# BraveGroup/DCD

Hardware: AMD Instinct MI355X
Metric: images/sec DGDE train step (bs=8, 384x1280) (higher is better)
Workload: dtype f32; 1 GPU; DGDE train bs=8 fp32 on 1xMI355X, synthetic KITTI 384x1280 + random kpts_ann (DGDE.yaml, DLA-34+DCNv2, 6 objects/image); global_batch=8, per_gpu_batch=8, input=384x1280, parallelism=dp1, dcn_precision=f32, step_launch=eager, sync_bn=False

## Files before the change

dcd_amd/_ext.py:

```python
import torch

from . import _lib

import threading

PRECISION = {"f32": 0, "bf16x3": 1, "bf16": 2}
_default_precision = "f32"
_scoped = threading.local()


def set_precision(name):
    global _default_precision
    if name not in PRECISION:
        raise ValueError("precision must be one of %s" % sorted(PRECISION))
    _default_precision = name


def get_precision():
    return getattr(_scoped, "name", None) or _default_precision


class precision_scope:

    def __init__(self, name):
# ... 25 lines not shown
    _lib.require_cuda(input, weight, bias, offset, mask)
    for name, t in (("input", input), ("weight", weight), ("bias", bias), ("offset", offset), ("mask", mask)):
        if t.dtype != torch.float32:
            raise RuntimeError("%s must be float32 (the op is fp32-only, like the reference)" % name)
    if input.dim() != 4 or weight.dim() != 4:
        raise RuntimeError("input and weight must be 4-D")
    if weight.shape[2] != kernel_h or weight.shape[3] != kernel_w:
        raise RuntimeError("Input shape and kernel shape wont match: (%d x %d vs %d x %d)." % (
            kernel_h, kernel_w, weight.shape[2], weight.shape[3]))
    if input.shape[1] != weight.shape[1]:
        raise RuntimeError("Input shape and kernel channels wont match: (%d vs %d)." % (input.shape[1], weight.shape[1]))
    if bias.numel() != weight.shape[0]:
        raise RuntimeError("bias must have Cout elements")


def _dims(input, weight, kernel_h, kernel_w, stride_h, stride_w, pad_h, pad_w, dilation_h, dilation_w):
    B, C, H, W = input.shape
    Ho = (H + 2 * pad_h - (dilation_h * (kernel_h - 1) + 1)) // stride_h + 1
    Wo = (W + 2 * pad_w - (dilation_w * (kernel_w - 1) + 1)) // stride_w + 1
    return B, C, H, W, weight.shape[0], Ho, Wo


def _workspace(L, input, geom):
    nbytes = L.dcd_dcn_v2_workspace_bytes(*geom)
    if nbytes == 0:
        raise RuntimeError("dcn_v2: unsupported geometry %s" % (geom,))
    return torch.empty(nbytes, dtype=torch.uint8, device=input.device), nbytes


def dcn_v2_forward(input, weight, bias, offset, mask, kernel_h, kernel_w, stride_h, stride_w,
                   pad_h, pad_w, dilation_h, dilation_w, deformable_group, precision=None):
    _check(input, weight, bias, offset, mask, kernel_h, kernel_w)
    L = _lib.lib()
    B, C, H, W, Co, Ho, Wo = _dims(input, weight, kernel_h, kernel_w, stride_h, stride_w, pad_h, pad_w,
                                   dilation_h, dilation_w)
    if tuple(offset.shape) != (B, 2 * deformable_group * kernel_h * kernel_w, Ho, Wo):
        raise RuntimeError("offset shape %s does not match (B, 2*dg*kh*kw, Ho, Wo)" % (tuple(offset.shape),))
    if tuple(mask.shape) != (B, deformable_group * kernel_h * kernel_w, Ho, Wo):
        raise RuntimeError("mask shape %s does not match (B, dg*kh*kw, Ho, Wo)" % (tuple(mask.shape),))
    input, weight, bias, offset, mask = (t.contiguous() for t in (input, weight, bias, offset, mask))
    geom = (B, C, H, W, Co, kernel_h, kernel_w, stride_h, stride_w, pad_h, pad_w, dilation_h, dilation_w,
            deformable_group)
    ws, nbytes = _workspace(L, input, geom)
    output = torch.empty((B, Co, Ho, Wo), dtype=torch.float32, device=input.device)
    prec = PRECISION[precision or get_precision()]
    st = L.dcd_dcn_v2_forward(_lib.stream_of(input), input.data_ptr(), weight.data_ptr(), bias.data_ptr(),
                              offset.data_ptr(), mask.data_ptr(), output.data_ptr(), *geom, prec,
                              ws.data_ptr(), nbytes)
    _lib.check(st, "dcd_dcn_v2_forward")
    return output


def dcn_v2_backward(input, weight, bias, offset, mask, grad_output, kernel_h, kernel_w, stride_h, stride_w,
                    pad_h, pad_w, dilation_h, dilation_w, deformable_group, precision=None):
    _check(input, weight, bias, offset, mask, kernel_h, kernel_w)
    _lib.require_cuda(grad_output)
    if not input.is_contiguous():
        raise RuntimeError("input tensor has to be contiguous")
    if not weight.is_contiguous():
        raise RuntimeError("weight tensor has to be contiguous")
    L = _lib.lib()
    B, C, H, W, Co, Ho, Wo = _dims(input, weight, kernel_h, kernel_w, stride_h, stride_w, pad_h, pad_w,
                                   dilation_h, dilation_w)
    if tuple(grad_output.shape) != (B, Co, Ho, Wo):
        raise RuntimeError("grad_output shape %s does not match the output" % (tuple(grad_output.shape),))
    if grad_output.dtype != torch.float32:
        raise RuntimeError("grad_output must be float32")
    bias, offset, mask, grad_output = (t.contiguous() for t in (bias, offset, mask, grad_output))
    geom = (B, C, H, W, Co, kernel_h, kernel_w, stride_h, stride_w, pad_h, pad_w, dilation_h, dilation_w,
            deformable_group)
    ws, nbytes = _workspace(L, input, geom)
    grad_input = torch.empty_like(input)
    grad_offset = torch.empty_like(offset)
    grad_mask = torch.empty_like(mask)
    grad_weight = torch.empty_like(weight)
    grad_bias = torch.empty_like(bias)
    prec = PRECISION[precision or get_precision()]
    st = L.dcd_dcn_v2_backward(_lib.stream_of(input), input.data_ptr(), weight.data_ptr(), bias.data_ptr(),
                               offset.data_ptr(), mask.data_ptr(), grad_output.data_ptr(),
                               grad_input.data_ptr(), grad_offset.data_ptr(), grad_mask.data_ptr(),
                               grad_weight.data_ptr(), grad_bias.data_ptr(), *geom, prec, ws.data_ptr(), nbytes)
    _lib.check(st, "dcd_dcn_v2_backward")
    return [grad_input, grad_offset, grad_mask, grad_weight, grad_bias]
```

dcd_amd/_lib.py:

```python
import ctypes
import os

_HERE = os.path.dirname(os.path.abspath(__file__))
LIB_PATH = os.path.join(_HERE, "libdcd_hip.so")
_LIB = None

c_void_p, c_int, c_float, c_size_t, c_int64, c_double = (ctypes.c_void_p, ctypes.c_int, ctypes.c_float,
                                                         ctypes.c_size_t, ctypes.c_int64, ctypes.c_double)


class LossRowsArgs(ctypes.Structure):
    _INTS = ("B", "M", "C", "K", "NP", "num_classes", "ch_box2d", "ch_offset", "ch_corner", "ch_corner_unc", "ch_dims",
             "ch_ori_cls", "ch_ori_off", "ch_depth", "ch_depth_unc", "ch_kpts2d", "ch_kpts3d", "trunc_log")
    _FLOATS = ("depth_lo", "depth_hi", "unc_lo", "unc_hi", "depth_weight")
    _POINTERS = ("pois", "reg_mask", "trunc_mask", "find_pcl", "ori_mask", "cls_ids", "centers", "pad_size", "bboxes",
                 "locations", "rotys", "offset_3D", "dimensions", "orientations", "keypoints", "kp_depth_mask", "kpts2d",
                 "kpts3d", "calib_P", "calib", "dim_mean", "kps_pred", "kps_tgt", "kps3d_pred", "kps3d_tgt", "rot", "P_rows",
                 "kmask", "pair_depth", "pair_mask", "cols", "corners_pred", "corners_tgt", "iou3d", "sums", "grad_sums",
                 "grad_pois", "grad_pair", "grad_kps", "grad_kps3d")
    _fields_ = ([(n, c_int) for n in _INTS] + [(n, c_float) for n in _FLOATS] + [("dim_weight", c_float * 3)]
                + [("down_ratio", c_float), ("kd_eps", c_float)] + [(n, c_void_p) for n in _POINTERS])

HEADS_MAX = 16


class HeadRowsArgs(ctypes.Structure):
    _fields_ = ([(n, c_int) for n in ("n_heads", "T", "R", "K", "C")]
                + [(n, c_int * HEADS_MAX) for n in ("trunk", "ch0", "out")]
                + [("weight", c_void_p * HEADS_MAX), ("bias", c_void_p * HEADS_MAX), ("feat", c_void_p), ("y", c_void_p),
                   ("grad_y", c_void_p), ("grad_feat", c_void_p), ("grad_weight", c_void_p * HEADS_MAX),
                   ("grad_bias", c_void_p * HEADS_MAX)])


class EvalMatchArgs(ctypes.Structure):
    _INTS = ("mode", "n_img", "n_comb", "n_rows", "G", "D", "n_dc", "max_dt", "T", "n_slots")
    _POINTERS = ("gt_off", "dt_off", "dc_off", "pair_off", "overlaps", "ign_gt", "ign_dt", "dt_score", "gt_alpha", "dt_alpha",
                 "dt_box2d", "dc_box", "comb", "min_overlap", "thresholds", "n_thresh", "scores", "counts", "sim_part")
    _fields_ = [(n, c_int) for n in _INTS] + [("P", c_int64)] + [(n, c_void_p) for n in _POINTERS]


DECODE_MAX_CLASSES = 8


class DecodeArgs(ctypes.Structure):
    _INTS = ("B", "K", "C", "nk", "n_bins", "num_classes", "ch_box2d", "ch_offset", "ch_corner", "ch_corner_unc", "ch_dims",
             "ch_ori_cls", "ch_ori_off", "ch_depth", "ch_depth_unc", "ch_kpts2d", "ch_kpts3d", "orientation", "dim_mode",
             "dim_std_on", "depth_mode", "uncertainty_as_conf", "records")
    _FLOATS = ("down_ratio", "depth_lo", "depth_hi", "eps")
    _fields_ = ([(n, c_int) for n in _INTS] + [(n, c_float) for n in _FLOATS] + [("depth_ref", c_float * 2)]
                + [("dim_mean", c_float * 3 * DECODE_MAX_CLASSES), ("dim_std", c_float * 3 * DECODE_MAX_CLASSES)])


class RecordsArgs(ctypes.Structure):
    _INTS = ("B", "M", "C", "nk", "n_bins", "ch_offset", "ch_ori_cls", "ch_ori_off", "ch_kpts2d", "ch_kpts3d")
    _fields_ = [(n, c_int) for n in _INTS] + [("down_ratio", c_float)]


SIGNATURES = {
    "dcd_version": (ctypes.c_char_p, []),
    "dcd_dcn_v2_workspace_bytes": (c_size_t, [c_int] * 14),
    "dcd_dcn_v2_forward": (c_int, [c_void_p] * 7 + [c_int] * 15 + [c_void_p, c_size_t]),
    "dcd_dcn_v2_backward": (c_int, [c_void_p] * 12 + [c_int] * 15 + [c_void_p, c_size_t]),
    "dcd_dcn_v2_forget": (c_int, [c_void_p]),
    "dcd_dcn_v2_policy_state": (c_int, [c_void_p, c_void_p]),
    "dcd_dcn_v2_policy_free": (c_int, []),
    "dcd_dcn_v2_set_handover": (c_int, [c_int]),
    "dcd_edge_depth_forward": (c_int, [c_void_p] * 6 + [c_int, c_int, c_int, c_float, c_float, c_int, c_int]
                               + [c_void_p] * 3),
    "dcd_edge_depth_backward": (c_int, [c_void_p] * 7 + [c_int, c_int, c_int, c_float, c_float, c_int]
                                + [c_void_p] * 2),
    "dcd_focal_loss": (c_int, [c_void_p, c_void_p, c_void_p, c_int64, c_float, c_float, c_void_p, c_void_p]),
    "dcd_giou_loss": (c_int, [c_void_p, c_void_p, c_void_p, c_int, c_void_p, c_void_p, c_void_p]),
    "dcd_nms_hm": (c_int, [c_void_p, c_void_p, c_int, c_int, c_int, c_int, c_void_p]),
    "dcd_heatmap_topk": (c_int, [c_void_p, c_void_p] + [c_int] * 6 + [c_void_p] * 5 + [c_void_p, c_size_t]),
    "dcd_heatmap_topk_workspace_bytes": (c_size_t, [c_int] * 5),
    "dcd_poi_gather": (c_int, [c_void_p, c_void_p, c_void_p] + [c_int] * 5 + [c_void_p]),
    "dcd_poi_scatter_add": (c_int, [c_void_p, c_void_p, c_void_p] + [c_int] * 5 + [c_void_p]),
    "dcd_patch_scatter_add": (c_int, [c_void_p, c_void_p, c_void_p, c_int, c_int, c_int64, c_int, c_int, c_void_p]),
    "dcd_iou3d": (c_int, [c_void_p, c_void_p, c_void_p, c_int, c_void_p]),
    "dcd_conv3x3_workspace_bytes": (c_size_t, [c_int] * 5),
    "dcd_conv3x3": (c_int, [c_void_p] * 6 + [c_int] * 6 + [c_void_p, c_size_t]),
    "dcd_conv3x3_weights_bytes": (c_size_t, [c_int] * 3),
    "dcd_conv3x3_transform_weights": (c_int, [c_void_p, c_void_p, c_int, c_int, c_void_p, c_void_p]),
    "dcd_conv3x3_transform_weights_table": (c_int, [c_void_p, c_void_p, c_int]),
    "dcd_conv3x3_prepared": (c_int, [c_void_p] * 6 + [c_int] * 6 + [c_void_p, c_size_t]),
    "dcd_conv3x3_split_weights_bytes": (c_size_t, [c_int] * 3),
    "dcd_conv3x3_split_transform_weights": (c_int, [c_void_p, c_void_p, c_int, c_int, c_void_p, c_void_p]),
    "dcd_conv3x3_split_transform_weights_table": (c_int, [c_void_p, c_void_p, c_int]),
    "dcd_conv3x3_split_workspace_bytes": (c_size_t, [c_int] * 5),
    "dcd_conv3x3_split_prepared": (c_int, [c_void_p] * 6 + [c_int] * 7 + [c_void_p, c_size_t]),
    "dcd_conv1x1_bf16": (c_int, [c_void_p, c_void_p, c_int, c_int, c_int, c_void_p, c_void_p, c_void_p, c_int, c_int, c_int64]),
    "dcd_conv1x1_wrw_bf16_workspace_bytes": (c_size_t, [c_int, c_int, c_int, c_int64]),
    "dcd_conv1x1_wrw_bf16": (c_int, [c_void_p, c_void_p, c_void_p, c_void_p, c_int, c_int, c_int, c_int, c_int64, c_void_p, c_size_t]),
    "dcd_conv3x3_s2_f32": (c_int, [c_void_p, c_void_p, c_void_p, c_void_p, c_int, c_int, c_int, c_int, c_int]),
    "dcd_conv3x3_s2_f32_backward_data": (c_int, [c_void_p, c_void_p, c_void_p, c_void_p, c_int, c_int, c_int, c_int, c_int]),
    "dcd_conv3x3_s2_f32_wrw_workspace_bytes": (c_size_t, [c_int, c_int, c_int, c_int, c_int]),
    "dcd_conv3x3_s2_f32_wrw": (c_int, [c_void_p, c_void_p, c_void_p, c_void_p, c_int, c_int, c_int, c_int, c_int, c_void_p, c_size_t]),
    "dcd_clip_adamw_workspace_bytes": (c_size_t, [c_int, c_void_p]),
    "dcd_clip_grad_norm_scalars": (c_int, [c_void_p, c_int, c_void_p, c_void_p, c_float, c_void_p, c_size_t, c_void_p]),
    "dcd_adamw_apply": (c_int, [c_void_p, c_int] + [c_void_p] * 7 + [c_double] * 4 + [c_void_p]),
    "dcd_conv1x1_f32": (c_int, [c_void_p, c_void_p, c_int, c_int, c_int, c_void_p, c_void_p, c_void_p, c_int, c_int, c_int64]),
    "dcd_conv1x1_wrw_f32_workspace_bytes": (c_size_t, [c_int, c_int, c_int, c_int64]),
    "dcd_conv1x1_wrw_f32": (c_int, [c_void_p, c_void_p, c_void_p, c_void_p, c_int, c_int, c_int, c_int, c_int64, c_void_p, c_size_t]),
    "dcd_conv3x3_bf16_weights_bytes": (c_size_t, [c_int] * 3),
    "dcd_conv3x3_bf16_transform_weights": (c_int, [c_void_p, c_void_p, c_int, c_int, c_void_p, c_void_p]),
    "dcd_conv3x3_bf16_transform_weights_table": (c_int, [c_void_p, c_void_p, c_int]),
    "dcd_conv3x3_bf16_workspace_bytes": (c_size_t, [c_int] * 5),
    "dcd_conv3x3_bf16_prepared": (c_int, [c_void_p] * 6 + [c_int] * 6 + [c_void_p, c_size_t]),
    "dcd_conv_stem_workspace_bytes": (c_size_t, [c_int] * 3),
    "dcd_conv_stem": (c_int, [c_void_p] * 4 + [c_int] * 7 + [c_void_p, c_size_t]),
    "dcd_conv_stem_wrw_workspace_bytes": (c_size_t, [c_int] * 3),
    "dcd_conv_stem_wrw": (c_int, [c_void_p] * 4 + [c_int] * 6 + [c_void_p, c_size_t]),
    "dcd_context_norm_forward": (c_int, [c_void_p] * 4 + [c_int, c_int, c_float]),
    "dcd_context_norm_backward": (c_int, [c_void_p] * 5 + [c_int, c_int]),
    "dcd_context_norm_relu_add_forward": (c_int, [c_void_p] * 4 + [c_int, c_int, c_float]),
    "dcd_gmw_refine": (c_int, [c_void_p] * 5 + [c_int, c_void_p, c_void_p, c_int, c_int, c_int] + [c_void_p] * 3),
    "dcd_gmw_pack_records": (c_int, [c_void_p] * 4 + [c_int, c_int, c_void_p, c_int, c_int, c_int] + [c_void_p] * 9),
    "dcd_sum_tensors": (c_int, [c_void_p, c_void_p, c_int, c_void_p, c_int64]),
    "dcd_conv3x3_wrw_workspace_bytes": (c_size_t, [c_int] * 5),
    "dcd_conv3x3_wrw": (c_int, [c_void_p] * 4 + [c_int] * 6 + [c_void_p, c_size_t]),
    "dcd_upsample_dw_forward": (c_int, [c_void_p] * 4 + [c_int] * 5),
    "dcd_upsample_dw_forward_add": (c_int, [c_void_p] * 5 + [c_int] * 5),
    "dcd_maxpool2x2_forward": (c_int, [c_void_p, c_void_p, c_void_p, c_int64, c_int, c_int]),
    "dcd_maxpool2x2_backward": (c_int, [c_void_p, c_void_p, c_void_p, c_void_p, c_int64, c_int, c_int]),
    "dcd_upsample_dw_backward": (c_int, [c_void_p] * 6 + [c_int] * 5),
    "dcd_bn_workspace_bytes": (c_size_t, [c_int]),
    "dcd_bn_stats": (c_int, [c_void_p, c_void_p, c_int, c_int, c_int64, c_void_p, c_void_p, c_size_t]),
    "dcd_channel_sums": (c_int, [c_void_p, c_void_p, c_int, c_int, c_int64, c_void_p, c_void_p, c_size_t]),
    "dcd_bn_train_apply": (c_int, [c_void_p] * 6 + [c_double] + [c_void_p] * 3 + [c_float, c_float, c_int] + [c_void_p] * 3
                           + [c_int, c_int, c_int64]),
    "dcd_bn_eval_apply": (c_int, [c_void_p] * 7 + [c_float, c_int, c_void_p, c_int, c_int, c_int64]),
    "dcd_bn_backward_stats": (c_int, [c_void_p] * 5 + [c_int, c_int, c_int64, c_void_p, c_void_p, c_size_t]),
    "dcd_trunk_row_sums": (c_int, [c_void_p, c_void_p, c_void_p, c_int, c_int, c_void_p]),
    "dcd_trunk_finalize_forward": (c_int, [c_void_p, c_void_p, c_void_p, c_void_p, c_double, c_double, c_int, c_void_p, c_void_p, c_void_p]),
    "dcd_trunk_finalize_backward": (c_int, [c_void_p, c_void_p, c_void_p, c_void_p, c_void_p, c_double, c_int, c_void_p, c_void_p, c_void_p]),
    "dcd_trunk_grad_wg": (c_int, [c_void_p, c_void_p, c_void_p, c_int, c_int, c_void_p]),
    "dcd_bn_backward_relu_from_x": (c_int, [c_void_p] * 10 + [c_int, c_int, c_int64, c_void_p, c_size_t]),
    "dcd_bn_backward_stats_params_relu_from_x": (c_int, [c_void_p] * 7 + [c_int, c_int, c_int64, c_void_p, c_void_p, c_void_p, c_void_p, c_size_t]),
# ... 80 lines not shown
```

dcd_amd/csrc/conv.hip:

```cpp
#include <hip/hip_runtime.h>
#include <stdint.h>
#include <stdlib.h>

#include "../../include/dcd_hip.h"
#include "tuning_env.h"
#include "lds_limit.h"
#include "bf16_split.h"

typedef float f32x16 __attribute__((ext_vector_type(16)));
typedef float f32x4 __attribute__((ext_vector_type(4)));
typedef float f32x2 __attribute__((ext_vector_type(2)));

namespace {

constexpr int WN_CH = 8;
constexpr int WN_NT = 512;

template <int TR, int TC, int NB>
struct WinoGeom {
    static constexpr int KS = 32 * NB;
    static constexpr int U = 16 * KS * WN_CH;
    static constexpr int NTILE = TR * TC;
    static constexpr int ROWS = 4 * TR + 2;
    static constexpr int Q = (2 * TC + 8) / 4;
// ... 59 lines not shown
        for (int b = 0; b < 3; ++b) {
            t[0][b] = g[0][b];
            t[1][b] = 0.5f * (g[0][b] + g[1][b] + g[2][b]);
            t[2][b] = 0.5f * (g[0][b] - g[1][b] + g[2][b]);
            t[3][b] = g[2][b];
        }
#pragma unroll
        for (int xi = 0; xi < 4; ++xi) {
            const float u[4] = {t[xi][0], 0.5f * (t[xi][0] + t[xi][1] + t[xi][2]), 0.5f * (t[xi][0] - t[xi][1] + t[xi][2]), t[xi][2]};
#pragma unroll
            for (int nu = 0; nu < 4; ++nu)
                ul[((((size_t)(z * nchunk + ck) * 16 + xi * 4 + nu) * 2 + h) * WN_KS + kk) * 4 + s] = u[nu];
        }
    }
}

__global__ void wino_prep_weights(const float *__restrict__ w, float *__restrict__ ul, int Cc, int Kk, int mode, int nchunk, int nz,
                                  int WN_KS)
{
    wino_prep_body(w, ul, Cc, Kk, mode, nchunk, nz, WN_KS, blockIdx.x * blockDim.x + threadIdx.x, gridDim.x * blockDim.x);
}

struct PrepBoth {
    float *ul[2];
    int Cc[2], Kk[2], nchunk[2], nz[2], ks[2];
};

__global__ void wino_prep_weights_both(const float *__restrict__ w, PrepBoth p)
{
    const int mode = blockIdx.y;
    if (!p.ul[mode]) return;
    wino_prep_body(w, p.ul[mode], p.Cc[mode], p.Kk[mode], mode, p.nchunk[mode], p.nz[mode], p.ks[mode],
                   blockIdx.x * blockDim.x + threadIdx.x, gridDim.x * blockDim.x);
}

__global__ void wino_prep_weights_table(const long long *__restrict__ table)
{
    const long long *e = table + 5 * (size_t)blockIdx.z;
    const float *w = reinterpret_cast<const float *>(e[0]);
    const int mode = blockIdx.y;
    float *ul = reinterpret_cast<float *>(e[1 + mode]);
    if (!w || !ul) return;
    const int Cin = (int)e[3], Cout = (int)e[4];
    const int Cc = mode ? Cout : Cin, Kk = mode ? Cin : Cout;
    const int WN_KS = Kk <= 32 ? 32 : 64;
    wino_prep_body(w, ul, Cc, Kk, mode, (Cc + WN_CH - 1) / WN_CH, (Kk + WN_KS - 1) / WN_KS, WN_KS,
                   blockIdx.x * blockDim.x + threadIdx.x, gridDim.x * blockDim.x);
}

template <int TR, int TC, int NB>
__global__ __launch_bounds__(WN_NT) void wino_conv3x3_f32(const float *__restrict__ x, const float *__restrict__ ul, float *y,
                                                          float *__restrict__ part, const float *__restrict__ bias,
                                                          const float *residual, int Cc, int H, int W, int Kk, int tiles_x,
                                                          int nchunk, int nz)
{
    using G = WinoGeom<TR, TC, NB>;
    constexpr int WN_ROWS = G::ROWS, WN_RS = G::RS, WN_PLANE = G::PLANE, WN_IN = G::IN, WN_BUF = G::BUF, WN_Q = G::Q;
    constexpr int WN_KS = G::KS, WN_U = G::U;
    extern __shared__ __attribute__((aligned(16))) float lds[];
    const int tid = threadIdx.x;
    const int lane = tid & 63, wave = tid >> 6;
    const int p = lane & 31, h = lane >> 5;
    const int xi = wave & 3, tg = wave >> 2;
    int bx = blockIdx.x, b = blockIdx.y;
    xcd_remap(bx, b);
    const int ty = bx / tiles_x, tx = bx - ty * tiles_x;
    const int r0 = ty * (4 * TR), c0 = tx * (2 * TC);
    const int z = blockIdx.z % nz, ks = blockIdx.z / nz, ksplit = gridDim.z / nz;
    const int ck0 = (int)((int64_t)ks * nchunk / ksplit), ck1 = (int)((int64_t)(ks + 1) * nchunk / ksplit);
    const int HW = H * W;
    const bool live = p < G::NTILE;
    const int pe = live ? p : 0;
    const int trow = pe / TC, tcol = pe - trow * TC;

    const int ra = xi == 0 ? 0 : 1, rb = xi == 3 ? 3 : 2;
    const float sa = xi == 2 ? -1.f : 1.f, sb = (xi == 0 || xi == 3) ? -1.f : 1.f;
    const int lanebase = (2 * TR * tg + 2 * trow) * WN_RS + 2 + 2 * tcol + h * WN_PLANE;
    const int base1 = lanebase + ra * WN_RS, base2 = lanebase + rb * WN_RS;

    const float *x_b = x + (size_t)b * Cc * HW;
    const float *ul_z = ul + (size_t)z * nchunk * WN_U;

    constexpr int KIN = (WN_CH * WN_ROWS * WN_Q + WN_NT - 1) / WN_NT;
    constexpr int KW = WN_U / 4 / WN_NT;
    int sg[KIN], sl[KIN];
    bool sv_[KIN];
#pragma unroll
    for (int k = 0; k < KIN; ++k) {
        const int e = tid + WN_NT * k;
        const int ch = e / (WN_ROWS * WN_Q), rem = e - ch * (WN_ROWS * WN_Q);
        const int row = rem / WN_Q, q = rem - row * WN_Q;
        const int yy = r0 - 1 + row, xx = c0 - 4 + 4 * q;
        sv_[k] = e < WN_CH * WN_ROWS * WN_Q;
        sg[k] = (sv_[k] && yy >= 0 && yy < H && xx >= 0 && xx < W) ? ch * HW + yy * W + xx : -1;
        sl[k] = ch * WN_PLANE + row * WN_RS + 4 * q;
    }
    f32x4 rin[KIN];
    auto issue_w = [&](int ck, float *buf) {
        const float *src = ul_z + (size_t)ck * WN_U + 4 * tid;
        float *dst = buf + WN_IN + 4 * 64 * __builtin_amdgcn_readfirstlane(wave);
#pragma unroll
        for (int k = 0; k < KW; ++k)
            __builtin_amdgcn_global_load_lds(src + 4 * WN_NT * k, (__attribute__((address_space(3))) void *)(dst + 4 * WN_NT * k), 16, 0, 0);
    };
    auto issue = [&](int ck) {
        const float *src = x_b + (size_t)ck * WN_CH * HW;
        const int cleft = Cc - ck * WN_CH;
// ... 55 lines not shown
            if (s + 1 < 4) {
                win_read4(cp1 + 2 * (s + 1) * WN_PLANE, qa);
                win_read4(cp2 + 2 * (s + 1) * WN_PLANE, qb);
            }
#endif
            const float v[4] = {t0 - t2, t1 + t2, t2 - t1, t1 - t3};
            __builtin_amdgcn_sched_barrier(0);
#pragma unroll
            for (int nu = 0; nu < 4; ++nu) {
                acc[nu][0] = __builtin_amdgcn_mfma_f32_32x32x2f32(a0[nu][s], v[nu], acc[nu][0], 0, 0, 0);
                if (NB == 2) acc[nu][NB - 1] = __builtin_amdgcn_mfma_f32_32x32x2f32(a1[nu][s], v[nu], acc[nu][NB - 1], 0, 0, 0);
            }
        }
#ifndef WN_ABL_NOSTAGE
        if (ck + 1 < ck1) commit(lds + ((ck + 1 - ck0) & 1) * WN_BUF);
#endif
        asm volatile("s_waitcnt vmcnt(0)" ::: "memory");
        __syncthreads();
    }
#ifdef WN_ABL_NOEPI
    if (acc[0][0][0] != 123.456f) return;
#endif

    float *ex = lds;
    float *y_b = (ks == 0 ? y : part + (size_t)(ks - 1) * gridDim.y * Kk * HW) + (size_t)b * Kk * HW;
    const float *r_b = (residual && ks == 0) ? residual + (size_t)b * Kk * HW : nullptr;
    const int orow0 = r0 + 2 * TR * tg + 2 * trow, ocol = c0 + 2 * tcol;
#pragma unroll
    for (int mb = 0; mb < NB; ++mb) {
        float *mine = ex + (size_t)wave * 32 * 64 + lane;
#pragma unroll
        for (int r = 0; r < 16; ++r) {
            mine[r * 64] = acc[0][mb][r] + acc[1][mb][r] + acc[2][mb][r];
            mine[(16 + r) * 64] = acc[1][mb][r] - acc[2][mb][r] - acc[3][mb][r];
        }
        __syncthreads();
        const float *t0 = ex + (size_t)(tg * 4 + 0) * 32 * 64 + lane, *t1 = t0 + 32 * 64, *t2 = t1 + 32 * 64, *t3 = t2 + 32 * 64;
        if (live && ocol < W) {
#pragma unroll
            for (int rr = 0; rr < 4; ++rr) {
                const int r = 4 * xi + rr;
                const int k = z * WN_KS + mb * 32 + (r & 3) + 8 * (r >> 2) + 4 * h;
                const float a0 = t0[r * 64], a1 = t1[r * 64], a2 = t2[r * 64], a3 = t3[r * 64];
                const float b0 = t0[(16 + r) * 64], b1 = t1[(16 + r) * 64], b2 = t2[(16 + r) * 64], b3 = t3[(16 + r) * 64];
                if (k < Kk) {
                    const float bk = (bias && ks == 0) ? bias[k] : 0.f;
                    const size_t o = (size_t)k * HW + (size_t)orow0 * W + ocol;
                    float *dst = y_b + o;
                    f32x2 r0 = {bk, bk}, r1 = {bk, bk};
                    if (r_b) {
                        if (orow0 < H) r0 += *reinterpret_cast<const f32x2 *>(r_b + o);
                        if (orow0 + 1 < H) r1 += *reinterpret_cast<const f32x2 *>(r_b + o + W);
                    }
                    if (orow0 < H) *reinterpret_cast<f32x2 *>(dst) = f32x2{a0 + a1 + a2 + r0.x, b0 + b1 + b2 + r0.y};
                    if (orow0 + 1 < H) *reinterpret_cast<f32x2 *>(dst + W) = f32x2{a1 - a2 - a3 + r1.x, b1 - b2 - b3 + r1.y};
                }
            }
        }
        __syncthreads();
    }
}

constexpr int WS_CH = 16;

template <int NB>
__device__ __forceinline__ void wino_prep_split_body(const float *__restrict__ w, unsigned *__restrict__ us, int Cc, int Kk, int mode,
                                                     int nchunk, int nz, int first, int step)
{
    constexpr int KS = 32 * NB;
    const int n = nz * nchunk * KS * 2 * 4;
    for (int idx = first; idx < n; idx += step) {
        int r = idx;
        const int d = r & 3; r >>= 2;
        const int h = r & 1; r >>= 1;
        const int kk = r % KS; r /= KS;
        const int ck = r % nchunk, z = r / nchunk;
        const int k = z * KS + kk;
        float u[2][16];
#pragma unroll
        for (int e = 0; e < 2; ++e) {
            const int c = ck * WS_CH + 2 * (2 * d + e) + h;
            float g[3][3];
#pragma unroll
            for (int a = 0; a < 3; ++a)
#pragma unroll
                for (int b = 0; b < 3; ++b) {
                    float v = 0.f;
                    if (k < Kk && c < Cc)
                        v = mode == 0 ? w[(((size_t)k * Cc + c) * 3 + a) * 3 + b] : w[(((size_t)c * Kk + k) * 3 + (2 - a)) * 3 + (2 - b)];
                    g[a][b] = v;
                }
            float t[4][3];
#pragma unroll
            for (int b = 0; b < 3; ++b) {
                t[0][b] = g[0][b];
                t[1][b] = 0.5f * (g[0][b] + g[1][b] + g[2][b]);
                t[2][b] = 0.5f * (g[0][b] - g[1][b] + g[2][b]);
                t[3][b] = g[2][b];
            }
#pragma unroll
            for (int xi = 0; xi < 4; ++xi) {
                u[e][xi * 4 + 0] = t[xi][0];
                u[e][xi * 4 + 1] = 0.5f * (t[xi][0] + t[xi][1] + t[xi][2]);
                u[e][xi * 4 + 2] = 0.5f * (t[xi][0] - t[xi][1] + t[xi][2]);
                u[e][xi * 4 + 3] = t[xi][2];
            }
        }
        const int ob = kk >> 5, lane = h * 32 + (kk & 31);
// ... 521 lines not shown
    }
}

}

struct ConvPlan {
    int geom;
    int nb;
    int tiles_x, tiles_y, nchunk, nz, ksplit;
};

static int device_cus()
{
    static int cus = 0;
    if (!cus) {
        int dev = 0, n = 0;
        if (hipGetDevice(&dev) != hipSuccess || hipDeviceGetAttribute(&n, hipDeviceAttributeMultiprocessorCount, dev) != hipSuccess || n <= 0)
            n = 256;
        cus = n;
    }
    return cus;
}

static ConvPlan conv_plan(int B, int Cc, int H, int W, int Kk)
{
    ConvPlan best{};
    const int cus = device_cus();
    int64_t best_cost = -1;
    for (int g = 0; g < 2; ++g) {
        ConvPlan p;
        p.geom = g;
        p.tiles_x = g == 0 ? (W + 31) / 32 : (W + 19) / 20;
        p.tiles_y = g == 0 ? (H + 7) / 8 : (H + 11) / 12;
        p.nchunk = (Cc + WN_CH - 1) / WN_CH;
        p.nb = Kk <= 32 ? 1 : 2;
        p.nz = (Kk + 32 * p.nb - 1) / (32 * p.nb);
        const int64_t wgs = (int64_t)p.tiles_x * p.tiles_y * B * p.nz;
        static const int min_chunks = dcd_env("DCD_CONV_MINCHUNK") ? atoi(dcd_env("DCD_CONV_MINCHUNK")) : 4;
        int ks = 1;
        while (ks < 8 && wgs * (ks * 2) <= cus && p.nchunk / (ks * 2) >= min_chunks) ks *= 2;
        p.ksplit = ks;
        const int64_t rounds = (wgs * ks + cus - 1) / cus;
        const int64_t cost = rounds * ((p.nchunk + ks - 1) / ks + 2) * (g == 0 ? 16 : 17);
        if (best_cost < 0 || cost < best_cost) {
            best_cost = cost;
            best = p;
        }
    }
    return best;
}

template <int TR, int TC, int NB>
static int conv_launch(hipStream_t stream, const ConvPlan &pl, const float *input, const float *ul, float *output, float *part,
                       const float *bias, const float *residual, int B, int Cc, int H, int W, int Kk)
{
    static LdsLimit lds_limit;
    size_t ldsb = (size_t)2 * WinoGeom<TR, TC, NB>::BUF * sizeof(float);
    if (ldsb < (size_t)8 * 32 * 64 * sizeof(float)) ldsb = (size_t)8 * 32 * 64 * sizeof(float);
    if (!lds_limit.raise((int)ldsb, wino_conv3x3_f32<TR, TC, NB>)) return DCD_ERR_LAUNCH;
    hipLaunchKernelGGL((wino_conv3x3_f32<TR, TC, NB>), dim3(pl.tiles_x * pl.tiles_y, B, pl.nz * pl.ksplit), dim3(WN_NT), ldsb, stream,
                       input, ul, output, part, bias, residual, Cc, H, W, Kk, pl.tiles_x, pl.nchunk, pl.nz);
    return DCD_OK;
}

template <int NB, int NP>
static int conv_launch_split(hipStream_t stream, const ConvPlan &pl, const float *input, const unsigned *us, float *output, float *part,
                             const float *bias, const float *residual, int B, int Cc, int H, int W, int Kk)
{
    static LdsLimit lds_limit;
    using G = WinoGeom<2, 16, NB>;
    const size_t ldsb = ((size_t)((WS_CH * G::PLANE + 3) & ~3) + (size_t)2 * 16 * NB * 2 * 256) * sizeof(float);
    if (!lds_limit.raise((int)ldsb, wino_conv3x3_split<NB, NP>)) return DCD_ERR_LAUNCH;
    hipLaunchKernelGGL((wino_conv3x3_split<NB, NP>), dim3(pl.tiles_x * pl.tiles_y, B, pl.nz * pl.ksplit), dim3(WN_NT), ldsb, stream, input,
                       us, output, part, bias, residual, Cc, H, W, Kk, pl.tiles_x, pl.nchunk, pl.nz);
    return DCD_OK;
}

static ConvPlan conv_plan_split(int B, int Cc, int H, int W, int Kk)
{
    ConvPlan p;
    p.geom = 0;
    p.tiles_x = (W + 31) / 32;
    p.tiles_y = (H + 7) / 8;
    p.nchunk = (Cc + WS_CH - 1) / WS_CH;
    p.nb = Kk <= 32 ? 1 : 2;
    p.nz = (Kk + 32 * p.nb - 1) / (32 * p.nb);
    const int64_t wgs = (int64_t)p.tiles_x * p.tiles_y * B * p.nz;
    const int cus = device_cus();
    int ks = 1;
    while (ks < 8 && wgs * (ks * 2) <= cus && p.nchunk / (ks * 2) >= 2) ks *= 2;
    p.ksplit = ks;
    return p;
}

static bool conv_direct_ok(int Cc, int H, int W)
{
    return (int64_t)(Cc + DC_CH) * H * W < (1ll << 29);
}

static ConvPlan conv_plan_direct(int B, int Cc, int H, int W, int Kk)
{
    static const int pin = dcd_env("DCD_CONV_DIRECT_P") ? atoi(dcd_env("DCD_CONV_DIRECT_P")) : 0;
    const int cus = device_cus();
    ConvPlan best{};
    int64_t best_cost = -1;
    for (int P = 2; P <= 4; P += 2) {
        if (P != (pin == 4 ? 4 : 2)) continue;
        ConvPlan p;
        static const int wxpin = dcd_env("DCD_CONV_DIRECT_WX") ? atoi(dcd_env("DCD_CONV_DIRECT_WX")) : 0;
        const int wx = P == 2 && wxpin == 2 ? 2 : 1;
        p.geom = P | (wx << 4);
        p.tiles_x = (W + 32 * wx - 1) / (32 * wx);
        p.tiles_y = (H + 4 * P - 1) / (4 * P);
        p.nchunk = (Cc + DC_CH - 1) / DC_CH;
// ... 4 lines not shown
        int ks = 1;
        while (ks < 8) {
            const int64_t next = wgs * ks * 2;
            const int left = p.nchunk / (ks * 2);
            const bool fill = next <= 3 * cus && left >= min_chunks;
            const bool small = 2 * next <= 3 * cus && left >= 2;
            if (!fill && !small) break;
            ks *= 2;
        }
        p.ksplit = ks;
        best = p;
    }
    (void)best_cost;
    return best;
}

template <int NB, int P, int MODE, int WX>
static int conv_launch_direct(hipStream_t stream, const ConvPlan &pl, const float *input, const unsigned *wd, float *output, float *part,
                              const float *bias, const float *residual, int B, int Cc, int H, int W, int Kk)
{
    static LdsLimit lds_limit;
    const size_t ldsb = ((size_t)2 * (4 * P + 2) * (32 * WX + 8) + (size_t)2 * 9 * NB * 64) * 16;
    if constexpr (MODE == 2) {
        if (!lds_limit.raise((int)ldsb, conv3x3_direct_bf16_w4<NB, P, WX>)) return DCD_ERR_LAUNCH;
        hipLaunchKernelGGL((conv3x3_direct_bf16_w4<NB, P, WX>), dim3(pl.tiles_x * pl.tiles_y, B, pl.nz * pl.ksplit), dim3(DC_NT * WX), ldsb,
                           stream, input, wd, output, part, bias, residual, Cc, H, W, Kk, pl.tiles_x, pl.nchunk, pl.nz);
    } else {
        if (!lds_limit.raise((int)ldsb, conv3x3_direct_bf16<NB, P, MODE, WX>)) return DCD_ERR_LAUNCH;
        hipLaunchKernelGGL((conv3x3_direct_bf16<NB, P, MODE, WX>), dim3(pl.tiles_x * pl.tiles_y, B, pl.nz * pl.ksplit), dim3(DC_NT * WX), ldsb,
                           stream, input, wd, output, part, bias, residual, Cc, H, W, Kk, pl.tiles_x, pl.nchunk, pl.nz);
    }
    return DCD_OK;
}

static size_t tw_dwords_split(int Cin, int Cout, int backward_data)
{
    const int Cc = backward_data ? Cout : Cin, Kk = backward_data ? Cin : Cout;
    const int nb = Kk <= 32 ? 1 : 2;
    return (size_t)((Cc + WS_CH - 1) / WS_CH) * ((Kk + 32 * nb - 1) / (32 * nb)) * 16 * nb * 2 * 256;
}

extern "C" {

size_t dcd_conv3x3_workspace_bytes(int B, int Cin, int H, int W, int Cout)
{
    if (B <= 0 || Cin <= 0 || Cout <= 0 || H <= 0 || W <= 0) return 0;
    const int cmax = Cin > Cout ? Cin : Cout;
    const size_t nchunk = (size_t)(cmax + WN_CH - 1) / WN_CH, nz = (size_t)(cmax + 63) / 64;
    const ConvPlan f = conv_plan(B, Cin, H, W, Cout), d = conv_plan(B, Cout, H, W, Cin);
    const size_t pf = (size_t)(f.ksplit - 1) * B * Cout * H * W, pd = (size_t)(d.ksplit - 1) * B * Cin * H * W;
    return (nchunk * nz * 16 * 64 * WN_CH + (pf > pd ? pf : pd)) * sizeof(float);
}

static int conv3x3_run(hipStream_t stream, const float *input, const float *weights, int prepared, const float *bias,
                       const float *residual, float *output, int B, int Cin, int H, int W, int Cout, int backward_data, void *workspace,
                       size_t workspace_bytes)
{
    (void)hipGetLastError();
    if (!input || !weights || !output || B <= 0 || Cin <= 0 || Cout <= 0 || H <= 0 || W <= 0) return DCD_ERR_BAD_ARG;
    if ((W & 3) || (H & 1) || (int64_t)(Cin > Cout ? Cin : Cout) * H * W >= (1ll << 31) || (bias && backward_data)) return DCD_ERR_BAD_ARG;
    const int Cc = backward_data ? Cout : Cin, Kk = backward_data ? Cin : Cout;
    ConvPlan pl = conv_plan(B, Cc, H, W, Kk);
    if (const char *e = dcd_env("DCD_CONV_GEOM")) {
        const int g = atoi(e);
        if (g == 0 || g == 1) {
            ConvPlan q = pl;
            q.geom = g;
            q.tiles_x = g == 0 ? (W + 31) / 32 : (W + 19) / 20;
            q.tiles_y = g == 0 ? (H + 7) / 8 : (H + 11) / 12;
            q.ksplit = 1;
            pl = q;
        }
    }
    const int ksz = 32 * pl.nb;
    const size_t ul_floats = prepared ? 0 : (size_t)pl.nchunk * pl.nz * 16 * ksz * WN_CH;
    const size_t img = (size_t)B * Kk * H * W;
    const size_t need = (ul_floats + (size_t)(pl.ksplit - 1) * img) * sizeof(float);
    if (need && (!workspace || workspace_bytes < need)) return DCD_ERR_WORKSPACE;
    float *part = (float *)workspace + ul_floats;
    const float *ul = weights;
    if (!prepared) {
        const int nprep = pl.nz * pl.nchunk * ksz * WN_CH;
        hipLaunchKernelGGL(wino_prep_weights, dim3((nprep + 255) / 256 < 4096 ? (nprep + 255) / 256 : 4096), dim3(256), 0, stream, weights,
                           (float *)workspace, Cc, Kk, backward_data ? 1 : 0, pl.nchunk, pl.nz, ksz);
        ul = (const float *)workspace;
    }
    const int st = pl.geom == 0 ? (pl.nb == 2 ? conv_launch<2, 16, 2>(stream, pl, input, ul, output, part, bias, residual, B, Cc, H, W, Kk)
                                              : conv_launch<2, 16, 1>(stream, pl, input, ul, output, part, bias, residual, B, Cc, H, W, Kk))
                                : (pl.nb == 2 ? conv_launch<3, 10, 2>(stream, pl, input, ul, output, part, bias, residual, B, Cc, H, W, Kk)
                                              : conv_launch<3, 10, 1>(stream, pl, input, ul, output, part, bias, residual, B, Cc, H, W, Kk));
    if (st != DCD_OK) return st;
    if (pl.ksplit > 1) {
        const size_t n4 = img / 4;
        const int nb = (int)((n4 + 255) / 256 < 2048 ? (n4 + 255) / 256 : 2048);
        hipLaunchKernelGGL(wino_sum_partials, dim3(nb), dim3(256), 0, stream, output, (const float *)part, n4, pl.ksplit - 1);
    }
    return hipGetLastError() == hipSuccess ? DCD_OK : DCD_ERR_LAUNCH;
}

int dcd_conv3x3(void *stream_, const float *input, const float *weight, const float *bias, const float *residual, float *output,
                int B, int Cin, int H, int W, int Cout, int backward_data, void *workspace, size_t workspace_bytes)
{
    if (!workspace) return DCD_ERR_BAD_ARG;
    return conv3x3_run((hipStream_t)stream_, input, weight, 0, bias, residual, output, B, Cin, H, W, Cout, backward_data, workspace,
                       workspace_bytes);
}

static size_t tw_floats(int Cin, int Cout, int backward_data)
{
    const int Cc = backward_data ? Cout : Cin, Kk = backward_data ? Cin : Cout;
    const int nb = Kk <= 32 ? 1 : 2, ks = 32 * nb;
    return (size_t)((Cc + WN_CH - 1) / WN_CH) * ((Kk + ks - 1) / ks) * 16 * ks * WN_CH;
}

size_t dcd_conv3x3_weights_bytes(int Cin, int Cout, int backward_data)
{
    return Cin > 0 && Cout > 0 ? tw_floats(Cin, Cout, backward_data) * sizeof(float) : 0;
}

int dcd_conv3x3_transform_weights(void *stream_, const float *weight, int Cin, int Cout, float *forward_out, float *backward_out)
{
    (void)hipGetLastError();
    if (!weight || Cin <= 0 || Cout <= 0 || (!forward_out && !backward_out)) return DCD_ERR_BAD_ARG;
    PrepBoth p;
    int nmax = 0;
    for (int mode = 0; mode < 2; ++mode) {
        const int Cc = mode ? Cout : Cin, Kk = mode ? Cin : Cout;
        p.ul[mode] = mode ? backward_out : forward_out;
        p.Cc[mode] = Cc;
        p.Kk[mode] = Kk;
        p.ks[mode] = Kk <= 32 ? 32 : 64;
        p.nchunk[mode] = (Cc + WN_CH - 1) / WN_CH;
        p.nz[mode] = (Kk + p.ks[mode] - 1) / p.ks[mode];
        const int n = p.nz[mode] * p.nchunk[mode] * p.ks[mode] * WN_CH;
        if (p.ul[mode] && n > nmax) nmax = n;
    }
    const int nb = (nmax + 255) / 256 < 4096 ? (nmax + 255) / 256 : 4096;
    hipLaunchKernelGGL(wino_prep_weights_both, dim3(nb, 2), dim3(256), 0, (hipStream_t)stream_, weight, p);
    return hipGetLastError() == hipSuccess ? DCD_OK : DCD_ERR_LAUNCH;
}

int dcd_conv3x3_transform_weights_table(void *stream_, const long long *table, int entries)
{
// ... 109 lines not shown
int dcd_conv3x3_bf16_transform_weights_table(void *stream_, const long long *table, int entries)
{
    (void)hipGetLastError();
    if (!table || entries <= 0 || entries > 65535) return DCD_ERR_BAD_ARG;
    hipLaunchKernelGGL(direct_prep_weights_table, dim3(32, 2, entries), dim3(256), 0, (hipStream_t)stream_, table);
    return hipGetLastError() == hipSuccess ? DCD_OK : DCD_ERR_LAUNCH;
}

size_t dcd_conv3x3_bf16_workspace_bytes(int B, int Cin, int H, int W, int Cout)
{
    if (B <= 0 || Cin <= 0 || Cout <= 0 || H <= 0 || W <= 0) return 0;
    const size_t pf = (size_t)(conv_plan_direct(B, Cin, H, W, Cout).ksplit - 1) * B * Cout * H * W;
    const size_t pd = (size_t)(conv_plan_direct(B, Cout, H, W, Cin).ksplit - 1) * B * Cin * H * W;
    return (pf > pd ? pf : pd) * sizeof(float) + 16;
}

int dcd_conv3x3_bf16_prepared(void *stream_, const float *input, const void *transformed, const float *bias, const float *residual,
                              float *output, int B, int Cin, int H, int W, int Cout, int backward_data, void *workspace,
                              size_t workspace_bytes)
{
    hipStream_t stream = (hipStream_t)stream_;
    (void)hipGetLastError();
    if (!input || !transformed || !output || B <= 0 || Cin <= 0 || Cout <= 0 || H <= 0 || W <= 0) return DCD_ERR_BAD_ARG;
    if (bias && backward_data) return DCD_ERR_BAD_ARG;
    const int Cc = backward_data ? Cout : Cin, Kk = backward_data ? Cin : Cout;
    if (!conv_direct_ok(Cc, H, W) || (int64_t)Kk * H * W >= (1ll << 31) || (W & 3)) return DCD_ERR_BAD_ARG;
    const ConvPlan pl = conv_plan_direct(B, Cc, H, W, Kk);
    const size_t img = (size_t)B * Kk * H * W;
    const size_t need = (size_t)(pl.ksplit - 1) * img * sizeof(float);
    if (need && (!workspace || workspace_bytes < need)) return DCD_ERR_WORKSPACE;
    if (pl.ksplit > 1 && (img & 3)) return DCD_ERR_BAD_ARG;
    float *part = (float *)workspace;
    const unsigned *wd = (const unsigned *)transformed;
    static const int mpin = dcd_env("DCD_CONV_DIRECT_MODE") ? atoi(dcd_env("DCD_CONV_DIRECT_MODE")) : -1;
    const int P = pl.geom & 15, wx = pl.geom >> 4;
    const int mode = P == 4 ? 0 : (mpin >= 0 ? mpin : 1);
#define DCD_DIRECT(NB_, P_, M_, WX_) conv_launch_direct<NB_, P_, M_, WX_>(stream, pl, input, wd, output, part, bias, residual, B, Cc, H, W, Kk)
#define DCD_DIRECT_NB(NB_)                                                                                                              \
    (P == 4 ? DCD_DIRECT(NB_, 4, 0, 1)                                                                                                  \
            : wx == 2 ? (mode == 2 ? DCD_DIRECT(NB_, 2, 2, 2) : DCD_DIRECT(NB_, 2, 1, 2))                                               \
                      : (mode == 2 ? DCD_DIRECT(NB_, 2, 2, 1) : mode == 1 ? DCD_DIRECT(NB_, 2, 1, 1) : DCD_DIRECT(NB_, 2, 0, 1)))
    const int st = pl.nb == 2 ? DCD_DIRECT_NB(2) : DCD_DIRECT_NB(1);
#undef DCD_DIRECT_NB
#undef DCD_DIRECT
    if (st != DCD_OK) return st;
    if (pl.ksplit > 1) {
        const size_t n4 = img / 4;
        const int nb = (int)((n4 + 255) / 256 < 2048 ? (n4 + 255) / 256 : 2048);
        hipLaunchKernelGGL(wino_sum_partials, dim3(nb), dim3(256), 0, stream, output, (const float *)part, n4, pl.ksplit - 1);
    }
    return hipGetLastError() == hipSuccess ? DCD_OK : DCD_ERR_LAUNCH;
}

int dcd_conv1x1_bf16(void *stream_, const float *weight, int ldw, int transposed, int n_inputs, const float *const *inputs,
                     const int *channels, float *output, int B, int M, long long HW)
{
    (void)hipGetLastError();
    if (!weight || !inputs || !channels || !output || n_inputs < 1 || n_inputs > 4 || B <= 0 || M <= 0 || HW <= 0 || (HW & 3) || ldw <= 0)
        return DCD_ERR_BAD_ARG;
    PwArgs a;
    a.n_in = n_inputs;
    a.K = 0;
    for (int i = 0; i < 4; ++i) {
        a.in[i] = i < n_inputs ? inputs[i] : nullptr;
        a.ch[i] = i < n_inputs ? channels[i] : 0;
        if (i < n_inputs && (!inputs[i] || channels[i] <= 0 || (channels[i] & 15) || (int64_t)channels[i] * HW >= (1ll << 29)))
            return DCD_ERR_BAD_ARG;
        a.K += a.ch[i];
    }
    if ((int64_t)M * HW >= (1ll << 31)) return DCD_ERR_BAD_ARG;
    a.w = weight; a.ldw = ldw; a.wt = transposed ? 1 : 0; a.out = output; a.M = M; a.HW = HW;
    const int nb = M <= 32 ? 1 : 2;
    dim3 grid((unsigned)((HW + 511) / 512), B, (M + 32 * nb - 1) / (32 * nb));
    if (nb == 2) hipLaunchKernelGGL(pw_conv_bf16<2>, grid, dim3(PW_NT), 0, (hipStream_t)stream_, a);
    else hipLaunchKernelGGL(pw_conv_bf16<1>, grid, dim3(PW_NT), 0, (hipStream_t)stream_, a);
    return hipGetLastError() == hipSuccess ? DCD_OK : DCD_ERR_LAUNCH;
}

static void pw_wrw_partition(int B, int O, int C, long long HW, int &nog, int &ncg, int &S)
{
    nog = (O + 63) / 64;
    ncg = (C + 127) / 128;
    const int64_t T = (int64_t)B * ((HW + 63) / 64);
    int64_t s = 2 * (int64_t)device_cus() / (nog * ncg);
    if (s > T / 4) s = T / 4;
    if (s < 1) s = 1;
    S = (int)s;
}

size_t dcd_conv1x1_wrw_bf16_workspace_bytes(int B, int O, int C, long long HW)
{
    if (B <= 0 || O <= 0 || C <= 0 || HW <= 0) return 0;
    int nog, ncg, S;
    pw_wrw_partition(B, O, C, HW, nog, ncg, S);
    return (size_t)nog * ncg * S * 64 * 128 * sizeof(float);
}

int dcd_conv1x1_wrw_bf16(void *stream_, const float *grad_output, const float *input, float *grad_weight, int ldw, int B, int O, int C,
                         long long HW, void *workspace, size_t workspace_bytes)
{
    hipStream_t stream = (hipStream_t)stream_;
    (void)hipGetLastError();
    if (!grad_output || !input || !grad_weight || !workspace || B <= 0 || O <= 0 || C <= 0 || HW <= 0 || (HW & 3) || ldw < C)
        return DCD_ERR_BAD_ARG;
    if ((int64_t)B * (O > C ? O : C) * HW >= (1ll << 29)) return DCD_ERR_BAD_ARG;
    int nog, ncg, S;
// ... 215 lines not shown
```

dcd_amd/csrc/dcn_bwd_sweep.inc:

```

#ifndef SW_ABL_TAPS
#define SW_ABL_TAPS 9
#endif
#ifdef SW_ABL_NOMFMA
__device__ __forceinline__ f32x4 sw_fake_mfma(float a, float b, f32x4 c) { c.x = fmaf(a, b, c.x); c.y += a; c.z += b; c.w = fmaf(a, b, c.w); return c; }
#define SW_MFMA(a, b, c) sw_fake_mfma(a, b, c)
#else
#define SW_MFMA(a, b, c) __builtin_amdgcn_mfma_f32_16x16x4f32(a, b, c, 0, 0, 0)
#endif
constexpr int SW_PX = 16;
constexpr int SW_WW = 24;
constexpr int SW_RING = 9;
constexpr int SW_CH = 16;
constexpr int SW_CELLS = SW_RING * SW_WW;
constexpr int SW_PLANE = SW_CELLS + 3;
constexpr int SW_ZERO = SW_CELLS;
constexpr int SW_W_FLOATS = 9 * 16 * 64;
constexpr int SW_DW_FLOATS = 9 * 64 * SW_CH;
constexpr int SW_PART_FLOATS = SW_DW_FLOATS + 64;

__device__ __forceinline__ void sweep_prep_weights_body(const float *__restrict__ w, float *__restrict__ wp, const Geom &g, int nck, int nob,
                                                        int bid, int nb)
{
    const int n = nck * SW_W_FLOATS * nob;
// ... 761 lines not shown
            const int e = lane + 64 * k;
            const int ch = e / SW_WW, col = e - ch * SW_WW;
            const float gv = ring[(ch * SW_PLANE + sl * SW_WW + col) * 2 + 1];
            const int xx = x0 - 4 + col;
            if (gv != 0.f && ch < cleft && yy >= 0 && yy < H && xx >= 0 && xx < W) atomicAdd(gin_c + (size_t)ch * HW + yy * W + xx, gv);
        }
    }

    if (DWK && !SPLIT) {
#pragma unroll
        for (int ob = 0; ob < 4; ++ob)
            accw[8][ob] = __builtin_amdgcn_mfma_f32_16x16x4f32(dyo_p3[ob], pend_col, accw[8][ob], 0, 0, 0);
    }
    }

    if (DWK) {
        float *dst = a.dwpart + ((size_t)ck * (a.nslot / a.nck) + (id0 / (8 * a.nck)) * 8 + (id0 & 7)) * SW_PART_FLOATS;
#pragma unroll
        for (int t = 0; t < 9; ++t)
#pragma unroll
            for (int ob = 0; ob < 4; ++ob)
#pragma unroll
                for (int i = 0; i < 4; ++i) dst[(t * 64 + 16 * ob + 4 * q + i) * SW_CH + j] = accw[t][ob][i];
#pragma unroll
        for (int ob = 0; ob < 4; ++ob) {
            float v_ = bsum[ob];
            v_ += __shfl_xor(v_, 16);
            v_ += __shfl_xor(v_, 32);
            if (q == 0) dst[SW_DW_FLOATS + 16 * ob + j] = v_;
        }
    }
}

__device__ __forceinline__ void sweep_reduce_coord_body(const float *__restrict__ cpart, float *__restrict__ goff,
                                                        float *__restrict__ gmsk, int B, int HW, int nck,
                                                        const unsigned *__restrict__ far_scal, int total_tiles, int bid, int nb)
{
    const bool zero = far_dominated(far_scal, total_tiles);
    const int64_t n4 = (int64_t)B * 27 * HW / 4, per_b4 = (int64_t)27 * HW / 4, off4 = (int64_t)18 * HW / 4;
    const size_t stride4 = (size_t)B * 27 * HW / 4;
    for (int64_t i = (int64_t)bid * blockDim.x + threadIdx.x; i < n4; i += (int64_t)nb * blockDim.x) {
        f32x4 s = {0.f, 0.f, 0.f, 0.f};
        if (!zero) s = reinterpret_cast<const f32x4 *>(cpart)[i];
        for (int ck = 1; ck < nck && !zero; ++ck) {
            const f32x4 v = reinterpret_cast<const f32x4 *>(cpart)[i + ck * stride4];
            s.x += v.x; s.y += v.y; s.z += v.z; s.w += v.w;
        }
        const int64_t b = i / per_b4, r = i - b * per_b4;
        if (r < off4) reinterpret_cast<f32x4 *>(goff)[b * off4 + r] = s;
        else reinterpret_cast<f32x4 *>(gmsk)[b * (per_b4 - off4) + (r - off4)] = s;
    }
}

__device__ __forceinline__ void sweep_reduce_dw_body(const float *__restrict__ part, float *__restrict__ gw, float *__restrict__ gbias,
                                                     const Geom &g, int nck, int nvp, const unsigned *__restrict__ far_scal,
                                                     int total_tiles, int bx, int nbx, int by, int nby)
{
    if (far_dominated(far_scal, total_tiles)) return;
    const int n = nck * SW_DW_FLOATS + 64;
    const int v0 = (int)((int64_t)by * nvp / nby), v1 = (int)((int64_t)(by + 1) * nvp / nby);
    for (int idx = bx * blockDim.x + threadIdx.x; idx < n; idx += nbx * blockDim.x) {
        const bool is_bias = idx >= nck * SW_DW_FLOATS;
        const int ck = is_bias ? 0 : idx / SW_DW_FLOATS, e = is_bias ? SW_DW_FLOATS + (idx - nck * SW_DW_FLOATS) : idx - ck * SW_DW_FLOATS;
        const int c = e & 15, o = is_bias ? e - SW_DW_FLOATS : (e >> 4) & 63, t = e >> 10;
        const int cc = ck * SW_CH + c;
        if (o >= g.Co || (!is_bias && cc >= g.C)) continue;
        const float *src = part + (size_t)ck * nvp * SW_PART_FLOATS + e;
        float s = 0.f;
#pragma unroll 8
        for (int vv = v0; vv < v1; ++vv) s += src[(size_t)vv * SW_PART_FLOATS];
        if (is_bias) atomicAdd(gbias + o, s);
        else atomicAdd(gw + ((size_t)o * g.C + cc) * 9 + t, s);
    }
}

__device__ __forceinline__ void sweep_reduce_gemm_body(const float *__restrict__ part, float *__restrict__ gw, int n, int S,
                                                       const unsigned *__restrict__ far_scal, int total_tiles, int bid, int nb)
{
    if (far_dominated(far_scal, total_tiles)) return;
    for (int i = (bid * blockDim.x + threadIdx.x) * 4; i < n; i += nb * blockDim.x * 4) {
        if (i + 3 < n) {
            f32x4 acc = {0.f, 0.f, 0.f, 0.f};
            for (int s = 0; s < S; ++s) acc += *reinterpret_cast<const f32x4 *>(part + (size_t)s * n + i);
            *reinterpret_cast<f32x4 *>(gw + i) = acc;
        } else {
            for (int j = 0; i + j < n; ++j) {
                float a = 0.f;
                for (int s = 0; s < S; ++s) a += part[(size_t)s * n + i + j];
                gw[i + j] = a;
            }
        }
    }
}

struct SweepEpilogueArgs {
    const float *cpart, *gy, *dwpart;
    float *goff, *gmsk, *gw, *gbias;
    const unsigned *far_scal, *bias_only_if_far;
    Geom g;
    int nck, nvp, total_tiles, nb_coord, bias_splits, dw_bx, dw_by, gemm_n, gemm_S;
    unsigned *far_report = nullptr;
    unsigned far_base = 0;
};
__global__ __launch_bounds__(256) void dcn_sweep_epilogue(SweepEpilogueArgs a)
{
    int bid = blockIdx.x;
    if (a.far_report && bid == 0 && threadIdx.x == 0) {
        const unsigned c = a.far_scal[3] & ~FAR_BY_COUNT;
        *a.far_report = c >= a.far_base ? c - a.far_base : 0u;
    }
    if (bid < a.nb_coord) {
        sweep_reduce_coord_body(a.cpart, a.goff, a.gmsk, a.g.B, a.g.HoWo, a.nck, a.far_scal, a.total_tiles, bid, a.nb_coord);
        return;
    }
    bid -= a.nb_coord;
    const int nb_bias = a.g.Co * a.bias_splits;
    if (bid < nb_bias) {
        bias_grad_body(a.gy, a.gbias, a.g.B, a.g.Co, a.g.HoWo, a.bias_only_if_far, bid % a.g.Co, bid / a.g.Co, a.bias_splits);
        return;
    }
    bid -= nb_bias;
    if (a.dw_by > 0)
        sweep_reduce_dw_body(a.dwpart, a.gw, a.gbias, a.g, a.nck, a.nvp, a.far_scal, a.total_tiles, bid % a.dw_bx, a.dw_bx, bid / a.dw_bx, a.dw_by);
    else
        sweep_reduce_gemm_body(a.dwpart, a.gw, a.gemm_n, a.gemm_S, a.far_scal, a.total_tiles, bid, (int)gridDim.x - a.nb_coord - nb_bias);
}

struct SweepPlan {
    int nck, nstrip, nseg, seg_rows, nv;
    int nslot;
    int nob;
    int dw_split, dw_kchunk;
    size_t wp_floats, cpart_floats, dw_floats, col_floats;
};
constexpr int SW_GEMM_T = 128, SW_GEMM_K = 16;

__host__ inline SweepPlan sweep_plan(const Geom &g)
{
    SweepPlan p;
    p.nck = (g.C + SW_CH - 1) / SW_CH;
    p.nstrip = (g.W + SW_PX - 1) / SW_PX;
    const int64_t base = (int64_t)g.B * p.nstrip * p.nck;
    static const int min_rows = dcd_env("DCD_SWEEP_MIN_ROWS") && atoi(dcd_env("DCD_SWEEP_MIN_ROWS")) > 0 ? atoi(dcd_env("DCD_SWEEP_MIN_ROWS")) : 3;
    int best = 1;
    int64_t best_cost = -1;
    for (int ns = 1; ns <= g.H; ++ns) {
        const int rows = (g.H + ns - 1) / ns;
        if (rows < min_rows && ns > 1) break;
        const int real_ns = (g.H + rows - 1) / rows;
        const int64_t total = base * real_ns;
        const int64_t cost = ((total + 1023) / 1024) * (rows + 5);
        if (best_cost < 0 || cost < best_cost) { best_cost = cost; best = real_ns; }
    }
    p.seg_rows = (g.H + best - 1) / best;
    p.nseg = (g.H + p.seg_rows - 1) / p.seg_rows;
    p.nv = g.B * p.nstrip * p.nseg;
    const int64_t units = (int64_t)((p.nv + 7) / 8) * 8 * p.nck;
    const int grp = 8 * p.nck;
    int64_t slots = units < 1024 ? units : (1024 / grp) * (int64_t)grp;
    if (slots < grp) slots = grp;
    if (const char *e = dcd_env("DCD_SWEEP_SLOTS")) {
        const int64_t v_ = atoll(e);
        slots = v_ <= 0 ? units : (v_ / grp > 0 ? v_ / grp : 1) * grp;
    }
// ... 45 lines not shown
```

dcd_amd/csrc/dcn_v2.hip:

```cpp

#include <hip/hip_runtime.h>
#include <stdint.h>
#include <stdlib.h>
#include <string.h>
#include <atomic>
#include <map>
#include <vector>
#include <mutex>
#include <utility>

#include "../../include/dcd_hip.h"
#include "tuning_env.h"
#include "lds_limit.h"

typedef float f32x16 __attribute__((ext_vector_type(16)));
typedef float f32x32 __attribute__((ext_vector_type(32)));

namespace {

template <int N> struct IntC {
    static constexpr int value = N;
};

struct Geom {
    int B, C, H, W, Co, kh, kw, sh, sw, ph, pw, dh, dw, dg;
    int Ho, Wo, HoWo, KK, cpg, cpgp, Kp, Cop;
};

__host__ inline int round_up(int x, int m) { return (x + m - 1) / m * m; }

__host__ inline bool make_geom(Geom &g, int B, int C, int H, int W, int Co, int kh, int kw, int sh, int sw, int ph,
                               int pw, int dh, int dw, int dg)
{
    if (B <= 0 || C <= 0 || H <= 0 || W <= 0 || Co <= 0 || kh <= 0 || kw <= 0 || sh <= 0 || sw <= 0 || ph < 0 ||
        pw < 0 || dh <= 0 || dw <= 0 || dg <= 0 || C % dg)
        return false;
    g.B = B; g.C = C; g.H = H; g.W = W; g.Co = Co; g.kh = kh; g.kw = kw; g.sh = sh; g.sw = sw;
    g.ph = ph; g.pw = pw; g.dh = dh; g.dw = dw; g.dg = dg;
    g.Ho = (H + 2 * ph - (dh * (kh - 1) + 1)) / sh + 1;
    g.Wo = (W + 2 * pw - (dw * (kw - 1) + 1)) / sw + 1;
    if (g.Ho <= 0 || g.Wo <= 0) return false;
    g.HoWo = g.Ho * g.Wo;
    g.KK = kh * kw;
    g.cpg = C / dg;
    g.cpgp = round_up(g.cpg, 32);
    g.Kp = dg * g.KK * g.cpgp;
    g.Cop = round_up(Co, 32);
    if ((int64_t)C * H * W >= (1ll << 31) || (int64_t)Co * g.HoWo >= (1ll << 31) ||
        (int64_t)g.Kp * g.Cop >= (1ll << 31) || (int64_t)dg * 2 * g.KK * g.HoWo >= (1ll << 31))
        return false;
    return true;
}

__device__ __forceinline__ void prep_weights_body(const float *__restrict__ w, float *__restrict__ wf, float *__restrict__ wb, const Geom &g,
                                                  int bid, int nb)
{
    const int n = g.Kp * g.Cop;
    for (int idx = bid * blockDim.x + threadIdx.x; idx < n; idx += nb * blockDim.x) {
        const int o = idx / g.Kp, kp = idx - o * g.Kp;
        const int seg = kp / g.cpgp, cc = kp - seg * g.cpgp;
        const int grp = seg / g.KK, t = seg - grp * g.KK;
        float v = 0.f;
        if (o < g.Co && cc < g.cpg) v = w[((size_t)o * g.C + grp * g.cpg + cc) * g.KK + t];
        wb[idx] = v;
        wf[(size_t)kp * g.Cop + o] = v;
    }
// ... 1927 lines not shown
__device__ __forceinline__ void zero_ranges_body(const ZeroRanges &z, unsigned bid, unsigned nb)
{
    if (z.mark_p && bid == 0 && threadIdx.x == 0) *z.mark_p = z.mark_v;
#pragma unroll
    for (int r = 0; r < 8; ++r) {
        unsigned *p = z.p[r];
        const unsigned n = z.n[r];
        for (unsigned i = bid * blockDim.x + threadIdx.x; i < n; i += nb * blockDim.x) p[i] = 0u;
    }
}
__global__ void dcn_zero_ranges(ZeroRanges z) { zero_ranges_body(z, blockIdx.x, gridDim.x); }

inline int pick_mb(int nb, int tiles_total)
{
    for (int mb = 8; mb > 1; mb >>= 1) {
        if (mb > nb) continue;
        if ((int64_t)tiles_total * ((nb + mb - 1) / mb) >= 1024) return mb;
    }
    return 1;
}

#include "dcn_v2_bf16x3.inc"
#include "dcn_bwd_sweep.inc"

}

namespace {

template <int V>
__global__ void dcn_offset_mask_split(const float *__restrict__ out, float *__restrict__ offset, float *__restrict__ mask, int B, int T,
                                      int64_t HW)
{
    const int64_t per_img = (int64_t)3 * T * HW / V, n = (int64_t)B * per_img;
    for (int64_t i = (int64_t)blockIdx.x * blockDim.x + threadIdx.x; i < n; i += (int64_t)gridDim.x * blockDim.x) {
        const int64_t b = i / per_img, r = (i - b * per_img) * V;
        const bool is_off = r < (int64_t)2 * T * HW;
        float *dst = is_off ? offset + b * 2 * T * HW + r : mask + b * T * HW + (r - (int64_t)2 * T * HW);
        if (V == 4) {
            f32x4 v = *reinterpret_cast<const f32x4 *>(out + b * 3 * T * HW + r);
            if (!is_off) {
#pragma unroll
                for (int j = 0; j < 4; ++j) v[j] = 1.f / (1.f + __expf(-v[j]));
            }
            *reinterpret_cast<f32x4 *>(dst) = v;
        } else {
            const float v = out[b * 3 * T * HW + r];
            *dst = is_off ? v : 1.f / (1.f + __expf(-v));
        }
    }
}

template <int V>
__global__ void dcn_offset_mask_merge(const float *__restrict__ goff, const float *__restrict__ gmask, const float *__restrict__ mask,
                                      float *__restrict__ gout, int B, int T, int64_t HW)
{
    const int64_t per_img = (int64_t)3 * T * HW / V, n = (int64_t)B * per_img;
    for (int64_t i = (int64_t)blockIdx.x * blockDim.x + threadIdx.x; i < n; i += (int64_t)gridDim.x * blockDim.x) {
        const int64_t b = i / per_img, r = (i - b * per_img) * V;
        const bool is_off = r < (int64_t)2 * T * HW;
        const int64_t rm = r - (int64_t)2 * T * HW;
        if (V == 4) {
            f32x4 v;
            if (is_off) v = *reinterpret_cast<const f32x4 *>(goff + b * 2 * T * HW + r);
            else {
                const f32x4 g = *reinterpret_cast<const f32x4 *>(gmask + b * T * HW + rm);
                const f32x4 m = *reinterpret_cast<const f32x4 *>(mask + b * T * HW + rm);
#pragma unroll
                for (int j = 0; j < 4; ++j) v[j] = g[j] * m[j] * (1.f - m[j]);
            }
            *reinterpret_cast<f32x4 *>(gout + b * 3 * T * HW + r) = v;
        } else {
            float v;
            if (is_off) v = goff[b * 2 * T * HW + r];
            else {
                const float m = mask[b * T * HW + rm];
                v = gmask[b * T * HW + rm] * m * (1.f - m);
            }
            gout[b * 3 * T * HW + r] = v;
        }
    }
}

}

#include "dcn_dense.inc"

extern "C" {

static size_t dw_partial_floats(int Cin, int Cout)
{
    const size_t nb = (size_t)((Cin + DW_CB - 1) / DW_CB) * ((Cout + TL_OB - 1) / TL_OB);
    return (nb > 512 ? nb : 512) * (size_t)(2 * 32 * DW_CB * 9);
}

static size_t tileflag_bytes(const Geom &g) { return ((size_t)g.B * ((g.H + 3) / 4) * ((g.W + 31) / 32) + 255) / 256 * 256; }

static size_t blockmax_bytes(const Geom &g)
{
    return ((size_t)g.B * g.dg * g.KK * ((g.Ho + 7) / 8) * ((g.Wo + 7) / 8) + 255) / 256 * 256 + tileflag_bytes(g);
}

static size_t base_workspace_bytes(const Geom &g)
{
    const size_t cells = (size_t)g.B * g.dg * g.KK * g.H * g.W;
    const size_t ntile = (size_t)g.B * ((g.HoWo + 31) / 32);
    const size_t n = (size_t)g.Kp * g.Cop * sizeof(float) * 2 + 256 + ((cells + 255) / 256 * 256) + cells * INV_CAP * 8 + 256 +
                     ((ntile + 255) / 256 * 256) + (ntile + 63) / 64 * 64 * sizeof(int) + dw_partial_floats(g.C, g.Co) * sizeof(float);
    return (n + 255) / 256 * 256 + blockmax_bytes(g);
}

size_t dcd_dcn_v2_workspace_bytes(int B, int Cin, int H, int W, int Cout, int kh, int kw, int sh, int sw, int ph,
                                  int pw, int dh, int dw, int dg)
{
    Geom g;
    if (!make_geom(g, B, Cin, H, W, Cout, kh, kw, sh, sw, ph, pw, dh, dw, dg)) return 0;
    return base_workspace_bytes(g) + dense_workspace_bytes(g) + sweep_workspace_bytes(g);
}

int dcd_dcn_v2_forward(void *stream_, const float *input, const float *weight, const float *bias,
                       const float *offset, const float *mask, float *output, int B, int Cin, int H, int W,
                       int Cout, int kh, int kw, int sh, int sw, int ph, int pw, int dh, int dw, int dg,
                       int precision, void *workspace, size_t workspace_bytes)
{
    hipStream_t stream = (hipStream_t)stream_;
    (void)hipGetLastError();
    Geom g;
    if (!input || !weight || !bias || !offset || !mask || !output || !workspace) return DCD_ERR_BAD_ARG;
    if (!make_geom(g, B, Cin, H, W, Cout, kh, kw, sh, sw, ph, pw, dh, dw, dg)) return DCD_ERR_BAD_ARG;
    if (precision != DCD_PREC_F32 && precision != DCD_PREC_BF16X3 && precision != DCD_PREC_BF16) return DCD_ERR_BAD_ARG;
    const bool split = precision != DCD_PREC_F32;
    const bool one = precision == DCD_PREC_BF16;
    const size_t nw = (size_t)g.Kp * g.Cop;
    if (workspace_bytes < nw * sizeof(float) * 2) return DCD_ERR_WORKSPACE;
    if (dense_ok(g, false)) {
        if (workspace_bytes < base_workspace_bytes(g) + dense_workspace_bytes(g)) return DCD_ERR_WORKSPACE;
        dense_forward(stream, input, weight, bias, offset, mask, output, g, (float *)((char *)workspace + base_workspace_bytes(g)),
                      precision);
        return hipGetLastError() == hipSuccess ? DCD_OK : DCD_ERR_LAUNCH;
    }
    float *wf = (float *)workspace, *wb = wf + nw;

    const int tiles = (g.HoWo + 31) / 32;
    const int nb = g.Cop / 32;
    const int mb = pick_mb(nb, tiles * B);
    dim3 grid((tiles + 3) / 4, B, (nb + mb - 1) / mb), block(256);
#ifndef DCN_NO_FWD_TILE
    if (kh == 3 && kw == 3 && sh == 1 && sw == 1 && ph == 1 && pw == 1 && dh == 1 && dw == 1 && dg == 1 && (W & 3) == 0 &&
        H >= 8 && W >= 32 && dcd_env("DCD_NO_TILE") == nullptr) {
        const int nz = (Cout + TL_OB - 1) / TL_OB;
        const int nchunk = split ? (Cin + TB_CH - 1) / TB_CH : (Cin + TL_CH - 1) / TL_CH;
        const size_t nwl = (size_t)nz * nchunk * (split ? TB_W_FLOATS : TL_W_FLOATS);
        if (nwl <= 2 * nw) {
            static LdsLimit lds_limit8, lds_limit4, lds_limit8b, lds_limit4b;
            static int tile_rows = 0;
            if (tile_rows == 0) {
                const char *e = dcd_env("DCD_TILE_ROWS");
                tile_rows = (e && atoi(e) == 4) ? 4 : 8;
            }
            if (!lds_limit8.raise((int)(2 * TileCfg<8>::BUF * sizeof(float)), dcn_fwd_tile_f32<8>) ||
                !lds_limit4.raise((int)(2 * TileCfg<4>::BUF * sizeof(float)), dcn_fwd_tile_f32<4>))
                return DCD_ERR_LAUNCH;
            if (split && (!lds_limit8b.raise((int)(TileCfgB<8>::NBUF * TileCfgB<8>::BUF * sizeof(float)), dcn_fwd_tile_bf16x3<8, 3>,
                                             dcn_fwd_tile_bf16x3<8, 1>) ||
                          !lds_limit4b.raise((int)(TileCfgB<4>::NBUF * TileCfgB<4>::BUF * sizeof(float)), dcn_fwd_tile_bf16x3<4, 3>,
                                             dcn_fwd_tile_bf16x3<4, 1>)))
                return DCD_ERR_LAUNCH;
            static int rescue_taps = 0;
            if (rescue_taps == 0) {
                const char *e = dcd_env("DCD_FWD_RESCUE_TAPS");
// ... 35 lines not shown
                }
#undef DCD_FWD_TILE_B
                else if (rows8)
                    hipLaunchKernelGGL(dcn_fwd_tile_f32<8>, dim3(regions, B, nz), dim3(512), 2 * TileCfg<8>::BUF * sizeof(float), stream,
                                       input, offset, mask, wf, bias, output, g, tiles_x, nchunk, flags, (const float *)wf9, rescue_taps_call,
                                       (const unsigned *)far_count, far_limit);
                else
                    hipLaunchKernelGGL(dcn_fwd_tile_f32<4>, dim3(regions, B, nz), dim3(256), 2 * TileCfg<4>::BUF * sizeof(float), stream,
                                       input, offset, mask, wf, bias, output, g, tiles_x, nchunk, flags, (const float *)wf9, rescue_taps_call,
                                       (const unsigned *)far_count, far_limit);
                if (keeps) return hipGetLastError() == hipSuccess ? DCD_OK : DCD_ERR_LAUNCH;
                const int nb9 = g.Cop / 32, mb9 = nb9 >= 4 ? 4 : nb9 >= 2 ? 2 : 1;
                dim3 gridr((tiles_x * g.Ho + 3) / 4, B, (nb9 + mb9 - 1) / mb9);
                if (mb9 == 4)
                    hipLaunchKernelGGL((dcn_fwd9_f32<4, true>), gridr, dim3(256), 0, stream, input, offset, mask, wf9, bias, output, g,
                                       (const unsigned char *)flags, tiles_x, TRr, nchunk);
                else if (mb9 == 2)
                    hipLaunchKernelGGL((dcn_fwd9_f32<2, true>), gridr, dim3(256), 0, stream, input, offset, mask, wf9, bias, output, g,
                                       (const unsigned char *)flags, tiles_x, TRr, nchunk);
                else
                    hipLaunchKernelGGL((dcn_fwd9_f32<1, true>), gridr, dim3(256), 0, stream, input, offset, mask, wf9, bias, output, g,
                                       (const unsigned char *)flags, tiles_x, TRr, nchunk);
                return hipGetLastError() == hipSuccess ? DCD_OK : DCD_ERR_LAUNCH;
            }
        }
    }
#endif
#ifndef DCN_NO_FWD9
    if (g.KK == 9 && W >= 2 && (size_t)Cin * 9 * g.Cop <= nw) {
        const size_t n9 = (size_t)Cin * 9 * g.Cop;
        hipLaunchKernelGGL(dcn_prep_weights9, dim3((unsigned)((n9 + 255) / 256 < 2048 ? (n9 + 255) / 256 : 2048)), dim3(256), 0,
                           stream, weight, wf, g);
        const int mb9 = mb > 4 ? 4 : mb;
        dim3 grid9((tiles + 3) / 4, B, (nb + mb9 - 1) / mb9);
        switch (mb9) {
            case 4: hipLaunchKernelGGL(dcn_fwd9_f32<4>, grid9, block, 0, stream, input, offset, mask, wf, bias, output, g); break;
            case 2: hipLaunchKernelGGL(dcn_fwd9_f32<2>, grid9, block, 0, stream, input, offset, mask, wf, bias, output, g); break;
            default: hipLaunchKernelGGL(dcn_fwd9_f32<1>, grid9, block, 0, stream, input, offset, mask, wf, bias, output, g); break;
        }
        return hipGetLastError() == hipSuccess ? DCD_OK : DCD_ERR_LAUNCH;
    }
#endif
    hipLaunchKernelGGL(dcn_prep_weights, dim3((unsigned)((nw + 255) / 256 < 2048 ? (nw + 255) / 256 : 2048)), dim3(256),
                       0, stream, weight, wf, wb, g);
    switch (mb) {
        case 8: hipLaunchKernelGGL(dcn_fwd_f32<8>, grid, block, 0, stream, input, offset, mask, wf, bias, output, g); break;
        case 4: hipLaunchKernelGGL(dcn_fwd_f32<4>, grid, block, 0, stream, input, offset, mask, wf, bias, output, g); break;
        case 2: hipLaunchKernelGGL(dcn_fwd_f32<2>, grid, block, 0, stream, input, offset, mask, wf, bias, output, g); break;
        default: hipLaunchKernelGGL(dcn_fwd_f32<1>, grid, block, 0, stream, input, offset, mask, wf, bias, output, g); break;
    }
    return hipGetLastError() == hipSuccess ? DCD_OK : DCD_ERR_LAUNCH;
}

int dcd_dcn_v2_backward(void *stream_, const float *input, const float *weight, const float *bias,
                        const float *offset, const float *mask, const float *grad_output, float *grad_input,
                        float *grad_offset, float *grad_mask, float *grad_weight, float *grad_bias, int B,
                        int Cin, int H, int W, int Cout, int kh, int kw, int sh, int sw, int ph, int pw, int dh,
                        int dw, int dg, int precision, void *workspace, size_t workspace_bytes)
{
    (void)bias;
    hipStream_t stream = (hipStream_t)stream_;
    (void)hipGetLastError();
    Geom g;
    if (!input || !weight || !offset || !mask || !grad_output || !grad_input || !grad_offset || !grad_mask ||
        !grad_weight || !grad_bias || !workspace)
        return DCD_ERR_BAD_ARG;
    if (!make_geom(g, B, Cin, H, W, Cout, kh, kw, sh, sw, ph, pw, dh, dw, dg)) return DCD_ERR_BAD_ARG;
    if (precision != DCD_PREC_F32 && precision != DCD_PREC_BF16X3 && precision != DCD_PREC_BF16) return DCD_ERR_BAD_ARG;
    const bool split = precision != DCD_PREC_F32;
    const bool one = precision == DCD_PREC_BF16;
    const size_t nw = (size_t)g.Kp * g.Cop;
    if (workspace_bytes + 256 < dcd_dcn_v2_workspace_bytes(B, Cin, H, W, Cout, kh, kw, sh, sw, ph, pw, dh, dw, dg))
        return DCD_ERR_WORKSPACE;
    float *wf = (float *)workspace, *wb = wf + nw;
    const size_t cells = (size_t)B * dg * g.KK * H * W;
    InvLists inv;
    unsigned *absmax = (unsigned *)(wb + nw);
    inv.absmax_bits = absmax;
    inv.cnt = (unsigned char *)absmax + 256;
    inv.idx = (int *)(inv.cnt + (cells + 255) / 256 * 256);
    inv.w = (float *)(inv.idx + cells * INV_CAP);
    inv.packed = 0;
    const size_t ntile = (size_t)B * ((g.HoWo + 31) / 32);
    unsigned char *far_flag = (unsigned char *)(((uintptr_t)(inv.w + cells * INV_CAP) + 255) / 256 * 256);
    int *far_list = (int *)(far_flag + (ntile + 255) / 256 * 256);
    float *dw_part = (float *)(far_list + (ntile + 63) / 64 * 64);
    unsigned char *blockmax = (unsigned char *)workspace + (base_workspace_bytes(g) - blockmax_bytes(g));
    inv.blockmax = blockmax;
    unsigned char *tileflag = (unsigned char *)workspace + (base_workspace_bytes(g) - tileflag_bytes(g));
    inv.tileflag = nullptr;
    inv.flag_tx = (W + 31) / 32;
    inv.flag_ty = (H + 3) / 4;
    const dim3 bm_grid(((g.Ho + 7) / 8) * ((g.Wo + 7) / 8), dg * g.KK, B);

    const char *sw_e = dcd_env("DCD_SWEEP_WIDE");
    const bool sweep_wide = !(sw_e && atoi(sw_e) == 0);
    const bool use_sweep = sweep_ok(g) && (g.Cop <= 64 || (sweep_wide && (g.Cop <= 128 || !dense_ok(g, true)))) && dense_mode() != 1 &&
                           (sweep_mode() == 1 || !dense_ok(g, true));
    unsigned *dense_report = nullptr;
    const bool far_to_dense = use_sweep && dense_ok(g, true) &&
                              handover_far_dominated(weight, far_count_limit(g, g.Co > 64), &dense_report);
    if ((!use_sweep || far_to_dense) && dense_ok(g, true)) {
        ZeroRanges z;
        for (int r = 0; r < 8; ++r) { z.p[r] = nullptr; z.n[r] = 0; }
        z.p[0] = absmax; z.n[0] = 4;
        z.p[1] = (unsigned *)far_flag; z.n[1] = (unsigned)((ntile + 3) / 4);
        z.p[3] = (unsigned *)grad_bias; z.n[3] = (unsigned)Cout;
        hipLaunchKernelGGL(dcn_zero_ranges, dim3(8), dim3(256), 0, stream, z);
        hipLaunchKernelGGL(dcn_prep_weights, dim3((unsigned)((nw + 255) / 256 < 2048 ? (nw + 255) / 256 : 2048)), dim3(256),
                           0, stream, weight, wf, wb, g);
        const int64_t noff = (int64_t)B * dg * 2 * g.KK * g.HoWo;
        int gsz = (int)((noff + 4095) / 4096);
        if (gsz > 512) gsz = 512;
        hipLaunchKernelGGL(dcn_offset_absmax, dim3(gsz), dim3(256), 0, stream, offset, noff, absmax, g.HoWo, dg * 2 * g.KK,
                           (g.HoWo + 31) / 32, far_flag, far_list);
        if (dense_report) hipLaunchKernelGGL(dcn_far_report, dim3(1), dim3(64), 0, stream, (const unsigned *)absmax, dense_report);
        hipLaunchKernelGGL(dcn_offset_blockmax, bm_grid, dim3(64), 0, stream, offset, g, blockmax);
        hipLaunchKernelGGL(dcn_build_inverse, dim3((H * W + 255) / 256, dg * g.KK, B), dim3(256), 0, stream, offset, mask, inv, g);
        int splits = (int)(((int64_t)g.HoWo + 4095) / 4096);
        if (splits > 32) splits = 32;
        hipLaunchKernelGGL(dcn_bias_grad, dim3(Cout, splits), dim3(256), 0, stream, grad_output, grad_bias, B, Cout, g.HoWo);
        dense_backward(stream, input, wb, offset, mask, grad_output, grad_input, grad_offset, grad_mask, grad_weight, g, inv,
                       (float *)((char *)workspace + base_workspace_bytes(g)), precision);
        return hipGetLastError() == hipSuccess ? DCD_OK : DCD_ERR_LAUNCH;
    }
    const int tiles = (g.HoWo + 31) / 32;
    const int nblk = g.cpgp / 32;
    if (!use_sweep)
        hipLaunchKernelGGL(dcn_prep_weights, dim3((unsigned)((nw + 255) / 256 < 2048 ? (nw + 255) / 256 : 2048)), dim3(256),
                           0, stream, weight, wf, wb, g);
    if (use_sweep) {
        const SweepPlan sp = sweep_plan(g);
        float *swp = (float *)((char *)workspace + base_workspace_bytes(g) + dense_workspace_bytes(g));
        float *cpart = swp + sp.wp_floats, *dwpart = cpart + sp.cpart_floats;
        const unsigned *fs = (const unsigned *)absmax;
        int nsplit = 1;
        while (nsplit * 2 <= nblk) nsplit *= 2;
        unsigned *far_report = nullptr;
        const unsigned real_limit = far_count_limit(g, sp.nob > 1);
        const int handover = handover_decide(stream, weight, real_limit, &far_report);
        const unsigned far_limit = handover ? real_limit : FAR_COUNT_PIVOT - 1;
        {
            const int nb_gen = handover ? (int)((nw + 255) / 256 < 1024 ? (nw + 255) / 256 : 1024) : 0;
            const int nb_sw = (int)((sp.wp_floats + 255) / 256 < 2048 ? (sp.wp_floats + 255) / 256 : 2048);
            hipLaunchKernelGGL(dcn_sweep_prologue_a, dim3(nb_gen + nb_sw), dim3(256), 0, stream, weight, wf, wb, swp, absmax, g, sp.nck, sp.nob,
                               split ? 1 : 0, nb_gen, far_limit);
        }
        {
            ZeroRanges z;
            for (int r = 0; r < 8; ++r) { z.p[r] = nullptr; z.n[r] = 0; }
            z.p[2] = (unsigned *)grad_weight; z.n[2] = (unsigned)((size_t)Cout * Cin * g.KK);
            z.p[3] = (unsigned *)grad_bias; z.n[3] = (unsigned)Cout;
            z.p[4] = (unsigned *)grad_input; z.n[4] = (unsigned)((size_t)B * Cin * H * W);
            const int nb_zero = (int)(z.n[4] / 1024 + 1 < 4096 ? z.n[4] / 1024 + 1 : 4096);
            const int64_t noff = (int64_t)B * 18 * g.HoWo;
            int nb_scan = (int)((noff + 4095) / 4096);
            if (nb_scan > 512) nb_scan = 512;
            hipLaunchKernelGGL(dcn_sweep_prologue_b, dim3(nb_zero + nb_scan), dim3(256), 0, stream, z, nb_zero, offset, noff, absmax, g.HoWo,
                               (g.HoWo + 31) / 32);
        }
        {
            SweepArgs a;
            a.in = input; a.off = offset; a.msk = mask; a.wp = swp; a.gy = grad_output; a.gin = grad_input; a.cpart = cpart;
            a.dwpart = dwpart; a.far_scal = fs; a.g = g; a.nstrip = sp.nstrip; a.nseg = sp.nseg; a.seg_rows = sp.seg_rows;
            a.nck = sp.nck; a.nv = sp.nv; a.nslot = sp.nslot;
            a.col = dwpart + sp.dw_floats;
            static LdsLimit sw_lds_limit;
            const int ldsb = SW_WAVES * SW_LDS_FLOATS * (int)sizeof(float);
            if (!sw_lds_limit.raise(ldsb, dcn_bwd_sweep<DCD_PREC_F32, 1, true>, dcn_bwd_sweep<DCD_PREC_BF16X3, 1, true>,
                                    dcn_bwd_sweep<DCD_PREC_F32, 2, false>, dcn_bwd_sweep<DCD_PREC_BF16X3, 2, false>,
                                    dcn_bwd_sweep<DCD_PREC_F32, 4, false>, dcn_bwd_sweep<DCD_PREC_BF16X3, 4, false>,
                                    dcn_bwd_sweep<DCD_PREC_BF16, 1, true>, dcn_bwd_sweep<DCD_PREC_BF16, 2, false>,
                                    dcn_bwd_sweep<DCD_PREC_BF16, 4, false>))
                return DCD_ERR_LAUNCH;
            const dim3 sgrid(sp.nslot / SW_WAVES), sblock(64 * SW_WAVES);
#define DCD_LAUNCH_SWEEP(NOBV, DWKV)                                                                                     \
    do {                                                                                                                \
        if (one) hipLaunchKernelGGL((dcn_bwd_sweep<DCD_PREC_BF16, NOBV, DWKV>), sgrid, sblock, ldsb, stream, a);        \
        else if (split) hipLaunchKernelGGL((dcn_bwd_sweep<DCD_PREC_BF16X3, NOBV, DWKV>), sgrid, sblock, ldsb, stream, a); \
        else hipLaunchKernelGGL((dcn_bwd_sweep<DCD_PREC_F32, NOBV, DWKV>), sgrid, sblock, ldsb, stream, a);             \
    } while (0)
            if (sp.nob == 1) DCD_LAUNCH_SWEEP(1, true);
            else if (sp.nob == 2) DCD_LAUNCH_SWEEP(2, false);
            else DCD_LAUNCH_SWEEP(4, false);
#undef DCD_LAUNCH_SWEEP
        }
        {
            SweepEpilogueArgs e;
            e.cpart = cpart; e.gy = grad_output; e.dwpart = dwpart; e.goff = grad_offset; e.gmsk = grad_mask; e.gw = grad_weight;
            e.gbias = grad_bias; e.far_scal = fs; e.g = g; e.nck = sp.nck; e.total_tiles = B * tiles;
            e.far_report = far_report; e.far_base = FAR_COUNT_PIVOT - far_limit;
            e.bias_only_if_far = sp.nob == 1 ? fs : (const unsigned *)nullptr;
            const int64_t n4 = (int64_t)B * 27 * g.HoWo / 4;
            e.nb_coord = (int)((n4 + 255) / 256 < 4096 ? (n4 + 255) / 256 : 4096);
            int splits = (int)(((int64_t)g.HoWo + 4095) / 4096);
            if (splits > 32) splits = 32;
            if (splits < 1) splits = 1;
            e.bias_splits = splits;
            int nb_dw;
            if (sp.nob == 1) {
                const int nred = sp.nck * SW_DW_FLOATS + 64;
                e.nvp = sp.nslot / sp.nck;
                e.dw_bx = (nred + 255) / 256;
                e.dw_by = e.nvp >= 64 ? 16 : (e.nvp >= 8 ? 4 : 1);
                e.gemm_n = 0; e.gemm_S = 0;
                nb_dw = e.dw_bx * e.dw_by;
            } else {
                static_assert(SW_GEMM_T == SG_T && SW_GEMM_K == SG_K, "sweep_plan sizes the product's partials with these");
                const int K9 = Cin * 9, n = Cout * K9;
                SgemmArgs ga;
                ga.A = grad_output; ga.B = dwpart + sp.dw_floats; ga.C = dwpart; ga.bias = nullptr; ga.M = Cout; ga.N = K9; ga.K = g.HoWo;
                ga.lda = g.HoWo; ga.ldb = g.HoWo; ga.ldc = K9;
                ga.strideA = (long long)Cout * g.HoWo; ga.strideB = (long long)K9 * g.HoWo;
                ga.strideC = (long long)sp.dw_split * n; ga.strideCs = n;
                ga.nsplit = sp.dw_split; ga.kchunk = sp.dw_kchunk; ga.ct = 0; ga.b_off = nullptr;
                ga.skip_count = fs + 3; ga.skip_above = FAR_COUNT_PIVOT;
                if (split) sgemm_bf16x3(stream, true, true, ga, B, one);
                else sgemm_f32(stream, true, true, ga, B);
                e.nvp = 0; e.dw_bx = 0; e.dw_by = 0;
                e.gemm_n = n; e.gemm_S = B * sp.dw_split;
                nb_dw = (n / 4 + 255) / 256 < 512 ? (n / 4 + 255) / 256 : 512;
            }
            hipLaunchKernelGGL(dcn_sweep_epilogue, dim3(e.nb_coord + Cout * splits + nb_dw), dim3(256), 0, stream, e);
        }
        if (!handover) return hipGetLastError() == hipSuccess ? DCD_OK : DCD_ERR_LAUNCH;
        inv.packed = 0;
        inv.tileflag = nullptr;
        hipLaunchKernelGGL(dcn_offset_blockmax, bm_grid, dim3(64), 0, stream, offset, g, blockmax, fs);
        hipLaunchKernelGGL(dcn_build_inverse, dim3((H * W + 255) / 256, 9, B), dim3(256), 0, stream, offset, mask, inv, g, fs);
        {
            const int in_tiles = (H * W + 31) / 32;
            int mbi = nblk >= 8 ? 8 : nblk >= 4 ? 4 : nblk >= 2 ? 2 : 1;
            while (mbi > 1 && (int64_t)in_tiles * B * ((nblk + mbi - 1) / mbi) < 1024) mbi >>= 1;
            dim3 grid((in_tiles + 3) / 4, B, (nblk + mbi - 1) / mbi), block(256);
            if (mbi == 8) hipLaunchKernelGGL(dcn_bwd_input_f32<8>, grid, block, 0, stream, grad_output, wb, inv, grad_input, g, 0, fs);
            else if (mbi == 4) hipLaunchKernelGGL(dcn_bwd_input_f32<4>, grid, block, 0, stream, grad_output, wb, inv, grad_input, g, 0, fs);
            else if (mbi == 2) hipLaunchKernelGGL(dcn_bwd_input_f32<2>, grid, block, 0, stream, grad_output, wb, inv, grad_input, g, 0, fs);
            else hipLaunchKernelGGL(dcn_bwd_input_f32<1>, grid, block, 0, stream, grad_output, wb, inv, grad_input, g, 0, fs);
        }
        {
            dim3 grid((tiles + 3) / 4, B, nsplit), block(256);
#define DCD_LAUNCH_BD_FAR(NS)                                                                                            \
    hipLaunchKernelGGL(dcn_bwd_data_f32<NS>, grid, block, 0, stream, input, offset, mask, wb, grad_output, grad_input,  \
                       grad_offset, grad_mask, grad_bias, g, nsplit, inv, fs, (const int *)far_list, 1)
            if (g.Cop == 32) DCD_LAUNCH_BD_FAR(16);
            else if (g.Cop == 64) DCD_LAUNCH_BD_FAR(32);
            else if (g.Cop == 128) DCD_LAUNCH_BD_FAR(64);
            else if (g.Cop == 256) DCD_LAUNCH_BD_FAR(128);
            else DCD_LAUNCH_BD_FAR(0);
#undef DCD_LAUNCH_BD_FAR
        }
        {
            const int RB = 9 * nblk;
            const int nb = g.Cop / 32;
            const int mb = nb >= 8 ? 8 : nb >= 4 ? 4 : nb >= 2 ? 2 : 1;
            const int gx = (RB + 3) / 4, gz = (nb + mb - 1) / mb;
            const int total = B * tiles;
            int S = 512 / (gx * gz);
            if (S < 1) S = 1;
            if (S > total) S = total;
            dim3 grid(gx, S, gz), block(256);
            const size_t lds = (size_t)(4 * 32 * 33 + mb * 32 * 33) * sizeof(float);
#define DCD_LAUNCH_BW_FAR(MBV)                                                                                           \
    hipLaunchKernelGGL(dcn_bwd_weight_f32<MBV>, grid, block, lds, stream, input, offset, mask, grad_output, grad_weight, g, \
                       tiles, S, fs, (const int *)far_list)
            if (mb == 8) DCD_LAUNCH_BW_FAR(8);
            else if (mb == 4) DCD_LAUNCH_BW_FAR(4);
            else if (mb == 2) DCD_LAUNCH_BW_FAR(2);
            else DCD_LAUNCH_BW_FAR(1);
#undef DCD_LAUNCH_BW_FAR
        }
        return hipGetLastError() == hipSuccess ? DCD_OK : DCD_ERR_LAUNCH;
    }
    int nsplit = 1;
    while ((int64_t)tiles * B * nsplit < 1536 && nsplit * 2 <= nblk) nsplit *= 2;

    const bool tile_shape = kh == 3 && kw == 3 && sh == 1 && sw == 1 && ph == 1 && pw == 1 && dh == 1 && dw == 1 && dg == 1 &&
                            (W & 3) == 0 && H >= 8 && W >= 32 && dcd_env("DCD_NO_TILE") == nullptr;
    static int bd128 = -1;
    if (bd128 < 0) {
        const char *e = dcd_env("DCD_BD_TILE128");
        bd128 = (e && atoi(e) == 1) ? 1 : 0;
    }
    const bool bd_tile_ok = tile_shape && (g.Cop == 64 || (g.Cop == 128 && bd128));
    {
        ZeroRanges z;
        for (int r = 0; r < 8; ++r) { z.p[r] = nullptr; z.n[r] = 0; }
        z.p[0] = absmax; z.n[0] = 4;
        z.p[1] = (unsigned *)far_flag; z.n[1] = (unsigned)((ntile + 3) / 4);
        z.p[2] = (unsigned *)grad_weight; z.n[2] = (unsigned)((size_t)Cout * Cin * g.KK);
        z.p[3] = (unsigned *)grad_bias; z.n[3] = (unsigned)Cout;
        if (nsplit > 1 || (bd_tile_ok && nblk > 1)) {
            z.p[4] = (unsigned *)grad_offset; z.n[4] = (unsigned)((size_t)B * dg * 2 * g.KK * g.HoWo);
            z.p[5] = (unsigned *)grad_mask; z.n[5] = (unsigned)((size_t)B * dg * g.KK * g.HoWo);
        }
        z.p[6] = (unsigned *)tileflag; z.n[6] = (unsigned)(tileflag_bytes(g) / 4);
        const size_t most = (size_t)z.n[2] > (size_t)z.n[4] ? z.n[2] : z.n[4];
        hipLaunchKernelGGL(dcn_zero_ranges, dim3((unsigned)(most / 1024 + 1 < 2048 ? most / 1024 + 1 : 2048)), dim3(256), 0, stream, z);
    }

    {
        const int64_t noff = (int64_t)B * dg * 2 * g.KK * g.HoWo;
        int gsz = (int)((noff + 4095) / 4096);
        if (gsz > 512) gsz = 512;
        hipLaunchKernelGGL(dcn_offset_absmax, dim3(gsz), dim3(256), 0, stream, offset, noff, absmax, g.HoWo, dg * 2 * g.KK,
                           (g.HoWo + 31) / 32, far_flag, far_list);
        const int HWin = H * W;
#ifndef DCN_NO_BWD_TILE
        static int bi_nblk = 0;
        if (bi_nblk == 0) {
            const char *e = dcd_env("DCD_BI_TILE_NBLK");
            bi_nblk = e ? atoi(e) : 2;
            if (bi_nblk < 1) bi_nblk = 2;
        }
        const bool bi_tile_ok = tile_shape && nblk <= bi_nblk && (nblk <= 2 || g.Cop <= 64) && H < 65536 && W < 65536 &&
                                dcd_env("DCD_NO_BI_TILE") == nullptr;
#else
        const bool bi_tile_ok = false;
#endif
        inv.packed = bi_tile_ok ? 1 : 0;
        static int bi_hybrid = -1;
        if (bi_hybrid < 0) {
            const char *e = dcd_env("DCD_BI_HYBRID");
            bi_hybrid = (e && atoi(e) == 0) ? 0 : 1;
        }
// ... 79 lines not shown
        if (dw_gen == 0) {
            const char *e = dcd_env("DCD_DW_GEN");
            dw_gen = (e && atoi(e) == 1) ? 1 : 2;
        }
        static int dw_colmajor = -1;
        if (dw_colmajor < 0) {
            const char *e = dcd_env("DCD_DW_ORDER");
            dw_colmajor = (e && atoi(e) == 0) ? 0 : 1;
        }
        const int tiles_x = (g.Wo + 31) / 32, tiles_y = (g.Ho + DW_TR - 1) / DW_TR;
        const int ncb = (Cin + DW_CB - 1) / DW_CB, nzo = (Cout + TL_OB - 1) / TL_OB;
        const int total = B * tiles_x * tiles_y;
        int S = 512 / (ncb * nzo);
        if (S < 1) S = 1;
        if (S > total) S = total;
        if (split)
            hipLaunchKernelGGL(dcn_bwd_weight_tile_v2<DCD_PREC_BF16X3>, dim3(ncb, S, nzo), dim3(DW_NT),
                               Dw2Cfg<DCD_PREC_BF16X3>::FLOATS * sizeof(float), stream, input, offset, mask, grad_output, dw_part, g,
                               tiles_x, tiles_y, S, (const unsigned *)absmax, dw_colmajor);
        else if (dw_gen == 2)
            hipLaunchKernelGGL(dcn_bwd_weight_tile_v2<DCD_PREC_F32>, dim3(ncb, S, nzo), dim3(DW_NT),
                               Dw2Cfg<DCD_PREC_F32>::FLOATS * sizeof(float), stream, input, offset, mask, grad_output, dw_part, g,
                               tiles_x, tiles_y, S, (const unsigned *)absmax, dw_colmajor);
        else
            hipLaunchKernelGGL(dcn_bwd_weight_tile_f32, dim3(ncb, S, nzo), dim3(DW_NT), ldsb, stream, input, offset, mask, grad_output,
                               dw_part, g, tiles_x, tiles_y, S, (const unsigned *)absmax);
        const int nred = ncb * nzo * 2 * 32 * DW_CB * 9;
        const int rgroups = S >= 16 ? 16 : S;
        hipLaunchKernelGGL(dcn_dw_reduce, dim3((nred + 255) / 256, rgroups), dim3(256), 0, stream, dw_part, grad_weight, g, ncb, nzo, S,
                           (const unsigned *)absmax);
        dw_tiled = true;
    }
#endif
    {
        const int RB = dg * g.KK * nblk;
        const int nb = g.Cop / 32;
        const int mb = nb >= 8 ? 8 : nb >= 4 ? 4 : nb >= 2 ? 2 : 1;
        const int gx = (RB + 3) / 4, gz = (nb + mb - 1) / mb;
        const int total = B * tiles;
        int S = 512 / (gx * gz);
        if (S < 1) S = 1;
        if (S > total) S = total;
        dim3 grid(gx, S, gz), block(256);
        const size_t lds = (size_t)(4 * 32 * 33 + mb * 32 * 33) * sizeof(float);
#define DCD_LAUNCH_BW(MBV)                                                                                        \
    hipLaunchKernelGGL(dcn_bwd_weight_f32<MBV>, grid, block, lds, stream, input, offset, mask, grad_output, grad_weight, g, \
                       tiles, S, dw_tiled ? (const unsigned *)absmax : (const unsigned *)nullptr, (const int *)far_list)
        if (mb == 8) DCD_LAUNCH_BW(8);
        else if (mb == 4) DCD_LAUNCH_BW(4);
        else if (mb == 2) DCD_LAUNCH_BW(2);
        else DCD_LAUNCH_BW(1);
#undef DCD_LAUNCH_BW
    }
    return hipGetLastError() == hipSuccess ? DCD_OK : DCD_ERR_LAUNCH;
}

#ifdef SW_PROFILE
int dcd_debug_sweep_profile(unsigned long long *host_out)
{
    return hipMemcpyFromSymbol(host_out, HIP_SYMBOL(sw_prof_buf), sizeof(unsigned long long) * 2048) == hipSuccess ? 0 : 1;
}
#endif

int dcd_dcn_v2_forget(const float *weight)
{
    int dev = 0;
    if (hipGetDevice(&dev) != hipSuccess) return DCD_ERR_LAUNCH;
    std::lock_guard<std::mutex> lock(g_handover_mu);
    int n = 0;
    for (auto it = g_handover.begin(); it != g_handover.end();) {
        if (it->first.first == dev && (!weight || it->first.second == (const void *)weight)) {
            if (it->second.host) {
                *(volatile unsigned *)it->second.host = HANDOVER_UNKNOWN;
                g_handover_free[dev].push_back(it->second);
            }
            it = g_handover.erase(it);
            ++n;
        } else {
            ++it;
        }
    }
    (void)n;
    return DCD_OK;
}

int dcd_dcn_v2_policy_state(const float *weight, unsigned *far_count)
{
    int dev = 0;
    if (!weight || hipGetDevice(&dev) != hipSuccess) return -1;
    std::lock_guard<std::mutex> lock(g_handover_mu);
    auto it = g_handover.find(std::make_pair(dev, (const void *)weight));
    if (it == g_handover.end() || !it->second.host) return 0;
    const unsigned far = *(volatile unsigned *)it->second.host;
    if (far == HANDOVER_UNKNOWN) return 1;
    if (far_count) *far_count = far;
    return 2;
}

int dcd_dcn_v2_set_handover(int mode)
{
    if (mode < -1 || mode > 2) return DCD_ERR_BAD_ARG;
    g_handover_pin.store(mode, std::memory_order_relaxed);
    return DCD_OK;
}

int dcd_dcn_v2_policy_free(void)
{
    std::lock_guard<std::mutex> lock(g_handover_mu);
    for (auto &kv : g_handover)
        if (kv.second.host) (void)hipHostFree(kv.second.host);
    g_handover.clear();
    for (auto &kv : g_handover_free)
        for (HandoverState &h : kv.second)
            if (h.host) (void)hipHostFree(h.host);
    g_handover_free.clear();
    (void)hipGetLastError();
    return DCD_OK;
}

int dcd_dcn_offset_mask_split(void *stream_, const float *out, float *offset, float *mask, int B, int taps, int64_t HW)
{
    (void)hipGetLastError();
    if (!out || !offset || !mask || B <= 0 || taps <= 0 || HW <= 0) return DCD_ERR_BAD_ARG;
    const bool v4 = (HW & 3) == 0 && (((uintptr_t)out | (uintptr_t)offset | (uintptr_t)mask) & 15) == 0;
    const int64_t n = (int64_t)B * 3 * taps * HW / (v4 ? 4 : 1);
    const unsigned grid = (unsigned)((n + 255) / 256 < 8192 ? (n + 255) / 256 : 8192);
    if (v4) hipLaunchKernelGGL(dcn_offset_mask_split<4>, dim3(grid), dim3(256), 0, (hipStream_t)stream_, out, offset, mask, B, taps, HW);
    else hipLaunchKernelGGL(dcn_offset_mask_split<1>, dim3(grid), dim3(256), 0, (hipStream_t)stream_, out, offset, mask, B, taps, HW);
    return hipGetLastError() == hipSuccess ? DCD_OK : DCD_ERR_LAUNCH;
}

int dcd_dcn_offset_mask_merge(void *stream_, const float *grad_offset, const float *grad_mask, const float *mask, float *grad_out, int B,
                              int taps, int64_t HW)
{
    (void)hipGetLastError();
    if (!grad_offset || !grad_mask || !mask || !grad_out || B <= 0 || taps <= 0 || HW <= 0) return DCD_ERR_BAD_ARG;
    const bool v4 = (HW & 3) == 0 &&
                    (((uintptr_t)grad_offset | (uintptr_t)grad_mask | (uintptr_t)mask | (uintptr_t)grad_out) & 15) == 0;
    const int64_t n = (int64_t)B * 3 * taps * HW / (v4 ? 4 : 1);
    const unsigned grid = (unsigned)((n + 255) / 256 < 8192 ? (n + 255) / 256 : 8192);
    if (v4)
        hipLaunchKernelGGL(dcn_offset_mask_merge<4>, dim3(grid), dim3(256), 0, (hipStream_t)stream_, grad_offset, grad_mask, mask, grad_out,
                           B, taps, HW);
    else
        hipLaunchKernelGGL(dcn_offset_mask_merge<1>, dim3(grid), dim3(256), 0, (hipStream_t)stream_, grad_offset, grad_mask, mask, grad_out,
                           B, taps, HW);
    return hipGetLastError() == hipSuccess ? DCD_OK : DCD_ERR_LAUNCH;
}

int dcd_sgemm_shifted(void *stream_, const float *A, int lda, long long strideA, const float *Bbase, const long long *b_off,
                      long long strideB, int b_kcontig, const float *bias, float *C, int ldc, long long strideC,
                      long long strideCs, int M, int N, int K, int Z, int nsplit)
{
    (void)hipGetLastError();
    if (!A || !Bbase || !b_off || !C || M <= 0 || N <= 0 || K <= 0 || Z <= 0 || nsplit <= 0 || (lda & 3) || ((uintptr_t)A & 15) ||
        (strideA & 3) || (bias && nsplit != 1))
        return DCD_ERR_BAD_ARG;
    SgemmArgs a;
    a.A = A; a.B = Bbase; a.C = C; a.bias = bias; a.M = M; a.N = N; a.K = K; a.lda = lda; a.ldb = 0; a.ldc = ldc;
    a.strideA = strideA; a.strideB = strideB; a.strideC = strideC; a.strideCs = strideCs;
    a.nsplit = nsplit; a.kchunk = ((K + nsplit - 1) / nsplit + SG_K - 1) / SG_K * SG_K; a.ct = 0; a.b_off = b_off;
    if ((long long)a.kchunk * (nsplit - 1) >= K) return DCD_ERR_BAD_ARG;
    sgemm_f32_rows64((hipStream_t)stream_, b_kcontig != 0, a, Z);
    return hipGetLastError() == hipSuccess ? DCD_OK : DCD_ERR_LAUNCH;
}

}
```

dcd_amd/csrc/norm.hip:

```cpp
#include <hip/hip_runtime.h>
#include <stdint.h>
#include <stdlib.h>

#include "../../include/dcd_hip.h"
#include "tuning_env.h"

namespace {

constexpr int BT = 256;
constexpr int CH = 4096;
constexpr int SMAX = 256;

__device__ inline double wave_sum(double v)
{
#pragma unroll
    for (int o = 32; o; o >>= 1) v += __shfl_down(v, o);
    return v;
}

__device__ inline float bn_shift(float bias, float mean, float scale) { return fmaf(-mean, scale, bias); }

__device__ inline void block_sum2(double &a, double &b)
{
    __shared__ double sh[2][BT / 64];
    a = wave_sum(a);
    b = wave_sum(b);
    const int w = threadIdx.x >> 6;
    if ((threadIdx.x & 63) == 0) { sh[0][w] = a; sh[1][w] = b; }
    __syncthreads();
    if (threadIdx.x == 0) {
        a = sh[0][0]; b = sh[1][0];
#pragma unroll
        for (int i = 1; i < BT / 64; ++i) { a += sh[0][i]; b += sh[1][i]; }
    }
}

__device__ inline void channel_sums(const double *__restrict__ combined, const double *__restrict__ partial, int S, int c,
                                    double &s0, double &s1)
{
    if (!partial) { s0 = combined[2 * c]; s1 = combined[2 * c + 1]; return; }
    __shared__ double bc[2];
    if (threadIdx.x < 64) {
        double a = 0.0, b = 0.0;
        for (int s = threadIdx.x; s < S; s += 64) {
            a += partial[((long)c * S + s) * 2 + 0];
            b += partial[((long)c * S + s) * 2 + 1];
        }
        a = wave_sum(a);
        b = wave_sum(b);
        if (threadIdx.x == 0) { bc[0] = a; bc[1] = b; }
    }
    __syncthreads();
    s0 = bc[0];
    s1 = bc[1];
}

struct Plane {
// ... 506 lines not shown
}

__global__ __launch_bounds__(256) void trunk_finalize_fwd(const double *__restrict__ sums, const float *__restrict__ gamma,
                                                          const float *__restrict__ beta, double n, double eps, int R,
                                                          float *__restrict__ scale, float *__restrict__ shift, double *__restrict__ stats)
{
    const int r = blockIdx.x * blockDim.x + threadIdx.x;
    if (r >= R) return;
    const double mean = sums[2 * r] / n;
    const double raw = sums[2 * r + 1] / n - mean * mean;
    const double var = raw > 0.0 ? raw : 0.0;
    const double invstd = 1.0 / sqrt(var + eps);
    const double sc = (double)gamma[r] * invstd;
    scale[r] = (float)sc;
    shift[r] = (float)((double)beta[r] - mean * sc);
    stats[3 * r] = mean;
    stats[3 * r + 1] = var;
    stats[3 * r + 2] = invstd;
}

__global__ __launch_bounds__(256) void trunk_finalize_bwd(const float *__restrict__ dscale, const float *__restrict__ dshift,
                                                          const float *__restrict__ gamma, const double *__restrict__ stats, double n, int R,
                                                          double *__restrict__ dsums, float *__restrict__ dgamma, float *__restrict__ dbeta)
{
    const int r = blockIdx.x * blockDim.x + threadIdx.x;
    if (r >= R) return;
    const double mean = stats[3 * r], var = stats[3 * r + 1], invstd = stats[3 * r + 2];
    const double ds = dscale[r], dh = dshift[r], g = gamma[r];
    dgamma[r] = (float)((ds - dh * mean) * invstd);
    dbeta[r] = (float)dh;
    const double dinv = (ds - dh * mean) * g;
    double dmean = -dh * g * invstd;
    const double dvar = var > 0.0 ? dinv * -0.5 * invstd * invstd * invstd : 0.0;
    dmean += dvar * -2.0 * mean;
    dsums[2 * r] = dmean / n;
    dsums[2 * r + 1] = dvar / n;
}

__global__ __launch_bounds__(256) void trunk_dwg(const double *__restrict__ dsums, const double *__restrict__ Wd, int R, int K,
                                                 double *__restrict__ dWG)
{
    const long n = (long)R * (K + 1);
    for (long i = (long)blockIdx.x * blockDim.x + threadIdx.x; i < n; i += (long)gridDim.x * blockDim.x) {
        const long r = i / (K + 1);
        const int k = (int)(i - r * (K + 1));
        dWG[i] = k < K ? dsums[2 * r + 1] * Wd[r * K + k] : dsums[2 * r];
    }
}

inline bool bad_shape(int B, int C, long HW) { return B <= 0 || C <= 0 || HW <= 0 || C > 65535 || (double)B * ((HW + CH - 1) / CH) > 2.0e9; }

}

extern "C" {

size_t dcd_bn_workspace_bytes(int C) { return C > 0 ? (size_t)C * SMAX * 2 * sizeof(double) : 0; }

int dcd_bn_stats(void *stream_, const float *x, int B, int C, int64_t HW, double *stats, void *ws, size_t ws_bytes)
{
    hipStream_t stream = (hipStream_t)stream_;
    (void)hipGetLastError();
    if (!x || !stats || bad_shape(B, C, HW)) return DCD_ERR_BAD_ARG;
    if (!ws || ws_bytes < dcd_bn_workspace_bytes(C)) return DCD_ERR_WORKSPACE;
    const Plane g = make_plane(B, C, HW);
    const int S = sync_slices(g);
    if (S == 1) {
        hipLaunchKernelGGL(bn_partial, dim3(1, C), dim3(BT), 0, stream, x, g, 1, stats);
    } else {
        hipLaunchKernelGGL(bn_partial, dim3(S, C), dim3(BT), 0, stream, x, g, S, (double *)ws);
        hipLaunchKernelGGL(bn_combine, dim3(C), dim3(64), 0, stream, (const double *)ws, S, stats, (const float *)nullptr, (float *)nullptr,
                           (float *)nullptr);
    }
    return hipGetLastError() == hipSuccess ? DCD_OK : DCD_ERR_LAUNCH;
}

int dcd_channel_sums(void *stream_, const float *x, int B, int C, int64_t HW, float *sums, void *ws, size_t ws_bytes)
{
    hipStream_t stream = (hipStream_t)stream_;
    (void)hipGetLastError();
    if (!x || !sums || bad_shape(B, C, HW)) return DCD_ERR_BAD_ARG;
    if (!ws || ws_bytes < dcd_bn_workspace_bytes(C)) return DCD_ERR_WORKSPACE;
    const Plane g = make_plane(B, C, HW);
    const int S = slices(g);
    unsigned *arrivals = reinterpret_cast<unsigned *>(reinterpret_cast<double *>(ws) + (size_t)C * SMAX);
    static const int pin = dcd_env("DCD_CHANNEL_SUM_ONE_LAUNCH") ? atoi(dcd_env("DCD_CHANNEL_SUM_ONE_LAUNCH")) : -1;
    const bool one = pin >= 0 ? pin != 0 : (long)S * C <= 256;
    if (one) {
        hipLaunchKernelGGL(channel_sum_kernel, dim3(S, C), dim3(BT), 0, stream, x, g, S, (double *)ws, arrivals, sums);
    } else {
        hipLaunchKernelGGL(channel_sum_kernel, dim3(S, C), dim3(BT), 0, stream, x, g, S, (double *)ws, (unsigned *)nullptr, sums);
        hipLaunchKernelGGL(channel_sum_combine, dim3(C), dim3(64), 0, stream, (const double *)ws, S, sums);
    }
    return hipGetLastError() == hipSuccess ? DCD_OK : DCD_ERR_LAUNCH;
}

int dcd_bn_train_apply(void *stream_, const float *x, const float *residual, const float *weight, const float *bias,
                       const double *stats, double count, float *running_mean, float *running_var,
                       int64_t *num_batches_tracked, float momentum, float eps, int relu, float *y, float *save_mean,
                       float *save_invstd, int B, int C, int64_t HW)
{
    hipStream_t stream = (hipStream_t)stream_;
    (void)hipGetLastError();
    if (!x || !y || !stats || !save_mean || !save_invstd || bad_shape(B, C, HW) || !(count >= 1.0)) return DCD_ERR_BAD_ARG;
    if ((running_mean == nullptr) != (running_var == nullptr)) return DCD_ERR_BAD_ARG;
    const Plane g = make_plane(B, C, HW);
    hipLaunchKernelGGL(bn_apply, dim3(B * g.cpp, C), dim3(BT), 0, stream, x, residual, weight, bias, stats, (const double *)nullptr, 0,
// ... 236 lines not shown
```

dcd_amd/model/backbone/DCNv2/dcn_v2.py:

```python
import math
import os

import torch
from torch import nn
from torch.autograd import Function
from torch.autograd.function import once_differentiable
from torch.nn.modules.utils import _pair

from dcd_amd import _ext as _backend
from dcd_amd.model.layers.conv import Conv2d


def _precision_scope():
    from dcd_amd import _ext
    return _ext.get_precision()


class _DCNv2(Function):

    @staticmethod
    def forward(ctx, input, offset, mask, weight, bias, stride, padding, dilation, deformable_groups, precision=None):
        kernel = tuple(weight.shape[2:4])
        ctx.geometry = (*kernel, *_pair(stride), *_pair(padding), *_pair(dilation), int(deformable_groups))
        p = _precision_scope() if precision is None else precision
# ... 2 lines not shown
        return _backend.dcn_v2_forward(input, weight, bias, offset, mask, *ctx.geometry, **ctx.precision)

    @staticmethod
    @once_differentiable
    def backward(ctx, grad_output):
        input, offset, mask, weight, bias = ctx.saved_tensors
        grads = _backend.dcn_v2_backward(input.contiguous(), weight.contiguous(), bias, offset, mask, grad_output.contiguous(),
                                         *ctx.geometry, **ctx.precision)
        grad_input, grad_offset, grad_mask, grad_weight, grad_bias = grads
        return (grad_input, grad_offset, grad_mask, grad_weight, grad_bias) + (None,) * 5


_FUSED_GLUE = os.environ.get("DCD_OFFSET_MASK_FUSED", "1") != "0"


def _offset_mask_split(out):
    from dcd_amd import _lib
    B, C3, H, W = out.shape
    T = C3 // 3
    offset = torch.empty((B, 2 * T, H, W), dtype=out.dtype, device=out.device)
    mask = torch.empty((B, T, H, W), dtype=out.dtype, device=out.device)
    st = _lib.lib().dcd_dcn_offset_mask_split(_lib.stream_of(out), out.data_ptr(), offset.data_ptr(), mask.data_ptr(), B, T, H * W)
    _lib.check(st, "dcd_dcn_offset_mask_split")
    return offset, mask


def _offset_mask_merge(goff, gmask, mask):
    from dcd_amd import _lib
    B, T, H, W = mask.shape
    goff, gmask = goff.contiguous(), gmask.contiguous()
    gout = torch.empty((B, 3 * T, H, W), dtype=mask.dtype, device=mask.device)
    st = _lib.lib().dcd_dcn_offset_mask_merge(_lib.stream_of(mask), goff.data_ptr(), gmask.data_ptr(), mask.data_ptr(),
                                              gout.data_ptr(), B, T, H * W)
    _lib.check(st, "dcd_dcn_offset_mask_merge")
    return gout


class _OffsetMask(torch.autograd.Function):

    @staticmethod
    def forward(ctx, out):
        offset, mask = _offset_mask_split(out)
        ctx.save_for_backward(mask)
        return offset, mask

    @staticmethod
    @torch.autograd.function.once_differentiable
    def backward(ctx, goff, gmask):
        (mask,) = ctx.saved_tensors
        return _offset_mask_merge(goff, gmask, mask)


_ONE_NODE = os.environ.get("DCD_DCN_NODE", "1") != "0"


class _DCNWithOffsets(Function):

    @staticmethod
    def forward(ctx, input, w_off, b_off, weight, bias, geometry):
        from dcd_amd import ops
        input, w_off, weight = input.contiguous(), w_off.contiguous(), weight.contiguous()
        ctx.cprec = ops._conv_prec(input)
        p = _precision_scope()
        ctx.precision = {} if p == "f32" else {"precision": p}
        tw, ctx.tw_back = (ops.conv3x3_step_weights(w_off, input) if ops._PREP_BOTH and ctx.needs_input_grad[0] else (None, None))
        out = ops._conv3x3_call(input, w_off, w_off.shape[0], False, b_off.contiguous(), transformed=tw, prec=ctx.cprec)
        offset, mask = _offset_mask_split(out)
        ctx.geometry = geometry
        ctx.save_for_backward(input, offset, mask, weight, bias, w_off)
        return _backend.dcn_v2_forward(input, weight, bias, offset, mask, *geometry, **ctx.precision)

    @staticmethod
    @once_differentiable
    def backward(ctx, grad_output):
        from dcd_amd import ops
        input, offset, mask, weight, bias, w_off = ctx.saved_tensors
        grad_input, grad_offset, grad_mask, grad_weight, grad_bias = _backend.dcn_v2_backward(
            input, weight, bias, offset, mask, grad_output.contiguous(), *ctx.geometry, **ctx.precision)
        gout = _offset_mask_merge(grad_offset, grad_mask, mask)
        if ctx.needs_input_grad[0]:
            grad_input = ops._conv3x3_call(gout, w_off, w_off.shape[1], True, residual=grad_input.contiguous(), transformed=ctx.tw_back,
                                           prec=ctx.cprec)
        gw_off = ops._conv3x3_wrw_call(input, gout, w_off.shape, ctx.cprec) if ctx.needs_input_grad[1] else None
        gb_off = ops.channel_sums(gout) if ctx.needs_input_grad[2] else None
        return grad_input, gw_off, gb_off, grad_weight, grad_bias, None


def dcn_v2_conv(input, offset, mask, weight, bias, stride, padding, dilation, deformable_groups):
    dev = input.device.type
    if torch.is_autocast_enabled(dev):
        with torch.autocast(device_type=dev, enabled=False):
            args = (input.float(), offset.float(), mask.float(), weight.float(), bias.float(), stride, padding, dilation,
                    deformable_groups)
            return _DCNv2.apply(*args, "bf16") if input.is_cuda else _DCNv2.apply(*args)
    return _DCNv2.apply(input, offset, mask, weight, bias, stride, padding, dilation, deformable_groups)


class DCNv2(nn.Module):
    def __init__(self, in_channels, out_channels, kernel_size, stride, padding, dilation=1, deformable_groups=1):
        super().__init__()
        self.in_channels = in_channels
        self.out_channels = out_channels
        self.kernel_size = _pair(kernel_size)
        self.stride = _pair(stride)
        self.padding = _pair(padding)
        self.dilation = _pair(dilation)
        self.deformable_groups = deformable_groups
        self.weight = nn.Parameter(torch.empty(out_channels, in_channels, *self.kernel_size))
        self.bias = nn.Parameter(torch.empty(out_channels))
        self.reset_parameters()

    def reset_parameters(self):
        fan_in = self.in_channels * self.kernel_size[0] * self.kernel_size[1]
        bound = 1.0 / math.sqrt(fan_in)
        self.weight.data.uniform_(-bound, bound)
        self.bias.data.zero_()

    def _forget_policy(self):
        w = self._parameters.get("weight") if hasattr(self, "_parameters") else None
        if w is None or not w.is_cuda:
            return
        try:
            from dcd_amd import _lib
            with torch.cuda.device(w.device):
                _lib.lib().dcd_dcn_v2_forget(w.data_ptr())
        except Exception:
            pass

    def _apply(self, fn, *args, **kwargs):
        self._forget_policy()
        return super()._apply(fn, *args, **kwargs)

    def __del__(self):
        self._forget_policy()

    def forward(self, input, offset, mask):
        taps = self.deformable_groups * self.kernel_size[0] * self.kernel_size[1]
# ... 37 lines not shown
```

dcd_amd/ops.py:

```python
import os

import torch

from . import _lib


def _f32c(t):
    if t.dtype != torch.float32:
        t = t.float()
    return t.contiguous()


class _PairsDepth(torch.autograd.Function):
    @staticmethod
    def forward(ctx, kps, kps3d, rot_y, P, kmask, topk, zmin, zmax, normalized, sub_b3):
        _lib.require_cuda(kps, kps3d, rot_y, P)
        L = _lib.lib()
        kps, kps3d, P = _f32c(kps), _f32c(kps3d), _f32c(P)
        rot = _f32c(rot_y).reshape(-1)
        N, K = kps.shape[0], kps.shape[1]
        npairs = K * (K - 1) // 2
        M = topk if topk else npairs
        dev = kps.device
        depth = torch.empty((N, M), dtype=torch.float32, device=dev)
# ... 786 lines not shown
    return _conv_prec(like) != PREC_F32


def _wrw_prec(prec):
    return PREC_BF16 if prec == PREC_BF16 else PREC_F32


class SplitWeights:

    def __init__(self, tensor, prec):
        self.tensor = tensor
        self.prec = prec


class Bf16Weights(SplitWeights):

    def __init__(self, tensor):
        super().__init__(tensor, PREC_BF16)


_BF16_DIRECT = os.environ.get("DCD_CONV_BF16_DIRECT", "1") != "0"


def _layout(prec):
    if prec == PREC_F32:
        return "f32"
    return "bf16" if prec == PREC_BF16 and _BF16_DIRECT else "split"


def conv3x3_transform_weights(weight, forward=True, backward=True, like=None, prec=None):
    L = _lib.lib()
    Co, Ci = weight.shape[0], weight.shape[1]
    prec = _conv_prec(like) if prec is None else prec
    if _layout(prec) == "bf16":
        tf = torch.empty(L.dcd_conv3x3_bf16_weights_bytes(Ci, Co, 0) // 4, dtype=torch.int32, device=weight.device) if forward else None
        tb = torch.empty(L.dcd_conv3x3_bf16_weights_bytes(Ci, Co, 1) // 4, dtype=torch.int32, device=weight.device) if backward else None
        _lib.check(L.dcd_conv3x3_bf16_transform_weights(_lib.stream_of(weight), weight.data_ptr(), Ci, Co, _lib.ptr(tf), _lib.ptr(tb)),
                   "dcd_conv3x3_bf16_transform_weights")
        return (Bf16Weights(tf) if forward else None), (Bf16Weights(tb) if backward else None)
    if prec != PREC_F32:
        tf = torch.empty(L.dcd_conv3x3_split_weights_bytes(Ci, Co, 0) // 4, dtype=torch.int32, device=weight.device) if forward else None
        tb = torch.empty(L.dcd_conv3x3_split_weights_bytes(Ci, Co, 1) // 4, dtype=torch.int32, device=weight.device) if backward else None
        _lib.check(L.dcd_conv3x3_split_transform_weights(_lib.stream_of(weight), weight.data_ptr(), Ci, Co, _lib.ptr(tf), _lib.ptr(tb)),
                   "dcd_conv3x3_split_transform_weights")
        return (SplitWeights(tf, prec) if forward else None), (SplitWeights(tb, prec) if backward else None)
    tf = torch.empty(L.dcd_conv3x3_weights_bytes(Ci, Co, 0) // 4, dtype=torch.float32, device=weight.device) if forward else None
    tb = torch.empty(L.dcd_conv3x3_weights_bytes(Ci, Co, 1) // 4, dtype=torch.float32, device=weight.device) if backward else None
    _lib.check(L.dcd_conv3x3_transform_weights(_lib.stream_of(weight), weight.data_ptr(), Ci, Co, _lib.ptr(tf), _lib.ptr(tb)),
               "dcd_conv3x3_transform_weights")
    return tf, tb


def _conv3x3_call(inp, weight, out_channels, backward_data, bias=None, residual=None, transformed=None, residual_inplace=True,
                  prec=None):
    L = _lib.lib()
    B, _, H, W = inp.shape
    Co, Ci = weight.shape[0], weight.shape[1]
    if residual is not None:
        if tuple(residual.shape) != (B, out_channels, H, W) or residual.dtype != torch.float32 or not residual.is_contiguous():
            raise RuntimeError("conv3x3: residual must be a contiguous fp32 tensor of the output's shape")
        out = residual if residual_inplace else torch.empty_like(residual)
    else:
        out = torch.empty((B, out_channels, H, W), dtype=torch.float32, device=inp.device)
    if transformed is None:
        prec = _conv_prec(inp) if prec is None else prec
        if prec != PREC_F32:
            transformed = conv3x3_transform_weights(weight, not backward_data, backward_data, prec=prec)[1 if backward_data else 0]
    if isinstance(transformed, Bf16Weights):
        n = L.dcd_conv3x3_bf16_workspace_bytes(B, Ci, H, W, Co)
        ws = torch.empty(max(n, 16), dtype=torch.uint8, device=inp.device)
        st = L.dcd_conv3x3_bf16_prepared(_lib.stream_of(inp), inp.data_ptr(), transformed.tensor.data_ptr(), _lib.ptr(bias),
                                         _lib.ptr(residual), out.data_ptr(), B, Ci, H, W, Co, 1 if backward_data else 0, ws.data_ptr(), n)
        _lib.check(st, "dcd_conv3x3_bf16_prepared")
        return out
    if isinstance(transformed, SplitWeights):
        n = L.dcd_conv3x3_split_workspace_bytes(B, Ci, H, W, Co)
        ws = torch.empty(max(n, 16), dtype=torch.uint8, device=inp.device)
        st = L.dcd_conv3x3_split_prepared(_lib.stream_of(inp), inp.data_ptr(), transformed.tensor.data_ptr(), _lib.ptr(bias),
                                          _lib.ptr(residual), out.data_ptr(), B, Ci, H, W, Co, 1 if backward_data else 0,
                                          transformed.prec, ws.data_ptr(), n)
        _lib.check(st, "dcd_conv3x3_split_prepared")
        return out
    n = L.dcd_conv3x3_workspace_bytes(B, Ci, H, W, Co)
    if transformed is not None:
        n = max(n - min(L.dcd_conv3x3_weights_bytes(Ci, Co, 0), L.dcd_conv3x3_weights_bytes(Ci, Co, 1)), 0)
        ws = torch.empty(max(n, 16), dtype=torch.uint8, device=inp.device)
        st = L.dcd_conv3x3_prepared(_lib.stream_of(inp), inp.data_ptr(), transformed.data_ptr(), _lib.ptr(bias), _lib.ptr(residual),
                                    out.data_ptr(), B, Ci, H, W, Co, 1 if backward_data else 0, ws.data_ptr(), n)
        _lib.check(st, "dcd_conv3x3_prepared")
        return out
    ws = torch.empty(n, dtype=torch.uint8, device=inp.device)
    st = L.dcd_conv3x3(_lib.stream_of(inp), inp.data_ptr(), weight.data_ptr(), _lib.ptr(bias), _lib.ptr(residual), out.data_ptr(),
                       B, Ci, H, W, Co,
                       1 if backward_data else 0, ws.data_ptr(), n)
    _lib.check(st, "dcd_conv3x3")
    return out


_PREP_BOTH = os.environ.get("DCD_CONV_PREP_BOTH", "1") != "0"
_PREP_TABLE = os.environ.get("DCD_CONV_PREP_TABLE", "1") != "0"


class _PreparedWeights:

    def __init__(self, split=False):
        self.split = split
        self.entries = {}
        self.table = None
        self.order = []
        self.dirty = False
        self.captured = False
        self._immortal = []

    def lookup(self, weight):
        e = self.entries.get(id(weight))
        if e is None or e[0]() is not weight or e[1] != weight.data_ptr() or e[4] != weight._version:
            return None
        if not self.captured and torch.cuda.is_current_stream_capturing():
            self.captured = True
        e[5] = 0
        return e

    def register(self, weight):
        import weakref
        if not _PREP_TABLE or torch.cuda.is_current_stream_capturing() or not isinstance(weight, torch.nn.Parameter):
            return
        e = self.entries.get(id(weight))
        if e is not None and e[0]() is weight and e[1] == weight.data_ptr():
            return
        L = _lib.lib()
        Co, Ci = weight.shape[0], weight.shape[1]
        if self.split == "bf16":
            tf = torch.empty(L.dcd_conv3x3_bf16_weights_bytes(Ci, Co, 0) // 4, dtype=torch.int32, device=weight.device)
            tb = torch.empty(L.dcd_conv3x3_bf16_weights_bytes(Ci, Co, 1) // 4, dtype=torch.int32, device=weight.device)
        elif self.split:
            tf = torch.empty(L.dcd_conv3x3_split_weights_bytes(Ci, Co, 0) // 4, dtype=torch.int32, device=weight.device)
            tb = torch.empty(L.dcd_conv3x3_split_weights_bytes(Ci, Co, 1) // 4, dtype=torch.int32, device=weight.device)
        else:
            tf = torch.empty(L.dcd_conv3x3_weights_bytes(Ci, Co, 0) // 4, dtype=torch.float32, device=weight.device)
            tb = torch.empty(L.dcd_conv3x3_weights_bytes(Ci, Co, 1) // 4, dtype=torch.float32, device=weight.device)
        self.entries[id(weight)] = [weakref.ref(weight), weight.data_ptr(), tf, tb, -1, 0]
        self.dirty = True

    def refresh(self):
        if not self.entries or not _PREP_TABLE:
            return
        dead = [k for k, e in self.entries.items() if e[0]() is None or e[0]().data_ptr() != e[1] or e[5] >= 3]
        if (dead or self.dirty) and torch.cuda.is_current_stream_capturing():
            return
        if torch.cuda.is_current_stream_capturing():
            self.captured = True
# ... 754 lines not shown
```

include/dcd_hip.h:

```cpp
#ifndef DCD_HIP_H
#define DCD_HIP_H

#include <stddef.h>
#include <stdint.h>

#ifdef __cplusplus
extern "C" {
#endif

#define DCD_OK 0
#define DCD_ERR_BAD_ARG 1
#define DCD_ERR_WORKSPACE 2
#define DCD_ERR_LAUNCH 3

const char *dcd_version(void);


#define DCD_PREC_F32 0
#define DCD_PREC_BF16X3 1
#define DCD_PREC_BF16 2

size_t dcd_dcn_v2_workspace_bytes(int B, int Cin, int H, int W, int Cout, int kh, int kw, int sh, int sw,
                                  int ph, int pw, int dh, int dw, int dg);

int dcd_dcn_v2_forward(void *stream, const float *input, const float *weight, const float *bias,
                       const float *offset, const float *mask, float *output, int B, int Cin, int H, int W,
                       int Cout, int kh, int kw, int sh, int sw, int ph, int pw, int dh, int dw, int dg,
                       int precision, void *workspace, size_t workspace_bytes);

int dcd_dcn_v2_backward(void *stream, const float *input, const float *weight, const float *bias,
                        const float *offset, const float *mask, const float *grad_output, float *grad_input,
                        float *grad_offset, float *grad_mask, float *grad_weight, float *grad_bias, int B,
                        int Cin, int H, int W, int Cout, int kh, int kw, int sh, int sw, int ph, int pw, int dh,
                        int dw, int dg, int precision, void *workspace, size_t workspace_bytes);

int dcd_dcn_v2_forget(const float *weight);
int dcd_dcn_v2_policy_state(const float *weight, unsigned *far_count);
int dcd_dcn_v2_policy_free(void);
int dcd_dcn_v2_set_handover(int mode);

int dcd_edge_depth_forward(void *stream, const float *kps, const float *kps3d, const float *rot_y,
                           const float *P, const uint8_t *kmask, int N, int K, int topk, float zmin,
                           float zmax, int normalized, int sub_b3, float *depth, int32_t *pair_idx,
                           float *pair_mask);

int dcd_edge_depth_backward(void *stream, const float *kps, const float *kps3d, const float *rot_y,
                            const float *P, const float *grad_depth, const int32_t *pair_idx, int N, int K,
                            int topk, float zmin, float zmax, int normalized, float *grad_kps,
                            float *grad_kps3d);

int dcd_focal_loss(void *stream, const float *pred, const float *target, int64_t n, float alpha, float beta,
                   float *out, float *grad_pred);

int dcd_giou_loss(void *stream, const float *pred, const float *target, int N, float *losses, float *ious,
                  float *grad_pred);

int dcd_nms_hm(void *stream, const float *heat, int B, int C, int H, int W, float *out);
int dcd_heatmap_topk(void *stream, const float *heat, int B, int C, int H, int W, int K, int fuse_nms,
                     float *scores, int64_t *inds, float *clses, float *ys, float *xs, void *workspace,
                     size_t workspace_bytes);
size_t dcd_heatmap_topk_workspace_bytes(int B, int C, int H, int W, int K);

int dcd_poi_gather(void *stream, const float *feat, const int64_t *index, int B, int C, int H, int W, int M,
                   float *out);
int dcd_poi_scatter_add(void *stream, const float *grad_out, const int64_t *index, int B, int C, int H, int W,
                        int M, float *grad_feat);
int dcd_patch_scatter_add(void *stream, const float *grad_patches, const int64_t *base, int B, int C, int64_t plane, int pitch, int M,
                          float *out);

int dcd_iou3d(void *stream, const float *pred_corners, const float *target_corners, int N, float *iou);

#define DCD_HEADS_MAX 16
typedef struct dcd_head_rows_args {
    int n_heads, T, R, K, C;
    int trunk[DCD_HEADS_MAX], ch0[DCD_HEADS_MAX], out[DCD_HEADS_MAX];
    const float *weight[DCD_HEADS_MAX];
    const float *bias[DCD_HEADS_MAX];
    const float *feat;
    float *y;
    const float *grad_y;
    float *grad_feat;
    float *grad_weight[DCD_HEADS_MAX];
    float *grad_bias[DCD_HEADS_MAX];
} dcd_head_rows_args;

int dcd_head_rows_forward(void *stream, const dcd_head_rows_args *args);
int dcd_head_rows_backward(void *stream, const dcd_head_rows_args *args);
// ... 77 lines not shown
int dcd_bn_backward_stats(void *stream, const float *grad_y, const float *y, const float *x, const float *save_mean,
                          int B, int C, int64_t HW, double *sums, void *workspace, size_t workspace_bytes);
int dcd_bn_backward_relu_from_x(void *stream, const float *grad_y, const float *x, const float *weight, const float *bias,
                                const float *save_mean, const float *save_invstd, float *grad_x, float *grad_weight, float *grad_bias,
                                int B, int C, int64_t HW, void *workspace, size_t workspace_bytes);
int dcd_bn_backward_stats_params_relu_from_x(void *stream, const float *grad_y, const float *x, const float *weight, const float *bias,
                                             const float *save_mean, const float *save_invstd, int B, int C, int64_t HW, double *sums,
                                             float *grad_weight, float *grad_bias, void *workspace, size_t workspace_bytes);
int dcd_bn_backward_apply_relu_from_x(void *stream, const float *grad_y, const float *x, const float *weight, const float *bias,
                                      const float *save_mean, const float *save_invstd, const double *sums, double count, float *grad_x,
                                      int B, int C, int64_t HW);
int dcd_bn_backward_stats_params(void *stream, const float *grad_y, const float *y, const float *x, const float *save_mean,
                                 const float *save_invstd, int B, int C, int64_t HW, double *sums, float *grad_weight,
                                 float *grad_bias, void *workspace, size_t workspace_bytes);
int dcd_bn_backward_apply(void *stream, const float *grad_y, const float *y, const float *x, const float *weight,
                          const float *save_mean, const float *save_invstd, const double *sums, double count,
                          float *grad_x, float *grad_residual, float *grad_weight, float *grad_bias, int B, int C,
                          int64_t HW);
int dcd_trunk_row_sums(void *stream, const double *WG, const double *Wd, int R, int K, double *sums);
int dcd_trunk_finalize_forward(void *stream, const double *sums, const float *gamma, const float *beta, double count, double eps, int R,
                               float *scale, float *shift, double *stats);
int dcd_trunk_finalize_backward(void *stream, const float *grad_scale, const float *grad_shift, const float *gamma, const double *stats,
                                double count, int R, double *grad_sums, float *grad_gamma, float *grad_beta);
int dcd_trunk_grad_wg(void *stream, const double *grad_sums, const double *Wd, int R, int K, double *grad_WG);

int dcd_bn_at_forward(void *stream, const float *x, const int64_t *pos, const float *weight, const float *bias,
                      const double *stats, double count, float *running_mean, float *running_var,
                      int64_t *num_batches_tracked, float momentum, float eps, int relu, float *x_at, float *y_at,
                      float *save_mean, float *save_invstd, int B, int C, int64_t HW, int N, void *workspace,
                      size_t workspace_bytes);
int dcd_bn_at_backward_sums(void *stream, const float *grad_at, const float *x_at, const float *y_at, const float *weight,
                            const float *save_mean, const float *save_invstd, int relu, int total, int C, double *sums,
                            float *dzk);
int dcd_bn_train_forward(void *stream, const float *x, const float *residual, const float *weight, const float *bias,
                         float *running_mean, float *running_var, int64_t *num_batches_tracked, float momentum, float eps,
                         int relu, float *y, float *save_mean, float *save_invstd, int B, int C, int64_t HW,
                         void *workspace, size_t workspace_bytes);
int dcd_bn_backward(void *stream, const float *grad_y, const float *y, const float *x, const float *weight,
                    const float *save_mean, const float *save_invstd, float *grad_x, float *grad_residual,
                    float *grad_weight, float *grad_bias, int B, int C, int64_t HW, void *workspace,
                    size_t workspace_bytes);

size_t dcd_conv3x3_workspace_bytes(int B, int Cin, int H, int W, int Cout);
int dcd_conv3x3(void *stream, const float *input, const float *weight, const float *bias, const float *residual, float *output,
                int B, int Cin, int H, int W, int Cout, int backward_data, void *workspace, size_t workspace_bytes);

size_t dcd_conv3x3_weights_bytes(int Cin, int Cout, int backward_data);
int dcd_conv3x3_transform_weights(void *stream, const float *weight, int Cin, int Cout, float *forward_out, float *backward_out);
int dcd_conv3x3_transform_weights_table(void *stream, const long long *table, int entries);
int dcd_conv3x3_prepared(void *stream, const float *input, const float *transformed, const float *bias, const float *residual,
                         float *output, int B, int Cin, int H, int W, int Cout, int backward_data, void *workspace,
                         size_t workspace_bytes);

size_t dcd_conv3x3_split_weights_bytes(int Cin, int Cout, int backward_data);
int dcd_conv3x3_split_transform_weights(void *stream, const float *weight, int Cin, int Cout, void *forward_out, void *backward_out);
int dcd_conv3x3_split_transform_weights_table(void *stream, const long long *table, int entries);
size_t dcd_conv3x3_split_workspace_bytes(int B, int Cin, int H, int W, int Cout);
int dcd_conv3x3_split_prepared(void *stream, const float *input, const void *transformed, const float *bias, const float *residual,
                               float *output, int B, int Cin, int H, int W, int Cout, int backward_data, int precision, void *workspace,
                               size_t workspace_bytes);

size_t dcd_conv3x3_bf16_weights_bytes(int Cin, int Cout, int backward_data);
int dcd_conv3x3_bf16_transform_weights(void *stream, const float *weight, int Cin, int Cout, void *forward_out, void *backward_out);
int dcd_conv3x3_bf16_transform_weights_table(void *stream, const long long *table, int entries);
size_t dcd_conv3x3_bf16_workspace_bytes(int B, int Cin, int H, int W, int Cout);
int dcd_conv3x3_bf16_prepared(void *stream, const float *input, const void *transformed, const float *bias, const float *residual,
                              float *output, int B, int Cin, int H, int W, int Cout, int backward_data, void *workspace,
                              size_t workspace_bytes);

int dcd_conv1x1_bf16(void *stream, const float *weight, int ldw, int transposed, int n_inputs, const float *const *inputs,
                     const int *channels, float *output, int B, int M, long long HW);
size_t dcd_conv1x1_wrw_bf16_workspace_bytes(int B, int O, int C, long long HW);
int dcd_conv1x1_wrw_bf16(void *stream, const float *grad_output, const float *input, float *grad_weight, int ldw, int B, int O, int C,
                         long long HW, void *workspace, size_t workspace_bytes);

int dcd_conv1x1_f32(void *stream, const float *weight, int ldw, int transposed, int n_inputs, const float *const *inputs,
                    const int *channels, float *output, int B, int M, long long HW);
size_t dcd_conv1x1_wrw_f32_workspace_bytes(int B, int O, int C, long long HW);
int dcd_conv1x1_wrw_f32(void *stream, const float *grad_output, const float *input, float *grad_weight, int ldw, int B, int O, int C,
                        long long HW, void *workspace, size_t workspace_bytes);

int dcd_conv3x3_s2_f32(void *stream, const float *input, const float *weight, float *output, int B, int Cin, int H, int W, int Cout);
int dcd_conv3x3_s2_f32_backward_data(void *stream, const float *grad_output, const float *weight, float *grad_input, int B, int Cin, int H,
                                     int W, int Cout);
size_t dcd_conv3x3_s2_f32_wrw_workspace_bytes(int B, int Cin, int H, int W, int Cout);
int dcd_conv3x3_s2_f32_wrw(void *stream, const float *input, const float *grad_output, float *grad_weight, int B, int Cin, int H, int W,
                           int Cout, void *workspace, size_t workspace_bytes);

size_t dcd_conv3x3_wrw_workspace_bytes(int B, int Cin, int H, int W, int Cout);
int dcd_conv3x3_wrw(void *stream, const float *input, const float *grad_output, float *grad_weight, int B, int Cin, int H, int W,
                    int Cout, int precision, void *workspace, size_t workspace_bytes);

size_t dcd_conv_stem_workspace_bytes(int Cin, int Cout, int ksize);
int dcd_conv_stem(void *stream, const float *input, const float *weight, float *output, int B, int Cin, int H, int W, int Cout,
                  int ksize, int backward_data, void *workspace, size_t workspace_bytes);
size_t dcd_conv_stem_wrw_workspace_bytes(int Cin, int Cout, int ksize);
int dcd_conv_stem_wrw(void *stream, const float *input, const float *grad_output, float *grad_weight, int B, int Cin, int H, int W,
                      int Cout, int ksize, void *workspace, size_t workspace_bytes);

int dcd_upsample_dw_forward(void *stream, const float *x, const float *weight, float *y, int B, int C, int H, int W, int f);
int dcd_upsample_dw_forward_add(void *stream, const float *x, const float *weight, const float *skip, float *y, int B, int C, int H,
                                int W, int f);

int dcd_maxpool2x2_forward(void *stream, const float *x, float *y, int64_t planes, int H, int W);
int dcd_maxpool2x2_backward(void *stream, const float *x, const float *grad_y, float *grad_x, int64_t planes, int H, int W);
int dcd_upsample_dw_backward(void *stream, const float *x, const float *weight, const float *grad_y, float *grad_x,
// ... 87 lines not shown
```

Baseline: 220.3 images/s.

## Fuse DCN offset/mask split and sigmoid into conv epilogue; merge backward gradient assembly

In the forward pass, the offset/mask 3x3 conv epilogue now writes offset channels and sigmoid-activated mask channels directly into separate tensors, replacing a separate split kernel. In the backward pass, a new merged path reduces the coordinate partials into the concatenated offset/mask gradient, applies the mask derivative, and accumulates the bias channel sums in the same kernel. This removes the separate merge and channel_sums launches and the intermediate tensors they write and read. The cost is more special-casing in the conv kernel epilogue, plus a fallback path for plans that do not meet the fusion conditions (nb==1, no k-split).

```diff
diff --git a/dcd_amd/_ext.py b/dcd_amd/_ext.py
--- a/dcd_amd/_ext.py
+++ b/dcd_amd/_ext.py
@@ -101,7 +101,7 @@
 
 
 def dcn_v2_backward(input, weight, bias, offset, mask, grad_output, kernel_h, kernel_w, stride_h, stride_w,
-                    pad_h, pad_w, dilation_h, dilation_w, deformable_group, precision=None):
+                    pad_h, pad_w, dilation_h, dilation_w, deformable_group, precision=None, merged=False):
     _check(input, weight, bias, offset, mask, kernel_h, kernel_w)
     _lib.require_cuda(grad_output)
     if not input.is_contiguous():
@@ -116,6 +116,9 @@
     if grad_output.dtype != torch.float32:
         raise RuntimeError("grad_output must be float32")
     bias, offset, mask, grad_output = (t.contiguous() for t in (bias, offset, mask, grad_output))
+    if merged:
+        return _dcn_v2_backward_merged(input, weight, bias, offset, mask, grad_output, kernel_h, kernel_w, stride_h, stride_w,
+                                       pad_h, pad_w, dilation_h, dilation_w, deformable_group, precision)
     geom = (B, C, H, W, Co, kernel_h, kernel_w, stride_h, stride_w, pad_h, pad_w, dilation_h, dilation_w,
             deformable_group)
     ws, nbytes = _workspace(L, input, geom)
@@ -131,3 +134,23 @@
                                grad_weight.data_ptr(), grad_bias.data_ptr(), *geom, prec, ws.data_ptr(), nbytes)
     _lib.check(st, "dcd_dcn_v2_backward")
     return [grad_input, grad_offset, grad_mask, grad_weight, grad_bias]
+
+
+def _dcn_v2_backward_merged(input, weight, bias, offset, mask, grad_output, kernel_h, kernel_w, stride_h, stride_w,
+                            pad_h, pad_w, dilation_h, dilation_w, deformable_group, precision=None):
+    L = _lib.lib()
+    B, C, H, W, Co, Ho, Wo = _dims(input, weight, kernel_h, kernel_w, stride_h, stride_w, pad_h, pad_w, dilation_h, dilation_w)
+    geom = (B, C, H, W, Co, kernel_h, kernel_w, stride_h, stride_w, pad_h, pad_w, dilation_h, dilation_w, deformable_group)
+    ws, nbytes = _workspace(L, input, geom)
+    taps = deformable_group * kernel_h * kernel_w
+    grad_input = torch.empty_like(input)
+    grad_out = torch.empty((B, 3 * taps, Ho, Wo), dtype=torch.float32, device=input.device)
+    grad_out_bias = torch.empty(3 * taps, dtype=torch.float32, device=input.device)
+    grad_weight = torch.empty_like(weight)
+    grad_bias = torch.empty_like(bias)
+    prec = PRECISION[precision or get_precision()]
+    st = L.dcd_dcn_v2_backward_merged(_lib.stream_of(input), input.data_ptr(), weight.data_ptr(), offset.data_ptr(), mask.data_ptr(),
+                                      grad_output.data_ptr(), grad_input.data_ptr(), grad_out.data_ptr(), grad_out_bias.data_ptr(),
+                                      grad_weight.data_ptr(), grad_bias.data_ptr(), *geom, prec, ws.data_ptr(), nbytes)
+    _lib.check(st, "dcd_dcn_v2_backward_merged")
+    return [grad_input, grad_out, grad_out_bias, grad_weight, grad_bias]
diff --git a/dcd_amd/_lib.py b/dcd_amd/_lib.py
--- a/dcd_amd/_lib.py
+++ b/dcd_amd/_lib.py
@@ -61,6 +61,7 @@
     "dcd_dcn_v2_workspace_bytes": (c_size_t, [c_int] * 14),
     "dcd_dcn_v2_forward": (c_int, [c_void_p] * 7 + [c_int] * 15 + [c_void_p, c_size_t]),
     "dcd_dcn_v2_backward": (c_int, [c_void_p] * 12 + [c_int] * 15 + [c_void_p, c_size_t]),
+    "dcd_dcn_v2_backward_merged": (c_int, [c_void_p] * 11 + [c_int] * 15 + [c_void_p, c_size_t]),
     "dcd_dcn_v2_forget": (c_int, [c_void_p]),
     "dcd_dcn_v2_policy_state": (c_int, [c_void_p, c_void_p]),
     "dcd_dcn_v2_policy_free": (c_int, []),
@@ -84,6 +85,8 @@
     "dcd_conv3x3_transform_weights": (c_int, [c_void_p, c_void_p, c_int, c_int, c_void_p, c_void_p]),
     "dcd_conv3x3_transform_weights_table": (c_int, [c_void_p, c_void_p, c_int]),
     "dcd_conv3x3_prepared": (c_int, [c_void_p] * 6 + [c_int] * 6 + [c_void_p, c_size_t]),
+    "dcd_conv3x3_offset_mask_workspace_bytes": (c_size_t, [c_int] * 6),
+    "dcd_conv3x3_offset_mask": (c_int, [c_void_p, c_void_p, c_void_p, c_int] + [c_void_p] * 3 + [c_int] * 6 + [c_void_p, c_size_t]),
     "dcd_conv3x3_split_weights_bytes": (c_size_t, [c_int] * 3),
     "dcd_conv3x3_split_transform_weights": (c_int, [c_void_p, c_void_p, c_int, c_int, c_void_p, c_void_p]),
     "dcd_conv3x3_split_transform_weights_table": (c_int, [c_void_p, c_void_p, c_int]),
diff --git a/dcd_amd/csrc/channel_sum.h b/dcd_amd/csrc/channel_sum.h
--- /dev/null
+++ b/dcd_amd/csrc/channel_sum.h
@@ -0,0 +1,13 @@
+#pragma once
+#include <hip/hip_runtime.h>
+
+#include <cstddef>
+#include <cstdint>
+
+namespace dcd_internal {
+
+void channel_sum_combine_launch(hipStream_t stream, const double *partial, int S, int C, float *out);
+
+int channel_sums_two_launch(hipStream_t stream, const float *x, int B, int C, int64_t HW, float *sums, void *ws, size_t ws_bytes);
+
+}
diff --git a/dcd_amd/csrc/conv.hip b/dcd_amd/csrc/conv.hip
--- a/dcd_amd/csrc/conv.hip
+++ b/dcd_amd/csrc/conv.hip
@@ -135,7 +135,7 @@
 __global__ __launch_bounds__(WN_NT) void wino_conv3x3_f32(const float *__restrict__ x, const float *__restrict__ ul, float *y,
                                                           float *__restrict__ part, const float *__restrict__ bias,
                                                           const float *residual, int Cc, int H, int W, int Kk, int tiles_x,
-                                                          int nchunk, int nz)
+                                                          int nchunk, int nz, float *__restrict__ mask_out, int split_at)
 {
     using G = WinoGeom<TR, TC, NB>;
     constexpr int WN_ROWS = G::ROWS, WN_RS = G::RS, WN_PLANE = G::PLANE, WN_IN = G::IN, WN_BUF = G::BUF, WN_Q = G::Q;
@@ -297,8 +297,21 @@
                         if (orow0 < H) r0 += *reinterpret_cast<const f32x2 *>(r_b + o);
                         if (orow0 + 1 < H) r1 += *reinterpret_cast<const f32x2 *>(r_b + o + W);
                     }
-                    if (orow0 < H) *reinterpret_cast<f32x2 *>(dst) = f32x2{a0 + a1 + a2 + r0.x, b0 + b1 + b2 + r0.y};
-                    if (orow0 + 1 < H) *reinterpret_cast<f32x2 *>(dst + W) = f32x2{a1 - a2 - a3 + r1.x, b1 - b2 - b3 + r1.y};
+                    f32x2 v0 = {a0 + a1 + a2 + r0.x, b0 + b1 + b2 + r0.y}, v1 = {a1 - a2 - a3 + r1.x, b1 - b2 - b3 + r1.y};
+                    if constexpr (NB == 1) {
+                        if (mask_out) {
+                            const size_t pix = (size_t)orow0 * W + ocol;
+                            if (k < split_at) {
+                                dst = y + ((size_t)b * split_at + k) * HW + pix;
+                            } else {
+                                dst = mask_out + ((size_t)b * (Kk - split_at) + (k - split_at)) * HW + pix;
+                                v0.x = 1.f / (1.f + __expf(-v0.x)); v0.y = 1.f / (1.f + __expf(-v0.y));
+                                v1.x = 1.f / (1.f + __expf(-v1.x)); v1.y = 1.f / (1.f + __expf(-v1.y));
+                            }
+                        }
+                    }
+                    if (orow0 < H) *reinterpret_cast<f32x2 *>(dst) = v0;
+                    if (orow0 + 1 < H) *reinterpret_cast<f32x2 *>(dst + W) = v1;
                 }
             }
         }
@@ -926,14 +939,15 @@
 
 template <int TR, int TC, int NB>
 static int conv_launch(hipStream_t stream, const ConvPlan &pl, const float *input, const float *ul, float *output, float *part,
-                       const float *bias, const float *residual, int B, int Cc, int H, int W, int Kk)
+                       const float *bias, const float *residual, int B, int Cc, int H, int W, int Kk, float *mask_out = nullptr,
+                       int split_at = 0)
 {
     static LdsLimit lds_limit;
     size_t ldsb = (size_t)2 * WinoGeom<TR, TC, NB>::BUF * sizeof(float);
     if (ldsb < (size_t)8 * 32 * 64 * sizeof(float)) ldsb = (size_t)8 * 32 * 64 * sizeof(float);
     if (!lds_limit.raise((int)ldsb, wino_conv3x3_f32<TR, TC, NB>)) return DCD_ERR_LAUNCH;
     hipLaunchKernelGGL((wino_conv3x3_f32<TR, TC, NB>), dim3(pl.tiles_x * pl.tiles_y, B, pl.nz * pl.ksplit), dim3(WN_NT), ldsb, stream,
-                       input, ul, output, part, bias, residual, Cc, H, W, Kk, pl.tiles_x, pl.nchunk, pl.nz);
+                       input, ul, output, part, bias, residual, Cc, H, W, Kk, pl.tiles_x, pl.nchunk, pl.nz, mask_out, split_at);
     return DCD_OK;
 }
 
@@ -1044,14 +1058,8 @@
     return (nchunk * nz * 16 * 64 * WN_CH + (pf > pd ? pf : pd)) * sizeof(float);
 }
 
-static int conv3x3_run(hipStream_t stream, const float *input, const float *weights, int prepared, const float *bias,
-                       const float *residual, float *output, int B, int Cin, int H, int W, int Cout, int backward_data, void *workspace,
-                       size_t workspace_bytes)
-{
-    (void)hipGetLastError();
-    if (!input || !weights || !output || B <= 0 || Cin <= 0 || Cout <= 0 || H <= 0 || W <= 0) return DCD_ERR_BAD_ARG;
-    if ((W & 3) || (H & 1) || (int64_t)(Cin > Cout ? Cin : Cout) * H * W >= (1ll << 31) || (bias && backward_data)) return DCD_ERR_BAD_ARG;
-    const int Cc = backward_data ? Cout : Cin, Kk = backward_data ? Cin : Cout;
+static ConvPlan conv_plan_of_call(int B, int Cc, int H, int W, int Kk)
+{
     ConvPlan pl = conv_plan(B, Cc, H, W, Kk);
     if (const char *e = dcd_env("DCD_CONV_GEOM")) {
         const int g = atoi(e);
@@ -1064,6 +1072,19 @@
             pl = q;
         }
     }
+    return pl;
+}
+
+static int conv3x3_run(hipStream_t stream, const float *input, const float *weights, int prepared, const float *bias,
+                       const float *residual, float *output, int B, int Cin, int H, int W, int Cout, int backward_data, void *workspace,
+                       size_t workspace_bytes, float *mask_out = nullptr, int split_at = 0)
+{
+    (void)hipGetLastError();
+    if (!input || !weights || !output || B <= 0 || Cin <= 0 || Cout <= 0 || H <= 0 || W <= 0) return DCD_ERR_BAD_ARG;
+    if ((W & 3) || (H & 1) || (int64_t)(Cin > Cout ? Cin : Cout) * H * W >= (1ll << 31) || (bias && backward_data)) return DCD_ERR_BAD_ARG;
+    const int Cc = backward_data ? Cout : Cin, Kk = backward_data ? Cin : Cout;
+    const ConvPlan pl = conv_plan_of_call(B, Cc, H, W, Kk);
+    if (mask_out && (pl.nb != 1 || pl.ksplit != 1 || backward_data || residual)) return DCD_ERR_BAD_ARG;
     const int ksz = 32 * pl.nb;
     const size_t ul_floats = prepared ? 0 : (size_t)pl.nchunk * pl.nz * 16 * ksz * WN_CH;
     const size_t img = (size_t)B * Kk * H * W;
@@ -1078,9 +1099,11 @@
         ul = (const float *)workspace;
     }
     const int st = pl.geom == 0 ? (pl.nb == 2 ? conv_launch<2, 16, 2>(stream, pl, input, ul, output, part, bias, residual, B, Cc, H, W, Kk)
-                                              : conv_launch<2, 16, 1>(stream, pl, input, ul, output, part, bias, residual, B, Cc, H, W, Kk))
+                                              : conv_launch<2, 16, 1>(stream, pl, input, ul, output, part, bias, residual, B, Cc, H, W, Kk,
+                                                                      mask_out, split_at))
                                 : (pl.nb == 2 ? conv_launch<3, 10, 2>(stream, pl, input, ul, output, part, bias, residual, B, Cc, H, W, Kk)
-                                              : conv_launch<3, 10, 1>(stream, pl, input, ul, output, part, bias, residual, B, Cc, H, W, Kk));
+                                              : conv_launch<3, 10, 1>(stream, pl, input, ul, output, part, bias, residual, B, Cc, H, W, Kk,
+                                                                      mask_out, split_at));
     if (st != DCD_OK) return st;
     if (pl.ksplit > 1) {
         const size_t n4 = img / 4;
@@ -1296,6 +1319,58 @@
     return hipGetLastError() == hipSuccess ? DCD_OK : DCD_ERR_LAUNCH;
 }
 
+static bool offset_conv_fuses(int B, int Cin, int H, int W, int taps, int weights_form)
+{
+    if (weights_form != DCD_CONV_WEIGHTS_RAW && weights_form != DCD_CONV_WEIGHTS_F32) return false;
+    const ConvPlan pl = conv_plan_of_call(B, Cin, H, W, 3 * taps);
+    return pl.nb == 1 && pl.ksplit == 1;
+}
+
+static size_t offset_conv_image_bytes(int B, int H, int W, int taps) { return ((size_t)B * 3 * taps * H * W * sizeof(float) + 255) / 256 * 256; }
+
+size_t dcd_conv3x3_offset_mask_workspace_bytes(int B, int Cin, int H, int W, int taps, int weights_form)
+{
+    if (B <= 0 || Cin <= 0 || taps <= 0 || H <= 0 || W <= 0) return 0;
+    const int Cout = 3 * taps;
+    size_t inner;
+    if (weights_form == DCD_CONV_WEIGHTS_SPLIT) inner = dcd_conv3x3_split_workspace_bytes(B, Cin, H, W, Cout);
+    else if (weights_form == DCD_CONV_WEIGHTS_BF16) inner = dcd_conv3x3_bf16_workspace_bytes(B, Cin, H, W, Cout);
+    else if (weights_form == DCD_CONV_WEIGHTS_RAW || weights_form == DCD_CONV_WEIGHTS_F32) inner = dcd_conv3x3_workspace_bytes(B, Cin, H, W, Cout);
+    else return 0;
+    return (offset_conv_fuses(B, Cin, H, W, taps, weights_form) ? 0 : offset_conv_image_bytes(B, H, W, taps)) + inner + 16;
+}
+
+int dcd_conv3x3_offset_mask(void *stream_, const float *input, const void *weights, int weights_form, const float *bias, float *offset,
+                            float *mask, int B, int Cin, int H, int W, int taps, int precision, void *workspace, size_t workspace_bytes)
+{
+    if (!input || !weights || !bias || !offset || !mask || !workspace || B <= 0 || Cin <= 0 || taps <= 0 || H <= 0 || W <= 0)
+        return DCD_ERR_BAD_ARG;
+    const bool f32 = weights_form == DCD_CONV_WEIGHTS_RAW || weights_form == DCD_CONV_WEIGHTS_F32;
+    if (f32 ? precision != DCD_PREC_F32
+            : weights_form == DCD_CONV_WEIGHTS_SPLIT ? (precision != DCD_PREC_BF16X3 && precision != DCD_PREC_BF16)
+                                                     : (weights_form != DCD_CONV_WEIGHTS_BF16 || precision != DCD_PREC_BF16))
+        return DCD_ERR_BAD_ARG;
+    if (workspace_bytes < dcd_conv3x3_offset_mask_workspace_bytes(B, Cin, H, W, taps, weights_form)) return DCD_ERR_WORKSPACE;
+    const int Cout = 3 * taps;
+    if (offset_conv_fuses(B, Cin, H, W, taps, weights_form))
+        return conv3x3_run((hipStream_t)stream_, input, (const float *)weights, weights_form == DCD_CONV_WEIGHTS_F32, bias, nullptr, offset, B,
+                           Cin, H, W, Cout, 0, workspace, workspace_bytes, mask, 2 * taps);
+    const size_t img = offset_conv_image_bytes(B, H, W, taps);
+    float *out = (float *)workspace;
+    void *inner = (char *)workspace + img;
+    const size_t inner_bytes = workspace_bytes - img;
+    int st;
+    if (weights_form == DCD_CONV_WEIGHTS_SPLIT)
+        st = dcd_conv3x3_split_prepared(stream_, input, weights, bias, nullptr, out, B, Cin, H, W, Cout, 0, precision, inner, inner_bytes);
+    else if (weights_form == DCD_CONV_WEIGHTS_BF16)
+        st = dcd_conv3x3_bf16_prepared(stream_, input, weights, bias, nullptr, out, B, Cin, H, W, Cout, 0, inner, inner_bytes);
+    else
+        st = conv3x3_run((hipStream_t)stream_, input, (const float *)weights, weights_form == DCD_CONV_WEIGHTS_F32, bias, nullptr, out, B, Cin,
+                         H, W, Cout, 0, inner, inner_bytes);
+    if (st != DCD_OK) return st;
+    return dcd_dcn_offset_mask_split(stream_, out, offset, mask, B, taps, (int64_t)H * W);
+}
+
 int dcd_conv1x1_bf16(void *stream_, const float *weight, int ldw, int transposed, int n_inputs, const float *const *inputs,
                      const int *channels, float *output, int B, int M, long long HW)
 {
diff --git a/dcd_amd/csrc/dcn_bwd_sweep.inc b/dcd_amd/csrc/dcn_bwd_sweep.inc
--- a/dcd_amd/csrc/dcn_bwd_sweep.inc
+++ b/dcd_amd/csrc/dcn_bwd_sweep.inc
@@ -837,6 +837,52 @@
     }
 }
 
+__device__ __forceinline__ void sweep_reduce_coord_merged_body(const float *__restrict__ cpart, const float *__restrict__ mask,
+                                                               float *__restrict__ gout, float *__restrict__ zoff,
+                                                               float *__restrict__ zmsk, double *__restrict__ bias_part, int B, int HW,
+                                                               int nck, const unsigned *__restrict__ far_scal, int total_tiles, int bid,
+                                                               int nseg, int seg4)
+{
+    const int plane = bid / nseg, s = bid - plane * nseg;
+    const int b = plane / 27, p = plane - b * 27;
+    const int hw4 = HW / 4;
+    const int lo = s * seg4, hi = lo + seg4 < hw4 ? lo + seg4 : hw4;
+    if (far_dominated(far_scal, total_tiles)) {
+        if (!zoff) return;
+        f32x4 *dst = reinterpret_cast<f32x4 *>(p < 18 ? zoff + ((size_t)b * 18 + p) * HW : zmsk + ((size_t)b * 9 + (p - 18)) * HW);
+        const f32x4 zero4 = {0.f, 0.f, 0.f, 0.f};
+        for (int i = lo + threadIdx.x; i < hi; i += blockDim.x) dst[i] = zero4;
+        return;
+    }
+    const size_t stride4 = (size_t)B * 27 * hw4;
+    const f32x4 *src = reinterpret_cast<const f32x4 *>(cpart) + (size_t)plane * hw4;
+    const f32x4 *m4 = p >= 18 ? reinterpret_cast<const f32x4 *>(mask + ((size_t)b * 9 + (p - 18)) * HW) : nullptr;
+    f32x4 *dst = reinterpret_cast<f32x4 *>(gout) + (size_t)plane * hw4;
+    float fs = 0.f;
+    for (int i = lo + threadIdx.x; i < hi; i += blockDim.x) {
+        f32x4 v = src[i];
+        for (int ck = 1; ck < nck; ++ck) {
+            const f32x4 u = src[i + ck * stride4];
+            v.x += u.x; v.y += u.y; v.z += u.z; v.w += u.w;
+        }
+        if (m4) {
+            const f32x4 m = m4[i];
+#pragma unroll
+            for (int j = 0; j < 4; ++j) v[j] = v[j] * m[j] * (1.f - m[j]);
+        }
+        dst[i] = v;
+        fs += (v.x + v.y) + (v.z + v.w);
+    }
+    if (!bias_part) return;
+    double d = (double)fs;
+#pragma unroll
+    for (int o = 32; o > 0; o >>= 1) d += __shfl_xor(d, o);
+    __shared__ double wsum[4];
+    if ((threadIdx.x & 63) == 0) wsum[threadIdx.x >> 6] = d;
+    __syncthreads();
+    if (threadIdx.x == 0) bias_part[(size_t)p * ((size_t)B * nseg) + (size_t)b * nseg + s] = (wsum[0] + wsum[1]) + (wsum[2] + wsum[3]);
+}
+
 __device__ __forceinline__ void sweep_reduce_dw_body(const float *__restrict__ part, float *__restrict__ gw, float *__restrict__ gbias,
                                                      const Geom &g, int nck, int nvp, const unsigned *__restrict__ far_scal,
                                                      int total_tiles, int bx, int nbx, int by, int nby)
@@ -886,6 +932,10 @@
     int nck, nvp, total_tiles, nb_coord, bias_splits, dw_bx, dw_by, gemm_n, gemm_S;
     unsigned *far_report = nullptr;
     unsigned far_base = 0;
+    float *gout = nullptr;
+    const float *mask = nullptr;
+    double *bias_part = nullptr;
+    int coord_nseg = 0, coord_seg4 = 0;
 };
 __global__ __launch_bounds__(256) void dcn_sweep_epilogue(SweepEpilogueArgs a)
 {
@@ -895,6 +945,11 @@
         *a.far_report = c >= a.far_base ? c - a.far_base : 0u;
     }
     if (bid < a.nb_coord) {
+        if (a.gout) {
+            sweep_reduce_coord_merged_body(a.cpart, a.mask, a.gout, a.goff, a.gmsk, a.bias_part, a.g.B, a.g.HoWo, a.nck, a.far_scal,
+                                           a.total_tiles, bid, a.coord_nseg, a.coord_seg4);
+            return;
+        }
         sweep_reduce_coord_body(a.cpart, a.goff, a.gmsk, a.g.B, a.g.HoWo, a.nck, a.far_scal, a.total_tiles, bid, a.nb_coord);
         return;
     }
diff --git a/dcd_amd/csrc/dcn_v2.hip b/dcd_amd/csrc/dcn_v2.hip
--- a/dcd_amd/csrc/dcn_v2.hip
+++ b/dcd_amd/csrc/dcn_v2.hip
@@ -12,6 +12,7 @@
 #include "../../include/dcd_hip.h"
 #include "tuning_env.h"
 #include "lds_limit.h"
+#include "channel_sum.h"
 
 typedef float f32x16 __attribute__((ext_vector_type(16)));
 typedef float f32x32 __attribute__((ext_vector_type(32)));
@@ -2045,8 +2046,10 @@
 
 template <int V>
 __global__ void dcn_offset_mask_merge(const float *__restrict__ goff, const float *__restrict__ gmask, const float *__restrict__ mask,
-                                      float *__restrict__ gout, int B, int T, int64_t HW)
-{
+                                      float *__restrict__ gout, int B, int T, int64_t HW, const unsigned *__restrict__ only_if_far = nullptr,
+                                      int total_tiles = 0)
+{
+    if (only_if_far && !far_dominated(only_if_far, total_tiles)) return;
     const int64_t per_img = (int64_t)3 * T * HW / V, n = (int64_t)B * per_img;
     for (int64_t i = (int64_t)blockIdx.x * blockDim.x + threadIdx.x; i < n; i += (int64_t)gridDim.x * blockDim.x) {
         const int64_t b = i / per_img, r = (i - b * per_img) * V;
@@ -2102,12 +2105,48 @@
     return (n + 255) / 256 * 256 + blockmax_bytes(g);
 }
 
+struct MergedPlan {
+    int nseg, seg4;
+    size_t scratch_bytes, bias_bytes;
+};
+static MergedPlan merged_plan(const Geom &g)
+{
+    MergedPlan m;
+    const int T = g.dg * g.KK;
+    const int64_t hw4 = g.HoWo / 4;
+    int64_t nseg = (hw4 + 511) / 512, cap = 4096 / ((int64_t)g.B * 3 * T);
+    if (cap < 1) cap = 1;
+    if (nseg > cap) nseg = cap;
+    if (nseg < 1) nseg = 1;
+    m.nseg = (int)nseg;
+    m.seg4 = (int)((hw4 + nseg - 1) / nseg);
+    m.scratch_bytes = ((size_t)g.B * 3 * T * g.HoWo * sizeof(float) + 255) / 256 * 256;
+    const size_t own = (size_t)3 * T * g.B * m.nseg * sizeof(double), sums = dcd_bn_workspace_bytes(3 * T);
+    m.bias_bytes = ((own > sums ? own : sums) + 255) / 256 * 256;
+    return m;
+}
+
+static void launch_offset_mask_merge(hipStream_t stream, const float *goff, const float *gmask, const float *mask, float *gout, int B,
+                                     int taps, int64_t HW, const unsigned *only_if_far, int total_tiles)
+{
+    const bool v4 = (HW & 3) == 0 && (((uintptr_t)goff | (uintptr_t)gmask | (uintptr_t)mask | (uintptr_t)gout) & 15) == 0;
+    const int64_t n = (int64_t)B * 3 * taps * HW / (v4 ? 4 : 1);
+    const unsigned grid = (unsigned)((n + 255) / 256 < 8192 ? (n + 255) / 256 : 8192);
+    if (v4)
+        hipLaunchKernelGGL(dcn_offset_mask_merge<4>, dim3(grid), dim3(256), 0, stream, goff, gmask, mask, gout, B, taps, HW, only_if_far,
+                           total_tiles);
+    else
+        hipLaunchKernelGGL(dcn_offset_mask_merge<1>, dim3(grid), dim3(256), 0, stream, goff, gmask, mask, gout, B, taps, HW, only_if_far,
+                           total_tiles);
+}
+
 size_t dcd_dcn_v2_workspace_bytes(int B, int Cin, int H, int W, int Cout, int kh, int kw, int sh, int sw, int ph,
                                   int pw, int dh, int dw, int dg)
 {
     Geom g;
     if (!make_geom(g, B, Cin, H, W, Cout, kh, kw, sh, sw, ph, pw, dh, dw, dg)) return 0;
-    return base_workspace_bytes(g) + dense_workspace_bytes(g) + sweep_workspace_bytes(g);
+    const MergedPlan m = merged_plan(g);
+    return (base_workspace_bytes(g) + dense_workspace_bytes(g) + sweep_workspace_bytes(g) + 255) / 256 * 256 + m.scratch_bytes + m.bias_bytes;
 }
 
 int dcd_dcn_v2_forward(void *stream_, const float *input, const float *weight, const float *bias,
@@ -2249,26 +2288,44 @@
     return hipGetLastError() == hipSuccess ? DCD_OK : DCD_ERR_LAUNCH;
 }
 
-int dcd_dcn_v2_backward(void *stream_, const float *input, const float *weight, const float *bias,
-                        const float *offset, const float *mask, const float *grad_output, float *grad_input,
-                        float *grad_offset, float *grad_mask, float *grad_weight, float *grad_bias, int B,
-                        int Cin, int H, int W, int Cout, int kh, int kw, int sh, int sw, int ph, int pw, int dh,
-                        int dw, int dg, int precision, void *workspace, size_t workspace_bytes)
-{
-    (void)bias;
+static int dcn_v2_backward_run(void *stream_, const float *input, const float *weight, const float *offset, const float *mask,
+                               const float *grad_output, float *grad_input, float *grad_offset, float *grad_mask, float *grad_out,
+                               float *grad_out_bias, float *grad_weight, float *grad_bias, int B, int Cin, int H, int W, int Cout, int kh,
+                               int kw, int sh, int sw, int ph, int pw, int dh, int dw, int dg, int precision, void *workspace,
+                               size_t workspace_bytes)
+{
     hipStream_t stream = (hipStream_t)stream_;
     (void)hipGetLastError();
     Geom g;
-    if (!input || !weight || !offset || !mask || !grad_output || !grad_input || !grad_offset || !grad_mask ||
-        !grad_weight || !grad_bias || !workspace)
+    if (!input || !weight || !offset || !mask || !grad_output || !grad_input || !grad_weight || !grad_bias || !workspace)
         return DCD_ERR_BAD_ARG;
+    if (grad_out ? !grad_out_bias : (!grad_offset || !grad_mask)) return DCD_ERR_BAD_ARG;
     if (!make_geom(g, B, Cin, H, W, Cout, kh, kw, sh, sw, ph, pw, dh, dw, dg)) return DCD_ERR_BAD_ARG;
     if (precision != DCD_PREC_F32 && precision != DCD_PREC_BF16X3 && precision != DCD_PREC_BF16) return DCD_ERR_BAD_ARG;
     const bool split = precision != DCD_PREC_F32;
     const bool one = precision == DCD_PREC_BF16;
     const size_t nw = (size_t)g.Kp * g.Cop;
-    if (workspace_bytes + 256 < dcd_dcn_v2_workspace_bytes(B, Cin, H, W, Cout, kh, kw, sh, sw, ph, pw, dh, dw, dg))
-        return DCD_ERR_WORKSPACE;
+    const size_t ws_total = dcd_dcn_v2_workspace_bytes(B, Cin, H, W, Cout, kh, kw, sh, sw, ph, pw, dh, dw, dg);
+    if (workspace_bytes + 256 < ws_total) return DCD_ERR_WORKSPACE;
+    const MergedPlan mp = merged_plan(g);
+    const int taps3 = 3 * g.dg * g.KK;
+    double *bias_ws = nullptr;
+    if (grad_out) {
+        if (workspace_bytes < ws_total) return DCD_ERR_WORKSPACE;
+        if ((((uintptr_t)mask | (uintptr_t)grad_out) & 15) != 0) return DCD_ERR_BAD_ARG;
+        grad_offset = (float *)((char *)workspace + (ws_total - mp.scratch_bytes - mp.bias_bytes));
+        grad_mask = grad_offset + (size_t)g.B * 2 * g.dg * g.KK * g.HoWo;
+        bias_ws = (double *)((char *)workspace + (ws_total - mp.bias_bytes));
+    }
+    auto finish = [&](const unsigned *merge_only_if_far) -> int {
+        if (grad_out) {
+            launch_offset_mask_merge(stream, grad_offset, grad_mask, mask, grad_out, g.B, g.dg * g.KK, g.HoWo, merge_only_if_far,
+                                     g.B * ((g.HoWo + 31) / 32));
+            const int st = dcd_internal::channel_sums_two_launch(stream, grad_out, g.B, taps3, g.HoWo, grad_out_bias, bias_ws, mp.bias_bytes);
+            if (st != DCD_OK) return st;
+        }
+        return hipGetLastError() == hipSuccess ? DCD_OK : DCD_ERR_LAUNCH;
+    };
     float *wf = (float *)workspace, *wb = wf + nw;
     const size_t cells = (size_t)B * dg * g.KK * H * W;
     InvLists inv;
@@ -2319,7 +2376,7 @@
         hipLaunchKernelGGL(dcn_bias_grad, dim3(Cout, splits), dim3(256), 0, stream, grad_output, grad_bias, B, Cout, g.HoWo);
         dense_backward(stream, input, wb, offset, mask, grad_output, grad_input, grad_offset, grad_mask, grad_weight, g, inv,
                        (float *)((char *)workspace + base_workspace_bytes(g)), precision);
-        return hipGetLastError() == hipSuccess ? DCD_OK : DCD_ERR_LAUNCH;
+        return finish(nullptr);
     }
     const int tiles = (g.HoWo + 31) / 32;
     const int nblk = g.cpgp / 32;
@@ -2390,6 +2447,12 @@
             e.bias_only_if_far = sp.nob == 1 ? fs : (const unsigned *)nullptr;
             const int64_t n4 = (int64_t)B * 27 * g.HoWo / 4;
             e.nb_coord = (int)((n4 + 255) / 256 < 4096 ? (n4 + 255) / 256 : 4096);
+            if (grad_out) {
+                e.gout = grad_out; e.mask = mask;
+                if (!handover) { e.goff = nullptr; e.gmsk = nullptr; e.bias_part = bias_ws; }
+                e.coord_nseg = mp.nseg; e.coord_seg4 = mp.seg4;
+                e.nb_coord = B * 27 * mp.nseg;
+            }
             int splits = (int)(((int64_t)g.HoWo + 4095) / 4096);
             if (splits > 32) splits = 32;
             if (splits < 1) splits = 1;
@@ -2420,7 +2483,10 @@
             }
             hipLaunchKernelGGL(dcn_sweep_epilogue, dim3(e.nb_coord + Cout * splits + nb_dw), dim3(256), 0, stream, e);
         }
-        if (!handover) return hipGetLastError() == hipSuccess ? DCD_OK : DCD_ERR_LAUNCH;
+        if (!handover) {
+            if (grad_out) dcd_internal::channel_sum_combine_launch(stream, bias_ws, B * mp.nseg, 27, grad_out_bias);
+            return hipGetLastError() == hipSuccess ? DCD_OK : DCD_ERR_LAUNCH;
+        }
         inv.packed = 0;
         inv.tileflag = nullptr;
         hipLaunchKernelGGL(dcn_offset_blockmax, bm_grid, dim3(64), 0, stream, offset, g, blockmax, fs);
@@ -2467,7 +2533,7 @@
             else DCD_LAUNCH_BW_FAR(1);
 #undef DCD_LAUNCH_BW_FAR
         }
-        return hipGetLastError() == hipSuccess ? DCD_OK : DCD_ERR_LAUNCH;
+        return finish(fs);
     }
     int nsplit = 1;
     while ((int64_t)tiles * B * nsplit < 1536 && nsplit * 2 <= nblk) nsplit *= 2;
@@ -2653,7 +2719,31 @@
         else DCD_LAUNCH_BW(1);
 #undef DCD_LAUNCH_BW
     }
-    return hipGetLastError() == hipSuccess ? DCD_OK : DCD_ERR_LAUNCH;
+    return finish(nullptr);
+}
+
+int dcd_dcn_v2_backward(void *stream_, const float *input, const float *weight, const float *bias,
+                        const float *offset, const float *mask, const float *grad_output, float *grad_input,
+                        float *grad_offset, float *grad_mask, float *grad_weight, float *grad_bias, int B,
+                        int Cin, int H, int W, int Cout, int kh, int kw, int sh, int sw, int ph, int pw, int dh,
+                        int dw, int dg, int precision, void *workspace, size_t workspace_bytes)
+{
+    (void)bias;
+    if (!grad_offset || !grad_mask) return DCD_ERR_BAD_ARG;
+    return dcn_v2_backward_run(stream_, input, weight, offset, mask, grad_output, grad_input, grad_offset, grad_mask, nullptr, nullptr,
+                               grad_weight, grad_bias, B, Cin, H, W, Cout, kh, kw, sh, sw, ph, pw, dh, dw, dg, precision, workspace,
+                               workspace_bytes);
+}
+
+int dcd_dcn_v2_backward_merged(void *stream_, const float *input, const float *weight, const float *offset, const float *mask,
+                               const float *grad_output, float *grad_input, float *grad_out, float *grad_out_bias, float *grad_weight,
+                               float *grad_bias, int B, int Cin, int H, int W, int Cout, int kh, int kw, int sh, int sw, int ph, int pw,
+                               int dh, int dw, int dg, int precision, void *workspace, size_t workspace_bytes)
+{
+    if (!grad_out || !grad_out_bias) return DCD_ERR_BAD_ARG;
+    return dcn_v2_backward_run(stream_, input, weight, offset, mask, grad_output, grad_input, nullptr, nullptr, grad_out, grad_out_bias,
+                               grad_weight, grad_bias, B, Cin, H, W, Cout, kh, kw, sh, sw, ph, pw, dh, dw, dg, precision, workspace,
+                               workspace_bytes);
 }
 
 #ifdef SW_PROFILE
@@ -2736,16 +2826,7 @@
 {
     (void)hipGetLastError();
     if (!grad_offset || !grad_mask || !mask || !grad_out || B <= 0 || taps <= 0 || HW <= 0) return DCD_ERR_BAD_ARG;
-    const bool v4 = (HW & 3) == 0 &&
-                    (((uintptr_t)grad_offset | (uintptr_t)grad_mask | (uintptr_t)mask | (uintptr_t)grad_out) & 15) == 0;
-    const int64_t n = (int64_t)B * 3 * taps * HW / (v4 ? 4 : 1);
-    const unsigned grid = (unsigned)((n + 255) / 256 < 8192 ? (n + 255) / 256 : 8192);
-    if (v4)
-        hipLaunchKernelGGL(dcn_offset_mask_merge<4>, dim3(grid), dim3(256), 0, (hipStream_t)stream_, grad_offset, grad_mask, mask, grad_out,
-                           B, taps, HW);
-    else
-        hipLaunchKernelGGL(dcn_offset_mask_merge<1>, dim3(grid), dim3(256), 0, (hipStream_t)stream_, grad_offset, grad_mask, mask, grad_out,
-                           B, taps, HW);
+    launch_offset_mask_merge((hipStream_t)stream_, grad_offset, grad_mask, mask, grad_out, B, taps, HW, nullptr, 0);
     return hipGetLastError() == hipSuccess ? DCD_OK : DCD_ERR_LAUNCH;
 }
 
diff --git a/dcd_amd/csrc/norm.hip b/dcd_amd/csrc/norm.hip
--- a/dcd_amd/csrc/norm.hip
+++ b/dcd_amd/csrc/norm.hip
@@ -3,6 +3,7 @@
 #include <stdlib.h>
 
 #include "../../include/dcd_hip.h"
+#include "channel_sum.h"
 #include "tuning_env.h"
 
 namespace {
@@ -615,6 +616,26 @@
 
 }
 
+namespace dcd_internal {
+
+void channel_sum_combine_launch(hipStream_t stream, const double *partial, int S, int C, float *out)
+{
+    hipLaunchKernelGGL(channel_sum_combine, dim3(C), dim3(64), 0, stream, partial, S, out);
+}
+
+int channel_sums_two_launch(hipStream_t stream, const float *x, int B, int C, int64_t HW, float *sums, void *ws, size_t ws_bytes)
+{
+    if (!x || !sums || bad_shape(B, C, HW)) return DCD_ERR_BAD_ARG;
+    if (!ws || ws_bytes < dcd_bn_workspace_bytes(C)) return DCD_ERR_WORKSPACE;
+    const Plane g = make_plane(B, C, HW);
+    const int S = slices(g);
+    hipLaunchKernelGGL(channel_sum_kernel, dim3(S, C), dim3(BT), 0, stream, x, g, S, (double *)ws, (unsigned *)nullptr, sums);
+    hipLaunchKernelGGL(channel_sum_combine, dim3(C), dim3(64), 0, stream, (const double *)ws, S, sums);
+    return DCD_OK;
+}
+
+}
+
 extern "C" {
 
 size_t dcd_bn_workspace_bytes(int C) { return C > 0 ? (size_t)C * SMAX * 2 * sizeof(double) : 0; }
diff --git a/dcd_amd/model/backbone/DCNv2/dcn_v2.py b/dcd_amd/model/backbone/DCNv2/dcn_v2.py
--- a/dcd_amd/model/backbone/DCNv2/dcn_v2.py
+++ b/dcd_amd/model/backbone/DCNv2/dcn_v2.py
@@ -78,6 +78,7 @@
 
 
 _ONE_NODE = os.environ.get("DCD_DCN_NODE", "1") != "0"
+_FOLDED_BRANCH = os.environ.get("DCD_DCN_FOLDED", "1") != "0"
 
 
 class _DCNWithOffsets(Function):
@@ -90,8 +91,14 @@
         p = _precision_scope()
         ctx.precision = {} if p == "f32" else {"precision": p}
         tw, ctx.tw_back = (ops.conv3x3_step_weights(w_off, input) if ops._PREP_BOTH and ctx.needs_input_grad[0] else (None, None))
-        out = ops._conv3x3_call(input, w_off, w_off.shape[0], False, b_off.contiguous(), transformed=tw, prec=ctx.cprec)
-        offset, mask = _offset_mask_split(out)
+        from dcd_amd import _ext
+        ctx.folded = _FOLDED_BRANCH and _backend is _ext
+        if ctx.folded:
+            offset, mask = ops._conv3x3_call(input, w_off, w_off.shape[0], False, b_off.contiguous(), transformed=tw, prec=ctx.cprec,
+                                             offset_mask=True)
+        else:
+            out = ops._conv3x3_call(input, w_off, w_off.shape[0], False, b_off.contiguous(), transformed=tw, prec=ctx.cprec)
+            offset, mask = _offset_mask_split(out)
         ctx.geometry = geometry
         ctx.save_for_backward(input, offset, mask, weight, bias, w_off)
         return _backend.dcn_v2_forward(input, weight, bias, offset, mask, *geometry, **ctx.precision)
@@ -101,14 +108,19 @@
     def backward(ctx, grad_output):
         from dcd_amd import ops
         input, offset, mask, weight, bias, w_off = ctx.saved_tensors
-        grad_input, grad_offset, grad_mask, grad_weight, grad_bias = _backend.dcn_v2_backward(
-            input, weight, bias, offset, mask, grad_output.contiguous(), *ctx.geometry, **ctx.precision)
-        gout = _offset_mask_merge(grad_offset, grad_mask, mask)
+        if ctx.folded:
+            grad_input, gout, gb_sums, grad_weight, grad_bias = _backend.dcn_v2_backward(
+                input, weight, bias, offset, mask, grad_output.contiguous(), *ctx.geometry, merged=True, **ctx.precision)
+        else:
+            grad_input, grad_offset, grad_mask, grad_weight, grad_bias = _backend.dcn_v2_backward(
+                input, weight, bias, offset, mask, grad_output.contiguous(), *ctx.geometry, **ctx.precision)
+            gout = _offset_mask_merge(grad_offset, grad_mask, mask)
+            gb_sums = None
         if ctx.needs_input_grad[0]:
             grad_input = ops._conv3x3_call(gout, w_off, w_off.shape[1], True, residual=grad_input.contiguous(), transformed=ctx.tw_back,
                                            prec=ctx.cprec)
         gw_off = ops._conv3x3_wrw_call(input, gout, w_off.shape, ctx.cprec) if ctx.needs_input_grad[1] else None
-        gb_off = ops.channel_sums(gout) if ctx.needs_input_grad[2] else None
+        gb_off = (gb_sums if gb_sums is not None else ops.channel_sums(gout)) if ctx.needs_input_grad[2] else None
         return grad_input, gw_off, gb_off, grad_weight, grad_bias, None
 
 
diff --git a/dcd_amd/ops.py b/dcd_amd/ops.py
--- a/dcd_amd/ops.py
+++ b/dcd_amd/ops.py
@@ -862,7 +862,10 @@
 
 
 def _conv3x3_call(inp, weight, out_channels, backward_data, bias=None, residual=None, transformed=None, residual_inplace=True,
-                  prec=None):
+                  prec=None, offset_mask=False):
+    if offset_mask:
+        assert not backward_data and residual is None and bias is not None
+        return conv3x3_offset_mask_call(inp, weight, bias, transformed=transformed, prec=prec)
     L = _lib.lib()
     B, _, H, W = inp.shape
     Co, Ci = weight.shape[0], weight.shape[1]
@@ -907,6 +910,32 @@
     return out
 
 
+def conv3x3_offset_mask_call(inp, weight, bias, transformed=None, prec=None):
+    L = _lib.lib()
+    B, Ci, H, W = inp.shape
+    taps = weight.shape[0] // 3
+    if transformed is None:
+        prec = _conv_prec(inp) if prec is None else prec
+        if prec != PREC_F32:
+            transformed = conv3x3_transform_weights(weight, True, False, prec=prec)[0]
+    if isinstance(transformed, Bf16Weights):
+        form, w_ptr, prec = 3, transformed.tensor.data_ptr(), PREC_BF16
+    elif isinstance(transformed, SplitWeights):
+        form, w_ptr, prec = 2, transformed.tensor.data_ptr(), transformed.prec
+    elif transformed is not None:
+        form, w_ptr, prec = 1, transformed.data_ptr(), PREC_F32
+    else:
+        form, w_ptr, prec = 0, weight.data_ptr(), PREC_F32
+    offset = torch.empty((B, 2 * taps, H, W), dtype=torch.float32, device=inp.device)
+    mask = torch.empty((B, taps, H, W), dtype=torch.float32, device=inp.device)
+    n = L.dcd_conv3x3_offset_mask_workspace_bytes(B, Ci, H, W, taps, form)
+    ws = torch.empty(max(n, 16), dtype=torch.uint8, device=inp.device)
+    st = L.dcd_conv3x3_offset_mask(_lib.stream_of(inp), inp.data_ptr(), w_ptr, form, bias.data_ptr(), offset.data_ptr(), mask.data_ptr(),
+                                   B, Ci, H, W, taps, prec, ws.data_ptr(), n)
+    _lib.check(st, "dcd_conv3x3_offset_mask")
+    return offset, mask
+
+
 _PREP_BOTH = os.environ.get("DCD_CONV_PREP_BOTH", "1") != "0"
 _PREP_TABLE = os.environ.get("DCD_CONV_PREP_TABLE", "1") != "0"
 
diff --git a/include/dcd_hip.h b/include/dcd_hip.h
--- a/include/dcd_hip.h
+++ b/include/dcd_hip.h
@@ -33,6 +33,12 @@
                         float *grad_offset, float *grad_mask, float *grad_weight, float *grad_bias, int B,
                         int Cin, int H, int W, int Cout, int kh, int kw, int sh, int sw, int ph, int pw, int dh,
                         int dw, int dg, int precision, void *workspace, size_t workspace_bytes);
+
+int dcd_dcn_v2_backward_merged(void *stream, const float *input, const float *weight, const float *offset, const float *mask,
+                               const float *grad_output, float *grad_input, float *grad_out, float *grad_out_bias,
+                               float *grad_weight, float *grad_bias, int B, int Cin, int H, int W, int Cout, int kh, int kw,
+                               int sh, int sw, int ph, int pw, int dh, int dw, int dg, int precision, void *workspace,
+                               size_t workspace_bytes);
 
 int dcd_dcn_v2_forget(const float *weight);
 int dcd_dcn_v2_policy_state(const float *weight, unsigned *far_count);
@@ -216,6 +222,15 @@
                          float *output, int B, int Cin, int H, int W, int Cout, int backward_data, void *workspace,
                          size_t workspace_bytes);
 
+#define DCD_CONV_WEIGHTS_RAW 0
+#define DCD_CONV_WEIGHTS_F32 1
+#define DCD_CONV_WEIGHTS_SPLIT 2
+#define DCD_CONV_WEIGHTS_BF16 3
+size_t dcd_conv3x3_offset_mask_workspace_bytes(int B, int Cin, int H, int W, int taps, int weights_form);
+int dcd_conv3x3_offset_mask(void *stream, const float *input, const void *weights, int weights_form, const float *bias,
+                            float *offset, float *mask, int B, int Cin, int H, int W, int taps, int precision, void *workspace,
+                            size_t workspace_bytes);
+
 size_t dcd_conv3x3_split_weights_bytes(int Cin, int Cout, int backward_data);
 int dcd_conv3x3_split_transform_weights(void *stream, const float *weight, int Cin, int Cout, void *forward_out, void *backward_out);
 int dcd_conv3x3_split_transform_weights_table(void *stream, const long long *table, int entries);
```

After: 218.9 images/s. No clear change (-0.7%).
